# YiZhiXiaoGuLI/xerus

Measured on AMD Instinct MI355X. Metric: GFLOP/s on TT contraction + TT-round sweep time, order-10 rank-256, higher is better.
Workload: dtype f64; 1 GPU; TT order-10 n=20 rank-256: <x,y> + x.round(256) per step; order=10, mode_size=20, rank=256, parallelism=replicas x1

## Files before the change

include/xerus_amd.h:

```cpp
#ifndef XERUS_AMD_H
#define XERUS_AMD_H

#include <stddef.h>
#include <stdint.h>

#ifdef __cplusplus
extern "C" {
#endif

typedef struct xrs_handle_s* xrs_handle_t;

#define XRS_OK 0
#define XRS_EINVAL (-1)
#define XRS_ENOMEM (-2)
#define XRS_EHIP (-3)
#define XRS_ENUMERIC 1

int xrs_create(xrs_handle_t* handle, int device);
int xrs_destroy(xrs_handle_t handle);
int xrs_set_stream(xrs_handle_t handle, void* hip_stream);
void* xrs_get_stream(xrs_handle_t handle);
int xrs_synchronize(xrs_handle_t handle);
const char* xrs_last_error(void);
const char* xrs_version(void);

int xrs_malloc(xrs_handle_t handle, void** ptr, size_t bytes);
int xrs_free(xrs_handle_t handle, void* ptr);
size_t xrs_pool_bytes(xrs_handle_t handle);
int xrs_upload(xrs_handle_t handle, double* dst_dev, const double* src_host, size_t n);
int xrs_download(xrs_handle_t handle, double* dst_host, const double* src_dev, size_t n);
int xrs_memset_zero(xrs_handle_t handle, double* dst_dev, size_t n);
int xrs_copy(xrs_handle_t handle, double* dst_dev, const double* src_dev, size_t n);

int xrs_nrm2(xrs_handle_t handle, double* result, const double* x, size_t n);
int xrs_dot(xrs_handle_t handle, double* result, const double* x, const double* y, size_t n);
int xrs_asum(xrs_handle_t handle, double* result, const double* x, size_t n);
int xrs_scal(xrs_handle_t handle, double* x, double alpha, size_t n);
int xrs_axpy(xrs_handle_t handle, double* y, double alpha, const double* x, size_t n);
int xrs_scale_rows(xrs_handle_t handle, double* X, const double* s, size_t m, size_t n);

int xrs_gemm(xrs_handle_t handle, double* C, size_t M, size_t N, double alpha,
             const double* A, size_t lda, int transA, size_t K,
             const double* B, size_t ldb, int transB);

int xrs_gemm_batched(xrs_handle_t handle, size_t count, double* const* C, size_t M, size_t N, double alpha,
                     const double* const* A, size_t lda, int transA, size_t K,
                     const double* const* B, size_t ldb, int transB);

int xrs_gemm_sym(xrs_handle_t handle, double* C, size_t N, double alpha,
                 const double* A, size_t lda, int transA, size_t K,
                 const double* B, size_t ldb, int transB);

int xrs_gemm_f32(xrs_handle_t handle, float* C, size_t M, size_t N, float alpha,
                 const float* A, size_t lda, int transA, size_t K,
                 const float* B, size_t ldb, int transB);

int xrs_permute(xrs_handle_t handle, double* out, const double* in, size_t ndim,
                const size_t* dims, const size_t* shuffle);

int xrs_qc(xrs_handle_t handle, double* Q, double* C, size_t* rank, const double* A, size_t m, size_t n);
int xrs_cq(xrs_handle_t handle, double* C, double* Q, size_t* rank, const double* A, size_t m, size_t n);
int xrs_qr(xrs_handle_t handle, double* Q, double* R, const double* A, size_t m, size_t n);
int xrs_rq(xrs_handle_t handle, double* R, double* Q, const double* A, size_t m, size_t n);
int xrs_svd(xrs_handle_t handle, double* U, double* S, double* Vt, const double* A, size_t m, size_t n);
int xrs_svd_batched(xrs_handle_t handle, double* U, double* S, double* Vt, int* status,
                    const double* A, size_t batch, size_t m, size_t n);
int xrs_svd_batched_fits(size_t m, size_t n);
int xrs_solve(xrs_handle_t handle, double* X, const double* A, size_t m, size_t n, const double* B, size_t p);
int xrs_solve_least_squares(xrs_handle_t handle, double* X, const double* A, size_t m, size_t n, const double* B, size_t p);
int xrs_svd_rows_vt(xrs_handle_t handle, double* S, double* Vt, int* sweeps, const double* A, size_t p, size_t q, int kernel);
int xrs_sym_tridiag(xrs_handle_t handle, double* d, double* e, const double* A, size_t n);
int xrs_sym_eig_top(xrs_handle_t handle, double* lam, double* Ut, int* status, const double* A, size_t n, size_t kk);


int xrs_tt_move_core(xrs_handle_t handle, size_t d, const size_t* n, size_t* r, double** cores,
                     int canonicalized, size_t core_position, size_t position, int keep_rank);
int xrs_tt_round(xrs_handle_t handle, size_t d, const size_t* n, size_t* r, double** cores,
                 int canonicalized, size_t core_position, const size_t* max_ranks, double eps);
int xrs_tt_soft_threshold(xrs_handle_t handle, size_t d, const size_t* n, size_t* r, double** cores,
                          int canonicalized, size_t core_position, const double* taus);
int xrs_tt_entrywise_product(xrs_handle_t handle, size_t d, const size_t* ext, const size_t* ra, const double* const* A,
                             const size_t* rb, const double* const* B, double alpha, double** out);
int xrs_tt_entrywise_square(xrs_handle_t handle, size_t d, const size_t* ext, const size_t* r, const double* const* A,
                            double alpha, double** out, size_t* r_out);
int xrs_tt_rank_one_argmax(xrs_handle_t handle, size_t d, const size_t* ext, const double* const* cores, size_t* pos);
int xrs_tt_operator_apply(xrs_handle_t handle, size_t d, const size_t* n, const size_t* m, const size_t* p, const size_t* ra,
                          const double* const* A, const size_t* rb, const double* const* B, int transpose_a, double** out);
#define XRS_ROUND_CHAIN 1
#define XRS_ROUND_TRUNCATE 2
#define XRS_ROUND_REFERENCE 3
#define XRS_ROUND_GENERAL 4
int xrs_tt_last_round_path(xrs_handle_t handle);
int xrs_tt_dot(xrs_handle_t handle, double* result, size_t d, const size_t* n,
               const size_t* rx, const double* const* xcores,
               const size_t* ry, const double* const* ycores);

int xrs_tt_dot_async(xrs_handle_t handle, size_t d, const size_t* n,
                     const size_t* rx, const double* const* xcores,
                     const size_t* ry, const double* const* ycores);
int xrs_tt_dot_wait(xrs_handle_t handle, double* result);
int xrs_tt_dot_f32(xrs_handle_t handle, double* result, size_t d, const size_t* n,
                   const size_t* rx, const double* const* xcores,
                   const size_t* ry, const double* const* ycores);

int xrs_tt_tangent_project(xrs_handle_t handle, size_t d, const size_t* n, const size_t* ru, const double* const* U,
                           const size_t* rz, const double* const* Z, double** V, double** UU, size_t* fallback_edges);
int xrs_tt_tangent_to_tt(xrs_handle_t handle, size_t d, const size_t* n, const size_t* r, const double* const* U,
                         const double* const* V, int add_base, double** out);
int xrs_tt_tangent_dot(xrs_handle_t handle, double* result, size_t d, const size_t* n, const size_t* r,
                       const double* const* UU, const double* const* A, const double* const* B);

typedef int (*xrs_allreduce_fn)(void* ctx, double* buf, size_t count);
typedef int (*xrs_allgather_fn)(void* ctx, const double* send, double* recv, size_t count);

typedef struct xrs_comm_s* xrs_comm_t;
int xrs_comm_unique_id(void* id128_out);
int xrs_comm_create(xrs_handle_t handle, int nranks, int rank, const void* id128, xrs_comm_t* comm_out);
int xrs_comm_destroy(xrs_comm_t comm);
size_t xrs_comm_calls(xrs_comm_t comm);
int xrs_comm_allreduce(void* comm, double* buf, size_t count);
int xrs_comm_emulate(xrs_handle_t handle, int nranks, xrs_comm_t* comm_out);
int xrs_comm_allgather(void* comm, const double* send, double* recv, size_t count);

int xrs_tt_gather_sharded(xrs_handle_t handle, size_t d, const size_t* n_global, int world, int rank, const size_t* r,
                          const double* const* local_cores, double** full_cores_out, xrs_allgather_fn allgather, void* ctx);
int xrs_tt_shard(xrs_handle_t handle, size_t d, const size_t* n_global, int world, int rank, const size_t* r,
                 const double* const* full_cores, double** local_out);

int xrs_tt_round_sharded(xrs_handle_t handle, size_t d, const size_t* n_local, size_t* r, double** cores,
                         const size_t* max_ranks, double eps, xrs_allreduce_fn allreduce, void* ctx, int* certified);

int xrs_tt_round_sharded_ex(xrs_handle_t handle, size_t d, const size_t* n_local, size_t* r, double** cores,
                            const size_t* max_ranks, double eps, int world, int rank, xrs_allreduce_fn allreduce,
                            void* ctx, int* path);

int xrs_tt_dot_sharded(xrs_handle_t handle, double* result, size_t d, const size_t* n_local, const size_t* rx,
                       const double* const* X, const size_t* ry, const double* const* Y, xrs_allreduce_fn allreduce,
                       void* ctx);

int xrs_uq_basis(xrs_handle_t handle, double* P, const double* xi, size_t N, size_t n);
int xrs_uq_stack_congruence(xrs_handle_t handle, double* Lout, const double* Lprev, const double* X, const double* P,
                            size_t N, size_t a, size_t n, size_t b);
int xrs_uq_quadform(xrs_handle_t handle, double* result, const double* L, const double* V, size_t N, size_t a);


int xrs_philox_words(xrs_handle_t handle, uint32_t* out, size_t s, size_t q, uint64_t seed, uint32_t stream);
int xrs_gaussian_matrix(xrs_handle_t handle, double* G, size_t s, size_t m, uint64_t seed, uint32_t stream);
#define XRS_SKETCH_FUSED 1
#define XRS_SKETCH_MATERIALISED 2
int xrs_sketch_gaussian(xrs_handle_t handle, double* Y, size_t s, const double* A, size_t m, size_t n, uint64_t seed,
                        uint32_t stream, int route);
int xrs_sketch_last_route(xrs_handle_t handle);

#define XRS_KFAM_GEMM 1u
#define XRS_KFAM_PERMUTE 2u
#define XRS_KFAM_QR 4u
#define XRS_KFAM_SVD 8u
#define XRS_KFAM_ELEMWISE 16u
#define XRS_KFAM_SPLITK 32u
int xrs_prof_begin(xrs_handle_t handle, uint32_t family_mask);
int xrs_prof_end(xrs_handle_t handle, size_t* launches, double* total_ms, double* flops, double* bytes);

#ifdef __cplusplus
}
#endif
#endif
```

xerus_amd/capi.py:

```python
from __future__ import annotations

import ctypes as C
import os
from typing import Sequence

import numpy as np

_HERE = os.path.dirname(os.path.abspath(__file__))
LIB_PATH = os.environ.get("XRS_LIB_PATH") or os.path.join(_HERE, "libxerus_amd.so")

_SZ = C.c_size_t
_DP = C.c_void_p

SIGNATURES = {
    "xrs_create": (C.c_int, [C.POINTER(_DP), C.c_int]),
    "xrs_destroy": (C.c_int, [_DP]),
    "xrs_set_stream": (C.c_int, [_DP, _DP]),
    "xrs_get_stream": (_DP, [_DP]),
    "xrs_synchronize": (C.c_int, [_DP]),
    "xrs_last_error": (C.c_char_p, []),
    "xrs_version": (C.c_char_p, []),
    "xrs_malloc": (C.c_int, [_DP, C.POINTER(_DP), _SZ]),
    "xrs_free": (C.c_int, [_DP, _DP]),
    "xrs_pool_bytes": (_SZ, [_DP]),
    "xrs_upload": (C.c_int, [_DP, _DP, _DP, _SZ]),
    "xrs_download": (C.c_int, [_DP, _DP, _DP, _SZ]),
    "xrs_memset_zero": (C.c_int, [_DP, _DP, _SZ]),
    "xrs_copy": (C.c_int, [_DP, _DP, _DP, _SZ]),
    "xrs_nrm2": (C.c_int, [_DP, C.POINTER(C.c_double), _DP, _SZ]),
    "xrs_dot": (C.c_int, [_DP, C.POINTER(C.c_double), _DP, _DP, _SZ]),
    "xrs_asum": (C.c_int, [_DP, C.POINTER(C.c_double), _DP, _SZ]),
    "xrs_scal": (C.c_int, [_DP, _DP, C.c_double, _SZ]),
    "xrs_axpy": (C.c_int, [_DP, _DP, C.c_double, _DP, _SZ]),
    "xrs_scale_rows": (C.c_int, [_DP, _DP, _DP, _SZ, _SZ]),
    "xrs_gemm": (C.c_int, [_DP, _DP, _SZ, _SZ, C.c_double, _DP, _SZ, C.c_int, _SZ, _DP, _SZ, C.c_int]),
    "xrs_gemm_f32": (C.c_int, [_DP, _DP, _SZ, _SZ, C.c_float, _DP, _SZ, C.c_int, _SZ, _DP, _SZ, C.c_int]),
    "xrs_gemm_sym": (C.c_int,[_DP, _DP, _SZ, C.c_double, _DP, _SZ, C.c_int, _SZ, _DP, _SZ, C.c_int]),
    "xrs_gemm_batched": (C.c_int, [_DP, _SZ, C.POINTER(_DP), _SZ, _SZ, C.c_double, C.POINTER(_DP), _SZ, C.c_int, _SZ,
                                   C.POINTER(_DP), _SZ, C.c_int]),
    "xrs_permute": (C.c_int, [_DP, _DP, _DP, _SZ, C.POINTER(_SZ), C.POINTER(_SZ)]),
    "xrs_qc": (C.c_int, [_DP, _DP, _DP, C.POINTER(_SZ), _DP, _SZ, _SZ]),
    "xrs_cq": (C.c_int, [_DP, _DP, _DP, C.POINTER(_SZ), _DP, _SZ, _SZ]),
    "xrs_qr": (C.c_int, [_DP, _DP, _DP, _DP, _SZ, _SZ]),
    "xrs_rq": (C.c_int, [_DP, _DP, _DP, _DP, _SZ, _SZ]),
    "xrs_svd": (C.c_int, [_DP, _DP, _DP, _DP, _DP, _SZ, _SZ]),
    "xrs_svd_batched": (C.c_int, [_DP, _DP, _DP, _DP, C.POINTER(C.c_int), _DP, _SZ, _SZ, _SZ]),
    "xrs_svd_batched_fits": (C.c_int, [_SZ, _SZ]),
    "xrs_solve": (C.c_int, [_DP, _DP, _DP, _SZ, _SZ, _DP, _SZ]),
    "xrs_solve_least_squares": (C.c_int, [_DP, _DP, _DP, _SZ, _SZ, _DP, _SZ]),
    "xrs_svd_rows_vt": (C.c_int, [_DP, _DP, _DP, C.POINTER(C.c_int), _DP, _SZ, _SZ, C.c_int]),
    "xrs_sym_eig_top": (C.c_int, [_DP, _DP, _DP, C.POINTER(C.c_int), _DP, _SZ, _SZ]),
    "xrs_sym_tridiag": (C.c_int, [_DP, _DP, _DP, _DP, _SZ]),
    "xrs_tt_entrywise_product": (C.c_int, [_DP, _SZ, C.POINTER(_SZ), C.POINTER(_SZ), C.POINTER(_DP), C.POINTER(_SZ), C.POINTER(_DP),
                                           C.c_double, C.POINTER(_DP)]),
    "xrs_tt_entrywise_square": (C.c_int, [_DP, _SZ, C.POINTER(_SZ), C.POINTER(_SZ), C.POINTER(_DP), C.c_double, C.POINTER(_DP),
                                          C.POINTER(_SZ)]),
    "xrs_tt_rank_one_argmax": (C.c_int, [_DP, _SZ, C.POINTER(_SZ), C.POINTER(_DP), C.POINTER(_SZ)]),
    "xrs_tt_operator_apply": (C.c_int, [_DP, _SZ, C.POINTER(_SZ), C.POINTER(_SZ), C.POINTER(_SZ), C.POINTER(_SZ), C.POINTER(_DP),
                                        C.POINTER(_SZ), C.POINTER(_DP), C.c_int, C.POINTER(_DP)]),
    "xrs_tt_move_core": (C.c_int, [_DP, _SZ, C.POINTER(_SZ), C.POINTER(_SZ), C.POINTER(_DP), C.c_int, _SZ, _SZ, C.c_int]),
    "xrs_tt_round": (C.c_int, [_DP, _SZ, C.POINTER(_SZ), C.POINTER(_SZ), C.POINTER(_DP), C.c_int, _SZ,
                               C.POINTER(_SZ), C.c_double]),
    "xrs_tt_dot": (C.c_int, [_DP, C.POINTER(C.c_double), _SZ, C.POINTER(_SZ), C.POINTER(_SZ), C.POINTER(_DP),
                             C.POINTER(_SZ), C.POINTER(_DP)]),
    "xrs_tt_dot_async": (C.c_int, [_DP, _SZ, C.POINTER(_SZ), C.POINTER(_SZ), C.POINTER(_DP), C.POINTER(_SZ),
                                   C.POINTER(_DP)]),
    "xrs_tt_dot_wait": (C.c_int, [_DP, C.POINTER(C.c_double)]),
    "xrs_tt_dot_f32": (C.c_int, [_DP, C.POINTER(C.c_double), _SZ, C.POINTER(_SZ), C.POINTER(_SZ), C.POINTER(_DP),
                                 C.POINTER(_SZ), C.POINTER(_DP)]),
    "xrs_tt_round_sharded": (C.c_int, [_DP, _SZ, C.POINTER(_SZ), C.POINTER(_SZ), C.POINTER(_DP), C.POINTER(_SZ),
                                       C.c_double, _DP, _DP, C.POINTER(C.c_int)]),
    "xrs_tt_round_sharded_ex": (C.c_int, [_DP, _SZ, C.POINTER(_SZ), C.POINTER(_SZ), C.POINTER(_DP), C.POINTER(_SZ),
                                          C.c_double, C.c_int, C.c_int, _DP, _DP, C.POINTER(C.c_int)]),
    "xrs_tt_dot_sharded": (C.c_int, [_DP, C.POINTER(C.c_double), _SZ, C.POINTER(_SZ), C.POINTER(_SZ), C.POINTER(_DP),
                                     C.POINTER(_SZ), C.POINTER(_DP), _DP, _DP]),
    "xrs_tt_tangent_project": (C.c_int, [_DP, _SZ, C.POINTER(_SZ), C.POINTER(_SZ), C.POINTER(_DP), C.POINTER(_SZ),
                                         C.POINTER(_DP), C.POINTER(_DP), C.POINTER(_DP), C.POINTER(_SZ)]),
    "xrs_tt_tangent_to_tt": (C.c_int, [_DP, _SZ, C.POINTER(_SZ), C.POINTER(_SZ), C.POINTER(_DP), C.POINTER(_DP), C.c_int,
                                       C.POINTER(_DP)]),
    "xrs_tt_tangent_dot": (C.c_int, [_DP, C.POINTER(C.c_double), _SZ, C.POINTER(_SZ), C.POINTER(_SZ), C.POINTER(_DP),
                                     C.POINTER(_DP), C.POINTER(_DP)]),
    "xrs_tt_last_round_path": (C.c_int, [_DP]),
    "xrs_tt_soft_threshold": (C.c_int, [_DP, _SZ, C.POINTER(_SZ), C.POINTER(_SZ), C.POINTER(_DP), C.c_int, _SZ,
                                        C.POINTER(C.c_double)]),
    "xrs_comm_unique_id": (C.c_int, [_DP]),
    "xrs_comm_create": (C.c_int, [_DP, C.c_int, C.c_int, _DP, C.POINTER(_DP)]),
    "xrs_comm_emulate": (C.c_int, [_DP, C.c_int, C.POINTER(_DP)]),
    "xrs_comm_destroy": (C.c_int, [_DP]),
    "xrs_comm_calls": (_SZ, [_DP]),
    "xrs_comm_allreduce": (C.c_int, [_DP, _DP, _SZ]),
    "xrs_comm_allgather": (C.c_int, [_DP, _DP, _DP, _SZ]),
    "xrs_tt_gather_sharded": (C.c_int, [_DP, _SZ, C.POINTER(_SZ), C.c_int, C.c_int, C.POINTER(_SZ), C.POINTER(_DP),
                                        C.POINTER(_DP), _DP, _DP]),
    "xrs_tt_shard": (C.c_int, [_DP, _SZ, C.POINTER(_SZ), C.c_int, C.c_int, C.POINTER(_SZ), C.POINTER(_DP), C.POINTER(_DP)]),
    "xrs_uq_basis": (C.c_int, [_DP, _DP, _DP, _SZ, _SZ]),
    "xrs_uq_stack_congruence": (C.c_int, [_DP, _DP, _DP, _DP, _DP, _SZ, _SZ, _SZ, _SZ]),
    "xrs_uq_quadform": (C.c_int, [_DP, C.POINTER(C.c_double), _DP, _DP, _SZ, _SZ]),
    "xrs_philox_words": (C.c_int, [_DP, _DP, _SZ, _SZ, C.c_uint64, C.c_uint32]),
    "xrs_gaussian_matrix": (C.c_int, [_DP, _DP, _SZ, _SZ, C.c_uint64, C.c_uint32]),
    "xrs_sketch_gaussian": (C.c_int, [_DP, _DP, _SZ, _DP, _SZ, _SZ, C.c_uint64, C.c_uint32, C.c_int]),
    "xrs_sketch_last_route": (C.c_int, [_DP]),
    "xrs_prof_begin": (C.c_int, [_DP, C.c_uint32]),
    "xrs_prof_end": (C.c_int, [_DP, C.POINTER(_SZ), C.POINTER(C.c_double), C.POINTER(C.c_double),
                               C.POINTER(C.c_double)]),
}

KFAM_GEMM, KFAM_PERMUTE, KFAM_QR, KFAM_SVD, KFAM_ELEMWISE, KFAM_SPLITK = 1, 2, 4, 8, 16, 32
ROUND_PATHS = {0: None, 1: "chain", 2: "truncate", 3: "reference", 4: "general"}
SKETCH_AUTO, SKETCH_FUSED, SKETCH_MATERIALISED = 0, 1, 2
SKETCH_ROUTES = {0: None, 1: "fused", 2: "materialised"}

_lib = None


class XrsError(RuntimeError):

    def __init__(self, fn: str, code: int, msg: str):
        super().__init__(f"{fn} failed with status {code}: {msg}")
        self.code = code


def load(path: str | None = None) -> C.CDLL:
    global _lib
    if _lib is not None and path is None:
        return _lib
    p = path or LIB_PATH
    if not os.path.exists(p):
        raise ImportError(f"{p} is missing: build it with `python -c 'import __graft_entry__ as g; g.build()'`")
    lib = C.CDLL(p)
    for name, (res, args) in SIGNATURES.items():
        f = getattr(lib, name)
        f.restype = res
        f.argtypes = args
    if path is None:
        _lib = lib
    return lib


def _check(fn: str, status: int):
    if status != 0:
        raise XrsError(fn, status, load().xrs_last_error().decode())


def svd_batched_fits(m: int, n: int) -> bool:
    return bool(load().xrs_svd_batched_fits(int(m), int(n)))


def _arr(vals: Sequence[int]):
    return (_SZ * len(vals))(*[int(v) for v in vals])


class Handle:

    def __init__(self, device: int = 0):
        self.lib = load()
        self.h = _DP()
        _check("xrs_create", self.lib.xrs_create(C.byref(self.h), device))

    def close(self):
        if self.h:
            _check("xrs_destroy", self.lib.xrs_destroy(self.h))
            self.h = _DP()

    def __del__(self):
        try:
            self.close()
        except Exception:
            pass

    def malloc(self, nbytes: int) -> int:
        p = _DP()
        _check("xrs_malloc", self.lib.xrs_malloc(self.h, C.byref(p), nbytes))
        return p.value or 0

    def free(self, ptr: int):
        _check("xrs_free", self.lib.xrs_free(self.h, _DP(ptr)))

    def synchronize(self):
        _check("xrs_synchronize", self.lib.xrs_synchronize(self.h))

    def set_stream(self, stream_ptr: int | None):
        _check("xrs_set_stream", self.lib.xrs_set_stream(self.h, _DP(stream_ptr or 0)))

    def stream(self) -> int:
        return self.lib.xrs_get_stream(self.h) or 0

    def array(self, a: np.ndarray) -> "DeviceArray":
        return DeviceArray.from_host(self, a)

    def empty(self, shape) -> "DeviceArray":
        return DeviceArray(self, tuple(int(s) for s in shape))

    def zeros(self, shape) -> "DeviceArray":
        d = DeviceArray(self, tuple(int(s) for s in shape))
        _check("xrs_memset_zero", self.lib.xrs_memset_zero(self.h, _DP(d.ptr), d.size))
        return d

    def gemm(self, C_: "DeviceArray", M, N, alpha, A: "DeviceArray", lda, transA, K, B: "DeviceArray", ldb, transB):
        _check("xrs_gemm", self.lib.xrs_gemm(self.h, _DP(C_.ptr), M, N, alpha, _DP(A.ptr), lda, int(transA), K,
                                            _DP(B.ptr), ldb, int(transB)))

    def gemm_f32(self, C_: "Float32Array", M, N, alpha, A: "Float32Array", lda, transA, K, B: "Float32Array", ldb, transB):
        _check("xrs_gemm_f32", self.lib.xrs_gemm_f32(self.h, _DP(C_.ptr), M, N, float(alpha), _DP(A.ptr), lda, int(transA),
                                                    K, _DP(B.ptr), ldb, int(transB)))

    def array_f32(self, a: np.ndarray) -> "Float32Array":
        return Float32Array.from_host(self, a)

    def gemm_sym(self, C_: "DeviceArray", N, alpha, A: "DeviceArray", lda, transA, K, B: "DeviceArray", ldb, transB):
        _check("xrs_gemm_sym", self.lib.xrs_gemm_sym(self.h, _DP(C_.ptr), N, alpha, _DP(A.ptr), lda, int(transA), K,
                                                    _DP(B.ptr), ldb, int(transB)))

    def gemm_batched(self, Cs, M, N, alpha, As, lda, transA, K, Bs, ldb, transB):
        cnt = len(Cs)
        tab = lambda xs: (_DP * max(1, cnt))(*[_DP(x.ptr) for x in xs])
        _check("xrs_gemm_batched", self.lib.xrs_gemm_batched(self.h, cnt, tab(Cs), M, N, alpha, tab(As), lda, int(transA),
                                                            K, tab(Bs), ldb, int(transB)))

    def tangent_to_tt(self, n, r, Us, Vs, add_base: bool):
        d = len(n)
        tab = lambda xs: (_DP * d)(*[_DP(x.ptr) for x in xs])
        out = (_DP * d)()
        _check("xrs_tt_tangent_to_tt", self.lib.xrs_tt_tangent_to_tt(self.h, d, _arr(n), _arr(r), tab(Us), tab(Vs),
                                                                    int(add_base), out))
        cores = []
        for k in range(d):
            shape = (2 * r[k] if k else 1, n[k], 2 * r[k + 1] if k + 1 < d else 1)
            c = DeviceArray(self, shape, ptr=out[k])
            c.owned = True
            cores.append(c)
        return cores

    def matmul(self, A: "DeviceArray", transA: bool, B: "DeviceArray", transB: bool, alpha: float = 1.0):
        am, ak = (A.shape[1], A.shape[0]) if transA else (A.shape[0], A.shape[1])
        bk, bn = (B.shape[1], B.shape[0]) if transB else (B.shape[0], B.shape[1])
        assert ak == bk, (A.shape, B.shape)
        out = self.empty((am, bn))
        self.gemm(out, am, bn, alpha, A, A.shape[1], transA, ak, B, B.shape[1], transB)
        return out

    def permute(self, out: "DeviceArray", inp: "DeviceArray", dims, shuffle):
        _check("xrs_permute", self.lib.xrs_permute(self.h, _DP(out.ptr), _DP(inp.ptr), len(dims), _arr(dims),
                                                  _arr(shuffle)))

    def reshuffle(self, inp: "DeviceArray", shuffle):
        dims = inp.shape
        out_dims = [0] * len(dims)
        for i, s in enumerate(shuffle):
            out_dims[s] = dims[i]
        out = self.empty(tuple(out_dims))
        self.permute(out, inp, dims, shuffle)
        return out

    def nrm2(self, x: "DeviceArray") -> float:
        r = C.c_double()
        _check("xrs_nrm2", self.lib.xrs_nrm2(self.h, C.byref(r), _DP(x.ptr), x.size))
        return r.value

    def dot(self, x: "DeviceArray", y: "DeviceArray") -> float:
        r = C.c_double()
        _check("xrs_dot", self.lib.xrs_dot(self.h, C.byref(r), _DP(x.ptr), _DP(y.ptr), x.size))
        return r.value

    def asum(self, x: "DeviceArray") -> float:
        r = C.c_double()
        _check("xrs_asum", self.lib.xrs_asum(self.h, C.byref(r), _DP(x.ptr), x.size))
        return r.value

    def scal(self, x: "DeviceArray", alpha: float):
        _check("xrs_scal", self.lib.xrs_scal(self.h, _DP(x.ptr), alpha, x.size))

    def axpy(self, y: "DeviceArray", alpha: float, x: "DeviceArray"):
        _check("xrs_axpy", self.lib.xrs_axpy(self.h, _DP(y.ptr), alpha, _DP(x.ptr), x.size))

    def scale_rows(self, X: "DeviceArray", s: "DeviceArray"):
        _check("xrs_scale_rows", self.lib.xrs_scale_rows(self.h, _DP(X.ptr), _DP(s.ptr), X.shape[0], X.size // max(1, X.shape[0])))

    def qc(self, A: "DeviceArray"):
        m, n = A.shape
        k = min(m, n)
        Q, Cm = self.empty((m, k)), self.empty((k, n))
        r = _SZ()
        _check("xrs_qc", self.lib.xrs_qc(self.h, _DP(Q.ptr), _DP(Cm.ptr), C.byref(r), _DP(A.ptr), m, n))
        rank = r.value
        Q.shape, Cm.shape = (m, rank), (rank, n)
        return Q, Cm, rank

    def cq(self, A: "DeviceArray"):
        m, n = A.shape
        k = min(m, n)
        Cm, Q = self.empty((m, k)), self.empty((k, n))
        r = _SZ()
        _check("xrs_cq", self.lib.xrs_cq(self.h, _DP(Cm.ptr), _DP(Q.ptr), C.byref(r), _DP(A.ptr), m, n))
        rank = r.value
        Cm.shape, Q.shape = (m, rank), (rank, n)
        return Cm, Q, rank

    def qr(self, A: "DeviceArray"):
        m, n = A.shape
        k = min(m, n)
        Q, R = self.empty((m, k)), self.empty((k, n))
        _check("xrs_qr", self.lib.xrs_qr(self.h, _DP(Q.ptr), _DP(R.ptr), _DP(A.ptr), m, n))
        return Q, R

    def rq(self, A: "DeviceArray"):
        m, n = A.shape
        k = min(m, n)
        R, Q = self.empty((m, k)), self.empty((k, n))
        _check("xrs_rq", self.lib.xrs_rq(self.h, _DP(R.ptr), _DP(Q.ptr), _DP(A.ptr), m, n))
        return R, Q

    def svd(self, A: "DeviceArray"):
        m, n = A.shape
        k = min(m, n)
        U, S, Vt = self.empty((m, k)), self.empty((k,)), self.empty((k, n))
        _check("xrs_svd", self.lib.xrs_svd(self.h, _DP(U.ptr), _DP(S.ptr), _DP(Vt.ptr), _DP(A.ptr), m, n))
        return U, S, Vt

    def svd_batched(self, A: "DeviceArray", want_status: bool = True):
        batch, m, n = A.shape
        k = min(m, n)
        U, S, Vt = self.empty((batch, m, k)), self.empty((batch, k)), self.empty((batch, k, n))
        st = np.zeros(batch, dtype=np.intc) if want_status else None
        _check("xrs_svd_batched", self.lib.xrs_svd_batched(
            self.h, _DP(U.ptr), _DP(S.ptr), _DP(Vt.ptr), st.ctypes.data_as(C.POINTER(C.c_int)) if want_status else None,
            _DP(A.ptr), batch, m, n))
        return U, S, Vt, st

    def solve(self, A: "DeviceArray", B: "DeviceArray", least_squares: bool = False):
        m, n = A.shape
        p = B.shape[1] if len(B.shape) == 2 else 1
        X = self.empty((n, p) if len(B.shape) == 2 else (n,))
        fn = "xrs_solve_least_squares" if least_squares else "xrs_solve"
        _check(fn, getattr(self.lib, fn)(self.h, _DP(X.ptr), _DP(A.ptr), m, n, _DP(B.ptr), p))
        return X

    def sym_eig_top(self, A: "DeviceArray", kk: int):
        n = A.shape[0]
        lam, Ut, st = self.empty((kk,)), self.empty((kk, n)), C.c_int()
        _check("xrs_sym_eig_top", self.lib.xrs_sym_eig_top(self.h, _DP(lam.ptr), _DP(Ut.ptr), C.byref(st), _DP(A.ptr), n, kk))
        return lam, Ut, st.value

    def sym_tridiag(self, A: "DeviceArray"):
        n = A.shape[0]
        d, e = self.empty((n,)), self.empty((n,))
        _check("xrs_sym_tridiag", self.lib.xrs_sym_tridiag(self.h, _DP(d.ptr), _DP(e.ptr), _DP(A.ptr), n))
        return d.numpy(), e.numpy()[: n - 1]

    def svd_rows_vt(self, A: "DeviceArray", kernel: int = 0):
        p, q = A.shape
        S, Vt, sw = self.empty((p,)), self.empty((p, q)), C.c_int()
        _check("xrs_svd_rows_vt", self.lib.xrs_svd_rows_vt(self.h, _DP(S.ptr), _DP(Vt.ptr), C.byref(sw), _DP(A.ptr), p, q, kernel))
        return S, Vt, sw.value

    def tt_operator_apply(self, n, m, ra, A, rb, B, p=None, transpose=False):
        d = len(n)
        out = (_DP * d)()
        tab = lambda xs: (_DP * d)(*[_DP(x.ptr) for x in xs])
        _check("xrs_tt_operator_apply", self.lib.xrs_tt_operator_apply(
            self.h, d, _arr(n), _arr(m), _arr(p) if p is not None else None, _arr(ra), tab(A), _arr(rb), tab(B),
            int(transpose), out))
        res = []
        for k in range(d):
            nk = m[k] if transpose else n[k]
            shape = (ra[k] * rb[k], nk) + ((p[k],) if p is not None else ()) + (ra[k + 1] * rb[k + 1],)
            arr = DeviceArray(self, shape, ptr=out[k], owned=False)
            res.append(arr.numpy())
            self.free(out[k])
        return res

    def uq_basis(self, xi: "DeviceArray", n: int) -> "DeviceArray":
        N = xi.size
        P = self.empty((N, n))
        _check("xrs_uq_basis", self.lib.xrs_uq_basis(self.h, _DP(P.ptr), _DP(xi.ptr), N, n))
        return P

    def uq_stack_congruence(self, Lprev: "DeviceArray | None", X: "DeviceArray", P: "DeviceArray") -> "DeviceArray":
        a, n, b = X.shape
        N = P.shape[0]
        out = self.empty((N, b, b))
        _check("xrs_uq_stack_congruence", self.lib.xrs_uq_stack_congruence(
            self.h, _DP(out.ptr), _DP(Lprev.ptr) if Lprev is not None else None, _DP(X.ptr), _DP(P.ptr), N, a, n, b))
        return out

    def uq_quadform(self, L: "DeviceArray | None", V: "DeviceArray") -> float:
        N, a = V.shape
        r = C.c_double()
        _check("xrs_uq_quadform", self.lib.xrs_uq_quadform(self.h, C.byref(r), _DP(L.ptr) if L is not None else None,
                                                          _DP(V.ptr), N, a))
        return r.value

    @staticmethod
    def _seed_stream(fn: str, seed: int, stream: int):
        if not 0 <= int(seed) < 2 ** 64:
            raise XrsError(fn, -1, f"seed {seed} is not a 64-bit word")
        if not 0 <= int(stream) < 2 ** 32:
            raise XrsError(fn, -1, f"stream {stream} must be below 2^32")
        return int(seed), int(stream)

    def philox_words(self, s: int, q: int, seed: int, stream: int = 0) -> np.ndarray:
        seed, stream = self._seed_stream("xrs_philox_words", seed, stream)
        legal = 0 < s <= 2 ** 32 and q > 0
        buf = self.empty((2 * s * q,)) if legal else None
        _check("xrs_philox_words", self.lib.xrs_philox_words(self.h, _DP(buf.ptr) if legal else None, s, q, seed, stream))
        return buf.numpy().view(np.uint32).reshape(s, q, 4)

    def gaussian_matrix(self, s: int, m: int, seed: int, stream: int = 0) -> "DeviceArray":
        seed, stream = self._seed_stream("xrs_gaussian_matrix", seed, stream)
        legal = 0 < s <= 2 ** 32 and m > 0
        G = self.empty((s, m)) if legal else None
        _check("xrs_gaussian_matrix", self.lib.xrs_gaussian_matrix(self.h, _DP(G.ptr) if legal else None, s, m, seed, stream))
        return G

    def sketch_gaussian(self, s: int, A: "DeviceArray", seed: int, stream: int = 0, route: int = 0, m: int | None = None,
                        out: "DeviceArray | None" = None) -> "DeviceArray":
        seed, stream = self._seed_stream("xrs_sketch_gaussian", seed, stream)
        n = A.shape[1]
        m = A.shape[0] if m is None else int(m)
        legal = 0 < s <= 2 ** 32 and m > 0 and n > 0
        Y = out if out is not None else (self.empty((s, n)) if legal else None)
        _check("xrs_sketch_gaussian", self.lib.xrs_sketch_gaussian(self.h, _DP(Y.ptr) if Y is not None else None, s, _DP(A.ptr),
                                                                  m, n, seed, stream, int(route)))
        return Y

    def sketch_last_route(self) -> str | None:
        return SKETCH_ROUTES[self.lib.xrs_sketch_last_route(self.h)]

    def last_round_path(self) -> str | None:
        return ROUND_PATHS[self.lib.xrs_tt_last_round_path(self.h)]

    def prof_begin(self, mask: int):
        _check("xrs_prof_begin", self.lib.xrs_prof_begin(self.h, mask))

    def prof_end(self):
        n, ms, fl, by = _SZ(), C.c_double(), C.c_double(), C.c_double()
        _check("xrs_prof_end", self.lib.xrs_prof_end(self.h, C.byref(n), C.byref(ms), C.byref(fl), C.byref(by)))
        return {"launches": n.value, "ms": ms.value, "flops": fl.value, "bytes": by.value}


class DeviceArray:

    def __init__(self, handle: Handle, shape: tuple, ptr: int | None = None, owned: bool = True):
        self.handle = handle
        self.shape = tuple(shape)
        self.capacity = self.size
        self.owned = owned and ptr is None
        self.ptr = ptr if ptr is not None else (handle.malloc(max(8, self.capacity * 8)))

    @property
    def size(self) -> int:
        return int(np.prod(self.shape)) if self.shape else 1

    @classmethod
    def from_host(cls, handle: Handle, a: np.ndarray) -> "DeviceArray":
        a = np.ascontiguousarray(a, dtype=np.float64)
        d = cls(handle, a.shape)
        if a.size:
            _check("xrs_upload", handle.lib.xrs_upload(handle.h, _DP(d.ptr), a.ctypes.data_as(_DP), a.size))
        return d

    def numpy(self) -> np.ndarray:
        out = np.empty(self.shape, dtype=np.float64)
        assert self.size <= self.capacity, "shape exceeds the allocation"
        if self.size:
            _check("xrs_download", self.handle.lib.xrs_download(self.handle.h, out.ctypes.data_as(_DP), _DP(self.ptr),
                                                               self.size))
        return out

    def free(self):
        if self.owned and self.ptr:
            self.handle.free(self.ptr)
        self.ptr = 0

    def __del__(self):
        try:
            self.free()
        except Exception:
            pass


class Float32Array:

    def __init__(self, handle: Handle, shape: tuple, offset: int = 0):
        self.handle = handle
        self.shape = tuple(int(s) for s in shape)
        self.offset = int(offset)
        self._words = max(1, (self.size + self.offset + 1) // 2)
        self.base = handle.malloc(8 * self._words)
        self.ptr = self.base + 4 * self.offset

    @property
    def size(self) -> int:
        return int(np.prod(self.shape)) if self.shape else 1

    @classmethod
    def from_host(cls, handle: Handle, a: np.ndarray, offset: int = 0) -> "Float32Array":
        a = np.ascontiguousarray(a, dtype=np.float32)
        d = cls(handle, a.shape, offset)
        buf = np.zeros(2 * d._words, dtype=np.float32)
        buf[d.offset:d.offset + a.size] = a.ravel()
        _check("xrs_upload", handle.lib.xrs_upload(handle.h, _DP(d.base), buf.view(np.float64).ctypes.data_as(_DP), d._words))
        return d

    def numpy(self) -> np.ndarray:
        buf = np.empty(self._words, dtype=np.float64)
        _check("xrs_download", self.handle.lib.xrs_download(self.handle.h, buf.ctypes.data_as(_DP), _DP(self.base), self._words))
        return buf.view(np.float32)[self.offset:self.offset + self.size].reshape(self.shape).copy()

    def free(self):
        if self.base:
            self.handle.free(self.base)
        self.base = self.ptr = 0

    def __del__(self):
        try:
            self.free()
        except Exception:
            pass


class DotFuture:

    def __init__(self, handle: Handle):
        self.handle = handle
        self._value = None

    def result(self) -> float:
        if self._value is None:
            out = C.c_double()
            _check("xrs_tt_dot_wait", self.handle.lib.xrs_tt_dot_wait(self.handle.h, C.byref(out)))
            self._value = out.value
        return self._value


class TTDevice:

    def __init__(self, handle: Handle, dims, ranks, ptrs, canonicalized=False, core_position=0):
        self.handle = handle
        self.dims = [int(x) for x in dims]
        self.r = [int(x) for x in ranks]
        self.ptrs = list(ptrs)
        self.canonicalized = canonicalized
        self.core_position = core_position

    @classmethod
    def from_cores(cls, handle: Handle, cores, canonicalized=False, core_position=0) -> "TTDevice":
        dims = [c.shape[1] for c in cores]
        ranks = [cores[0].shape[0]] + [c.shape[2] for c in cores]
        ptrs = []
        for c in cores:
            c = np.ascontiguousarray(c, dtype=np.float64)
            p = handle.malloc(max(8, c.size * 8))
            _check("xrs_upload", handle.lib.xrs_upload(handle.h, _DP(p), c.ctypes.data_as(_DP), c.size))
            ptrs.append(p)
        return cls(handle, dims, ranks, ptrs, canonicalized, core_position)

    def clone(self) -> "TTDevice":
        ptrs = []
        for k, p in enumerate(self.ptrs):
            size = self.r[k] * self.dims[k] * self.r[k + 1]
            q = self.handle.malloc(max(8, size * 8))
            _check("xrs_copy", self.handle.lib.xrs_copy(self.handle.h, _DP(q), _DP(p), size))
            ptrs.append(q)
        return TTDevice(self.handle, self.dims, self.r, ptrs, self.canonicalized, self.core_position)

    @property
    def order(self):
        return len(self.dims)

    @property
    def ranks(self):
        return self.r[1:-1]

    def cores(self):
        out = []
        for k, p in enumerate(self.ptrs):
            shp = (self.r[k], self.dims[k], self.r[k + 1])
            a = np.empty(shp)
            _check("xrs_download", self.handle.lib.xrs_download(self.handle.h, a.ctypes.data_as(_DP), _DP(p), a.size))
            out.append(a)
        return out

    def _arrays(self):
        c = getattr(self, "_cache", None)
        if c is not None and c[3] is self.r and c[4] is self.ptrs:
            return c[0], c[1], c[2]
        d = self.order
        n = _arr(self.dims)
        r = _arr(self.r)
        cores = (_DP * d)(*self.ptrs)
        self._cache = (n, r, cores, self.r, self.ptrs)
        return n, r, cores

    def _writeback(self, r, cores):
        self.r = r[:]
        self.ptrs = [p or 0 for p in cores[:]]
        c = getattr(self, "_cache", None)
        if c is not None and c[1] is r and c[2] is cores:
            self._cache = (c[0], r, cores, self.r, self.ptrs)

    def move_core(self, position: int, keep_rank: bool = False):
        n, r, cores = self._arrays()
        st = self.handle.lib.xrs_tt_move_core(self.handle.h, self.order, n, r, cores, int(self.canonicalized),
                                              self.core_position, position, int(keep_rank))
        self._writeback(r, cores)
        _check("xrs_tt_move_core", st)
        self.canonicalized, self.core_position = True, position

    def round(self, max_ranks, eps: float = 8 * np.finfo(float).eps):
        d = self.order
        if isinstance(max_ranks, (int, np.integer)):
            max_ranks = [int(max_ranks)] * (d - 1)
        n, r, cores = self._arrays()
        key = tuple(max_ranks)
        mc = getattr(self, "_mr_cache", None)
        if mc is None or mc[0] != key:
            mc = (key, _arr(list(max_ranks) + [1]))
            self._mr_cache = mc
        mr = mc[1]
        st = self.handle.lib.xrs_tt_round(self.handle.h, d, n, r, cores, int(self.canonicalized), self.core_position,
                                          mr, eps)
        self._writeback(r, cores)
        _check("xrs_tt_round", st)
        self.canonicalized, self.core_position = True, 0

    def soft_threshold(self, taus):
        d = self.order
        if isinstance(taus, (int, float)):
            taus = [float(taus)] * (d - 1)
        n, r, cores = self._arrays()
        t = (C.c_double * max(1, d - 1))(*taus)
        st = self.handle.lib.xrs_tt_soft_threshold(self.handle.h, d, n, r, cores, int(self.canonicalized),
                                                   self.core_position, t)
        self._writeback(r, cores)
        _check("xrs_tt_soft_threshold", st)
        self.canonicalized, self.core_position = True, 0

    def dot(self, other: "TTDevice") -> float:
        if self.dims != other.dims:
            raise ValueError(f"dot of TTs with different dimensions: {self.dims} vs {other.dims}")
        out = C.c_double()
        n, rx, xc = self._arrays()
        _, ry, yc = other._arrays()
        _check("xrs_tt_dot", self.handle.lib.xrs_tt_dot(self.handle.h, C.byref(out), self.order, n, rx, xc, ry, yc))
        return out.value

    def dot_f32(self, other: "TTDevice") -> float:
        if self.dims != other.dims:
            raise ValueError(f"dot of TTs with different dimensions: {self.dims} vs {other.dims}")
        out = C.c_double()
        n, rx, xc = self._arrays()
        _, ry, yc = other._arrays()
        _check("xrs_tt_dot_f32", self.handle.lib.xrs_tt_dot_f32(self.handle.h, C.byref(out), self.order, n, rx, xc, ry, yc))
        return out.value

    def dot_async(self, other: "TTDevice") -> "DotFuture":
        if self.dims != other.dims:
            raise ValueError(f"dot of TTs with different dimensions: {self.dims} vs {other.dims}")
        if other.handle is not self.handle:
            raise ValueError("dot_async: both TTs must live on the same handle")
        n, rx, xc = self._arrays()
        _, ry, yc = other._arrays()
        _check("xrs_tt_dot_async", self.handle.lib.xrs_tt_dot_async(self.handle.h, self.order, n, rx, xc, ry, yc))
        return DotFuture(self.handle)

    def entrywise_square(self, alpha: float = 1.0) -> "TTDevice":
        d = self.order
        n, r, cores = self._arrays()
        out, r_out = (_DP * d)(), (_SZ * (d + 1))()
        _check("xrs_tt_entrywise_square", self.handle.lib.xrs_tt_entrywise_square(self.handle.h, d, n, r, cores, float(alpha),
                                                                                  out, r_out))
        return TTDevice(self.handle, self.dims, list(r_out), [p or 0 for p in out])

    def rank_one_argmax(self) -> list:
        if any(x != 1 for x in self.r):
            raise ValueError(f"rank_one_argmax needs ranks 1, got {self.r}")
        d = self.order
        n, _, cores = self._arrays()
        pos = (_SZ * d)()
        _check("xrs_tt_rank_one_argmax", self.handle.lib.xrs_tt_rank_one_argmax(self.handle.h, d, n, cores, pos))
        return [int(p) for p in pos]

    def frob_norm(self) -> float:
        if self.canonicalized:
            k = self.core_position
            size = self.r[k] * self.dims[k] * self.r[k + 1]
            return self.handle.nrm2(DeviceArray(self.handle, (size,), ptr=self.ptrs[k], owned=False))
        return float(np.sqrt(max(0.0, self.dot(self))))

    def free(self):
        for p in self.ptrs:
            if p:
                self.handle.free(p)
        self.ptrs = [0] * len(self.ptrs)

    def __del__(self):
        try:
            self.free()
        except Exception:
            pass
```

xerus_amd/csrc/chol_batch.hip:

```cpp
#include <algorithm>

#include "tt_common.hpp"

namespace xrs {

namespace {

using ttd::GemmJob;
using ttd::gemm_grouped;

static_assert(kCholLaunchJobs == kPotrfBatchMax);
constexpr int kBigMax = 64;
struct BigJob {
    const double* src;
    double shift_rel;
    int n;
    double* L;
    double* Z;
};

struct BigArgs {
    const double* src[kBigMax];
    double* w11[kBigMax];
    double* w21[kBigMax];
    double* w22[kBigMax];
    double shift[kBigMax];
    int n[kBigMax];
};

__global__ void __launch_bounds__(256) k_split_shift(const BigArgs a) {
    const int j = blockIdx.y, n = a.n[j], n1 = 256, n2 = n - 256;
    const double* A = a.src[j];
    __shared__ double red[4];
    double tr = 0.0;
    for (int i = threadIdx.x; i < n; i += 256) tr += A[size_t(i) * n + i];
#pragma unroll
    for (int o = 32; o > 0; o >>= 1) tr += __shfl_xor(tr, o, 64);
    if ((threadIdx.x & 63) == 0) red[threadIdx.x >> 6] = tr;
    __syncthreads();
    const double shift = a.shift[j] * (red[0] + red[1] + red[2] + red[3]);
    const size_t total = size_t(n) * n;
    for (size_t e = size_t(blockIdx.x) * 256 + threadIdx.x; e < total; e += size_t(gridDim.x) * 256) {
        const int r = int(e / n), c = int(e - size_t(r) * n);
        const double v = A[e] + (r == c ? shift : 0.0);
        if (r < n1 && c < n1) a.w11[j][size_t(r) * n1 + c] = v;
        else if (r >= n1 && c < n1) a.w21[j][size_t(r - n1) * n1 + c] = v;
        else if (r >= n1 && c >= n1) a.w22[j][size_t(r - n1) * n2 + (c - n1)] = v;
    }
}

struct SubArgs {
    double* y[kBigMax];
    const double* x[kBigMax];
    int count[kBigMax];
};

__global__ void __launch_bounds__(256) k_sub_batched(const SubArgs a) {
    const int j = blockIdx.y;
    for (int e = blockIdx.x * 256 + threadIdx.x; e < a.count[j]; e += gridDim.x * 256) a.y[j][e] -= a.x[j][e];
}

struct AssembleArgs {
    double* out[kBigMax];
    const double* b11[kBigMax];
    const double* b21[kBigMax];
    const double* b22[kBigMax];
    int n[kBigMax];
};

__global__ void __launch_bounds__(256) k_assemble_lower(const AssembleArgs a) {
    const int j = blockIdx.y, n = a.n[j], n1 = 256, n2 = n - 256;
    const size_t total = size_t(n) * n;
    for (size_t e = size_t(blockIdx.x) * 256 + threadIdx.x; e < total; e += size_t(gridDim.x) * 256) {
        const int r = int(e / n), c = int(e - size_t(r) * n);
        double v = 0.0;
        if (r < n1) v = c < n1 ? a.b11[j][size_t(r) * n1 + c] : 0.0;
        else v = c < n1 ? a.b21[j][size_t(r - n1) * n1 + c] : a.b22[j][size_t(r - n1) * n2 + (c - n1)];
        a.out[j][e] = v;
    }
}


void factor_big(xrs_handle_t h, const std::vector<BigJob>& jobs, int* status, std::vector<DevBuf>& keep) {
    const int nj = int(jobs.size());
    XRS_REQUIRE(nj <= kBigMax, "factor_big: too many jobs");
    constexpr int n1 = 256;
    BigArgs ba{};
    std::vector<double*> w11(nj), w21(nj), w22(nj), d11(nj), d22(nj), z11(nj), pp(nj);
    auto buf = [&](size_t elems) { keep.emplace_back(h, std::max<size_t>(elems, 1) * 8); return keep.back().d(); };
    size_t maxn2 = 0;
    for (int j = 0; j < nj; ++j) {
        const int n = jobs[j].n, n2 = n - n1;
        XRS_REQUIRE(n > n1 && n <= 2 * n1, "factor_big: n out of range");
        w11[j] = buf(size_t(n1) * n1);
        w21[j] = buf(size_t(n2) * n1);
        w22[j] = buf(size_t(n2) * n2);
        d11[j] = buf(dinv_elems(n1));
        d22[j] = buf(dinv_elems(n2));
        z11[j] = buf(size_t(n1) * n1);
        pp[j] = buf(size_t(n2) * n2);
        ba.src[j] = jobs[j].src;
        ba.w11[j] = w11[j];
        ba.w21[j] = w21[j];
        ba.w22[j] = w22[j];
        ba.shift[j] = jobs[j].shift_rel;
        ba.n[j] = n;
        maxn2 = std::max(maxn2, size_t(n2));
    }
    hipLaunchKernelGGL(k_split_shift, dim3(256, nj), dim3(256), 0, h->stream, ba);
    check_launch("k_split_shift");
    auto chol = [&](const std::vector<double*>& W, const std::vector<double*>& D, int first_slot, bool upper_half) {
        for (int b0 = 0; b0 < nj; b0 += kPotrfBatchMax) {
            PotrfBatch pb{};
            const int c = std::min(kPotrfBatchMax, nj - b0);
            for (int i = 0; i < c; ++i) {
                pb.src[i] = nullptr;
                pb.G[i] = W[b0 + i];
                pb.Dinv[i] = D[b0 + i];
                pb.shift[i] = 0.0;
                pb.n[i] = upper_half ? n1 : jobs[b0 + i].n - n1;
            }
            pb.status = status + first_slot + b0;
            potrf_batched(h, pb, c);
        }
    };
    auto inverse = [&](const std::vector<double*>& L, const std::vector<double*>& D, const std::vector<double*>& X,
                       bool upper_half, const std::vector<int>& which) {
        TrinvBatch tb{};
        int c = 0;
        for (int j : which) {
            tb.L[c] = L[j];
            tb.Dinv[c] = D[j];
            tb.X[c] = X[j];
            tb.n[c] = upper_half ? n1 : jobs[j].n - n1;
            ++c;
        }
        if (c) trinv_batched(h, tb, c);
    };
    std::vector<int> all(nj), fac;
    for (int j = 0; j < nj; ++j) {
        all[j] = j;
        if (jobs[j].L) fac.push_back(j);
    }
    chol(w11, d11, 0, true);
    inverse(w11, d11, z11, true, all);
    std::vector<GemmJob> g1, g2;
    for (int j = 0; j < nj; ++j) {
        const size_t n2 = size_t(jobs[j].n - n1);
        g1.push_back({n2, size_t(n1), size_t(n1), size_t(n1), size_t(n1), false, true, w21[j], z11[j], w21[j] == nullptr ? nullptr : buf(n2 * n1)});
    }
    std::vector<double*> l21(nj);
    for (int j = 0; j < nj; ++j) l21[j] = g1[j].C;
    gemm_grouped(h, g1);
    for (int j = 0; j < nj; ++j) {
        const size_t n2 = size_t(jobs[j].n - n1);
        g2.push_back({n2, n2, size_t(n1), size_t(n1), size_t(n1), false, true, l21[j], l21[j], pp[j], true});
    }
    gemm_grouped(h, g2);
    SubArgs sa{};
    for (int j = 0; j < nj; ++j) {
        sa.y[j] = w22[j];
        sa.x[j] = pp[j];
        sa.count[j] = (jobs[j].n - n1) * (jobs[j].n - n1);
    }
    hipLaunchKernelGGL(k_sub_batched, dim3(64, nj), dim3(256), 0, h->stream, sa);
    check_launch("k_sub_batched");
    chol(w22, d22, nj, false);
    if (fac.empty()) return;
    std::vector<double*> z22(nj, nullptr), tt(nj, nullptr), z21(nj, nullptr);
    for (int j : fac) {
        const size_t n2 = size_t(jobs[j].n - n1);
        z22[j] = buf(n2 * n2);
        tt[j] = buf(n2 * n1);
        z21[j] = buf(n2 * n1);
    }
    inverse(w22, d22, z22, false, fac);
    std::vector<GemmJob> g3, g4;
    for (int j : fac) {
        const size_t n2 = size_t(jobs[j].n - n1);
        g3.push_back({n2, size_t(n1), size_t(n1), size_t(n1), size_t(n1), false, false, l21[j], z11[j], tt[j]});
    }
    gemm_grouped(h, g3);
    for (int j : fac) {
        const size_t n2 = size_t(jobs[j].n - n1);
        GemmJob g{n2, size_t(n1), n2, n2, size_t(n1), false, false, z22[j], tt[j], z21[j]};
        g.alpha = -1.0;
        g4.push_back(g);
    }
    gemm_grouped(h, g4);
    AssembleArgs al{}, az{};
    int c = 0;
    for (int j : fac) {
        al.out[c] = jobs[j].L; al.b11[c] = w11[j]; al.b21[c] = l21[j]; al.b22[c] = w22[j]; al.n[c] = jobs[j].n;
        az.out[c] = jobs[j].Z; az.b11[c] = z11[j]; az.b21[c] = z21[j]; az.b22[c] = z22[j]; az.n[c] = jobs[j].n;
        ++c;
    }
    hipLaunchKernelGGL(k_assemble_lower, dim3(256, c), dim3(256), 0, h->stream, al);
    check_launch("k_assemble_lower");
    hipLaunchKernelGGL(k_assemble_lower, dim3(256, c), dim3(256), 0, h->stream, az);
    check_launch("k_assemble_lower");
}

}

int chol_status_count(const std::vector<CholJob>& jobs) {
    int c = 0;
    for (const CholJob& j : jobs) c += j.n > 512 ? chol_full_blocks(size_t(j.n)) : (j.n > 256 ? 2 : 1);
    return c;
}

void chol_enqueue(xrs_handle_t h, const std::vector<CholJob>& jobs, int* status, std::vector<DevBuf>& keep) {
    std::vector<const CholJob*> small, huge;
    std::vector<BigJob> big;
    size_t dsz = 0;
    for (const CholJob& j : jobs) {
        XRS_REQUIRE(j.A != nullptr && j.n >= 1, "chol_enqueue: empty job");
        if (j.n > 512) {
            huge.push_back(&j);
        } else if (j.n > 256) {
            double* Z = j.Z;
            if (j.L && !Z) {
                keep.emplace_back(h, size_t(j.n) * j.n * 8);
                Z = keep.back().d();
            }
            big.push_back({j.A, j.shift, j.n, j.L, Z});
        } else {
            small.push_back(&j);
            dsz += dinv_elems(j.n);
        }
    }
    const int ns = int(small.size());
    int slot = ns + 2 * int(big.size());
    for (const CholJob* j : huge) {
        chol_full(h, j->A, size_t(j->n), j->shift, j->L, j->Z, status + slot);
        slot += chol_full_blocks(size_t(j->n));
    }
    for (size_t b0 = 0; b0 < big.size(); b0 += kBigMax) {
        const std::vector<BigJob> part(big.begin() + long(b0), big.begin() + long(std::min(big.size(), b0 + kBigMax)));
        factor_big(h, part, status + ns + 2 * b0, keep);
    }
    if (ns == 0) return;
    keep.emplace_back(h, dsz * 8);
    double* dinv = keep.back().d();
    struct Inverse { const double* L; const double* Dinv; double* X; int n; };
    std::vector<Inverse> inv;
    for (int b0 = 0; b0 < ns; b0 += kPotrfBatchMax) {
        PotrfBatch pb{};
        const int c = std::min(kPotrfBatchMax, ns - b0);
        for (int i = 0; i < c; ++i) {
            const CholJob& j = *small[size_t(b0 + i)];
            pb.src[i] = j.A;
            pb.G[i] = j.L;
            pb.Dinv[i] = dinv;
            pb.shift[i] = j.shift;
            pb.n[i] = j.n;
            if (j.L && j.Z) inv.push_back({j.L, dinv, j.Z, j.n});
            dinv += dinv_elems(j.n);
        }
        pb.status = status + b0;
        potrf_batched(h, pb, c);
    }
    for (size_t b0 = 0; b0 < inv.size(); b0 += kTrinvBatchMax) {
        TrinvBatch tb{};
        const int c = int(std::min<size_t>(kTrinvBatchMax, inv.size() - b0));
        for (int i = 0; i < c; ++i) {
            const Inverse& v = inv[b0 + size_t(i)];
            tb.L[i] = v.L;
            tb.Dinv[i] = v.Dinv;
            tb.X[i] = v.X;
            tb.n[i] = v.n;
        }
        trinv_batched(h, tb, c);
    }
}

}
```

xerus_amd/csrc/elementwise.hpp:

```cpp
#pragma once
#include <algorithm>

#include "runtime.hpp"

namespace xrs {

void reduce_to_device(xrs_handle_t h, int mode, const double* x, const double* y, size_t n, double* out_dev,
                      double* partial = nullptr);
double reduce_to_host(xrs_handle_t h, int mode, const double* x, const double* y, size_t n);
void scal(xrs_handle_t h, double* x, double alpha, size_t n);
void axpy(xrs_handle_t h, double* y, double alpha, const double* x, size_t n);
void ldexp_copy(xrs_handle_t h, double* dst, const double* src, int ex, size_t n);
constexpr int kAmaxMany = 64;
void amax_enqueue(xrs_handle_t h, const double* const* x, const size_t* n, int count, double* out_dev);
void norms_enqueue(xrs_handle_t h, const double* const* x, const size_t* n, int count, double* out_dev);
int range_exponent(double am);
int range_exponent(xrs_handle_t h, const double* A, size_t n);
void scale_rows(xrs_handle_t h, double* X, const double* s, size_t m, size_t n);
void scale_cols(xrs_handle_t h, double* X, const double* s, size_t m, size_t n);
void diag_sum(xrs_handle_t h, double* out, const double* X, size_t P, size_t m);
void offset_add(xrs_handle_t h, double* out, const size_t* out_dims, const double* in, const size_t* in_dims, size_t nd,
                const size_t* offsets, double alpha);
void strided_eval(xrs_handle_t h, double* out, const double* in, size_t nd, const size_t* out_dims, const size_t* in_strides,
                  size_t nt, const size_t* tr_dims, const size_t* tr_strides, size_t base);

constexpr int kTriA = 1, kTriB = 2;
void gemm(xrs_handle_t h, double* C, size_t M, size_t N, double alpha, const double* A, size_t lda, bool ta, size_t K,
          const double* B, size_t ldb, bool tb, int tri = 0);
constexpr int kGemmBatchMax = 32;
void gemm_batched(xrs_handle_t h, int count, double* const* C, size_t M, size_t N, double alpha, const double* const* A,
                  size_t lda, bool ta, size_t K, const double* const* B, size_t ldb, bool tb, bool sym = false,
                  int tri = 0);
void gemm_sym(xrs_handle_t h, double* C, size_t N, double alpha, const double* A, size_t lda, bool ta, size_t K,
              const double* B, size_t ldb, bool tb);

struct GemmSpec {
    const double* A;
    const double* B;
    double* C;
    size_t M, N, K, lda, ldb;
    bool ta, tb;
};
inline void gemm(xrs_handle_t h, const GemmSpec& g) {
    gemm(h, g.C, g.M, g.N, 1.0, g.A, g.lda, g.ta, g.K, g.B, g.ldb, g.tb);
}

void permute(xrs_handle_t h, double* out, const double* in, size_t ndim, const size_t* dims, const size_t* shuffle);

}
```

xerus_amd/csrc/gemm.hip:

```cpp
#include <algorithm>
#include <type_traits>
#include <utility>
#include <cstdio>
#include <cstdlib>

#include <hip/hip_ext.h>

#include "elementwise.hpp"
#include "runtime.hpp"

namespace xrs {

typedef double d4 __attribute__((ext_vector_type(4)));

struct GemmOne {
    const double* A;
    const double* B;
    double* C;
    __host__ __device__ const double* a(int) const { return A; }
    __host__ __device__ const double* b(int) const { return B; }
    __device__ double* c(int) const { return C; }
};
struct GemmMany {
    const double* A[kGemmBatchMax];
    const double* B[kGemmBatchMax];
    double* C[kGemmBatchMax];
    __host__ __device__ const double* a(int i) const { return A[i]; }
    __host__ __device__ const double* b(int i) const { return B[i]; }
    __device__ double* c(int i) const { return C[i]; }
};

template <int BM, int BN, int WGM, int WGN, int WGK>
constexpr int gemm_min_waves() { return (BM * BN >= 128 * 128) ? 2 : 4; }

#ifdef XRS_GEMM_TRACE
__device__ unsigned long long* g_gemm_trace = nullptr;
__device__ unsigned long long* g_gemm_steps = nullptr;
#define XRS_TRACE_BEGIN                                                   \
    const unsigned long long xrs_t0 = __builtin_amdgcn_s_memrealtime();  \
    const unsigned long long xrs_c0 = __builtin_amdgcn_s_memtime();
#define XRS_TRACE_STEP(t)                                                                                   \
    if (threadIdx.x == 0 && g_gemm_steps != nullptr && (t) < 15) {                                          \
        const size_t wg = blockIdx.x + size_t(gridDim.x) * (blockIdx.y + size_t(gridDim.y) * blockIdx.z);   \
        g_gemm_steps[16 * wg + (t)] = __builtin_amdgcn_s_memtime() - xrs_c0;                                \
    }
#define XRS_TRACE_END                                                                                     \
    if (threadIdx.x == 0 && g_gemm_trace != nullptr) {                                                    \
        const size_t wg = blockIdx.x + size_t(gridDim.x) * (blockIdx.y + size_t(gridDim.y) * blockIdx.z); \
        const unsigned long long t1 = __builtin_amdgcn_s_memrealtime();                                   \
        const unsigned hw = __builtin_amdgcn_s_getreg((31 << 11) | 4);                 \
        const unsigned xcc = __builtin_amdgcn_s_getreg((31 << 11) | 20);              \
        g_gemm_trace[3 * wg] = xrs_t0;                                                                   \
        g_gemm_trace[3 * wg + 1] = t1;                                                                   \
        g_gemm_trace[3 * wg + 2] = (static_cast<unsigned long long>(xcc) << 32) | hw;                    \
        if (g_gemm_steps != nullptr) g_gemm_steps[16 * wg + 15] = __builtin_amdgcn_s_memtime() - xrs_c0;  \
    }
#else
#define XRS_TRACE_BEGIN
#define XRS_TRACE_END
#define XRS_TRACE_STEP(t)
#endif

template <int BM, int BN, int GBK, int WGM, int WGN, int WGK, int PD, bool TA, bool TB, class PTR>
__device__ __forceinline__ void gemm_body(const PTR& ptrs, size_t lda, size_t ldb, int M, int N, int K, int kps,
                                          double alpha, double* __restrict__ slab, int tiles_m, int xcd_group,
                                          int* __restrict__ tickets, int sym);

template <int BM, int BN, int GBK, int WGM, int WGN, int WGK, int PD, bool TA, bool TB, class PTR>
__global__ void __launch_bounds__(WGM * WGN * WGK * 64, (gemm_min_waves<BM, BN, WGM, WGN, WGK>()))
k_gemm_f64(const PTR ptrs, size_t lda, size_t ldb, int M, int N, int K, int kps, double alpha,
           double* __restrict__ slab, int tiles_m, int xcd_group, int* __restrict__ tickets, int sym) {
    XRS_TRACE_BEGIN
    gemm_body<BM, BN, GBK, WGM, WGN, WGK, PD, TA, TB, PTR>(ptrs, lda, ldb, M, N, K, kps, alpha, slab, tiles_m,
                                                          xcd_group, tickets, sym);
    XRS_TRACE_END
}

template <int TM, int TN, int WGM, int WGN, int WGK, int NACC, class PTR>
__device__ __forceinline__ void gemm_finish(d4 (&acc2)[NACC][TM][TN], double* lds, const PTR& ptrs, int M, int N,
                                            double alpha, double* __restrict__ slab, int* __restrict__ tickets,
                                            int sym, int m0, int n0, int wm, int wn, int kg, int pos, int xb, int yb, int zb) {
    const int bz = yb;
    double* __restrict__ C = ptrs.c(bz);
    const int zslice = bz * int(gridDim.z) + zb;
    const int tslot = bz * int(gridDim.x) + xb;
    const int tid = threadIdx.x;
    const int lane = tid & 63;
    const bool mirror = sym != 0;
    d4 acc[TM][TN];
#pragma unroll
    for (int i = 0; i < TM; ++i)
#pragma unroll
        for (int j = 0; j < TN; ++j) {
            acc[i][j] = acc2[0][i][j];
            if constexpr (NACC > 1) acc[i][j] += acc2[1][i][j];
        }
    if constexpr (WGK > 1) {
        double* red = lds;
        if (kg > 0) {
#pragma unroll
            for (int i = 0; i < TM; ++i)
#pragma unroll
                for (int j = 0; j < TN; ++j)
#pragma unroll
                    for (int r = 0; r < 4; ++r)
                        red[((((kg - 1) * (WGM * WGN) + pos) * TM * TN + i * TN + j) * 4 + r) * 64 + lane] = acc[i][j][r];
        }
        __syncthreads();
        if (kg > 0 && tickets == nullptr) return;
        if (kg == 0)
#pragma unroll
        for (int g = 1; g < WGK; ++g)
#pragma unroll
            for (int i = 0; i < TM; ++i)
#pragma unroll
                for (int j = 0; j < TN; ++j)
#pragma unroll
                    for (int r = 0; r < 4; ++r)
                        acc[i][j][r] += red[((((g - 1) * (WGM * WGN) + pos) * TM * TN + i * TN + j) * 4 + r) * 64 + lane];
    }
    const bool to_slab = slab != nullptr;
    const size_t MN = size_t(M) * size_t(N);
    double* out = to_slab ? slab + size_t(zslice) * MN : C;
    const double scale = to_slab ? 1.0 : alpha;
    const int lc = lane & 15, lg = lane >> 4;
    if (kg == 0) {
#pragma unroll
        for (int i = 0; i < TM; ++i)
#pragma unroll
            for (int j = 0; j < TN; ++j) {
                const int col = n0 + wn + j * 16 + lc;
#pragma unroll
                for (int r = 0; r < 4; ++r) {
                    const int row = m0 + wm + i * 16 + lg + 4 * r;
                    if (row < M && col < N) {
                        if (tickets != nullptr)
                            __hip_atomic_store(&out[size_t(row) * N + col], acc[i][j][r], __ATOMIC_RELAXED,
                                               __HIP_MEMORY_SCOPE_AGENT);
                        else if (!mirror || to_slab)
                            out[size_t(row) * N + col] = scale * acc[i][j][r];
                        else if (row >= col) {
                            out[size_t(row) * N + col] = scale * acc[i][j][r];
                            out[size_t(col) * N + row] = scale * acc[i][j][r];
                        }
                    }
                }
            }
    }
    if (tickets == nullptr) return;
    asm volatile("s_waitcnt vmcnt(0)" ::: "memory");
    __syncthreads();
    double* flag = lds;
    if (tid == 0) {
        const int t = __hip_atomic_fetch_add(&tickets[tslot], 1, __ATOMIC_RELAXED, __HIP_MEMORY_SCOPE_AGENT);
        const bool last = (t == int(gridDim.z) - 1);
        if (last) __hip_atomic_store(&tickets[tslot], 0, __ATOMIC_RELAXED, __HIP_MEMORY_SCOPE_AGENT);
        flag[0] = last ? 1.0 : 0.0;
    }
    __syncthreads();
    if (flag[0] == 0.0 || kg != 0) return;
#pragma unroll
    for (int i = 0; i < TM; ++i)
#pragma unroll
        for (int j = 0; j < TN; ++j) {
            const int col = n0 + wn + j * 16 + lc;
#pragma unroll
            for (int r = 0; r < 4; ++r) {
                const int row = m0 + wm + i * 16 + lg + 4 * r;
                if (row < M && col < N && (!mirror || row >= col)) {
                    const size_t o = size_t(row) * N + col;
                    double sum = 0.0;
                    for (int z = 0; z < int(gridDim.z); ++z)
                        sum += (z == zb) ? acc[i][j][r]
                                                      : __hip_atomic_load(&slab[(size_t(bz) * gridDim.z + z) * MN + o], __ATOMIC_RELAXED,
                                                                          __HIP_MEMORY_SCOPE_AGENT);
                    C[o] = alpha * sum;
                    if (mirror) C[size_t(col) * N + row] = alpha * sum;
                }
            }
        }
}


template <int BM, int BN, int GBK, int WGM, int WGN, int WGK, int PD, bool TA, bool TB, class PTR>
__device__ __forceinline__ void gemm_body(const PTR& ptrs, size_t lda, size_t ldb, int M, int N, int K, int kps,
                                          double alpha, double* __restrict__ slab, int tiles_m, int xcd_group,
                                          int* __restrict__ tickets, int sym) {
    const int bz = blockIdx.y;
    const double* __restrict__ A = ptrs.a(bz);
    const double* __restrict__ B = ptrs.b(bz);
    constexpr int NT = WGM * WGN * WGK * 64;
    constexpr int SA = BM;
    constexpr int SB = BN;
    static_assert(BM % 16 == 0 && BN % 16 == 0, "tile rows must be whole MFMA tiles");
    constexpr bool WIDE_SWZ_A = BM % 32 == 0, WIDE_SWZ_B = BN % 32 == 0;
    constexpr int WM = BM / WGM, WN = BN / WGN;
    constexpr int TM = WM / 16, TN = WN / 16;
    static_assert(TM >= 1 && TN >= 1, "wave tile smaller than one MFMA tile");
    constexpr int NACC = (TM * TN <= 2) ? 2 : 1;
    constexpr int A_PER = (BM * GBK + NT - 1) / NT;
    constexpr int B_PER = (BN * GBK + NT - 1) / NT;

    __shared__ double As[2][GBK * SA];
    __shared__ double Bs[2][GBK * SB];

    const int tid = threadIdx.x;
    const int lane = tid & 63;
    const int wave = tid >> 6;
    const int kg = wave / (WGM * WGN);
    const int pos = wave % (WGM * WGN);
    const int wm = (pos / WGN) * WM;
    const int wn = (pos % WGN) * WN;
    static_assert(GBK % (4 * WGK) == 0, "K-step must split evenly over the wave groups");
    static_assert(WGK == 1 || (WGK - 1) * BM * BN <= 2 * GBK * (SA + SB), "LDS reduction buffer too small");

    int tm, tn;
    {
        const int b = blockIdx.x, tiles_n = gridDim.x / tiles_m;
        if (xcd_group == 1) {
            const int xcd = b & 7, slot = b >> 3;
            tn = (slot / tiles_m) * 8 + xcd;
            tm = slot % tiles_m;
        } else if (xcd_group == 2) {
            const int xcd = b & 7, slot = b >> 3;
            tm = (slot / tiles_n) * 8 + xcd;
            tn = slot % tiles_n;
        } else {
            tm = b % tiles_m;
            tn = b / tiles_m;
        }
    }
    if (sym && tm < tn) return;
    const int m0 = tm * BM, n0 = tn * BN;
    const int kbeg = blockIdx.z * kps;
    const int kend = min(K, kbeg + kps);

    d4 acc2[NACC][TM][TN];
#pragma unroll
    for (int a = 0; a < NACC; ++a)
#pragma unroll
        for (int i = 0; i < TM; ++i)
#pragma unroll
            for (int j = 0; j < TN; ++j) acc2[a][i][j] = d4{0.0, 0.0, 0.0, 0.0};
    auto swza = [](int k) { return WIDE_SWZ_A ? (((k & 1) << 4) | (k & 15)) : (k & 15); };
    auto swzb = [](int k) { return WIDE_SWZ_B ? (((k & 1) << 4) | (k & 15)) : (k & 15); };

    double ra[PD][A_PER], rb[PD][B_PER];

    auto a_coord = [&](int e, int& m, int& k) {
        const int idx = tid + e * NT;
        if (TA) { m = idx % BM; k = idx / BM; } else { k = idx % GBK; m = idx / GBK; }
    };
    auto b_coord = [&](int e, int& n, int& k) {
        const int idx = tid + e * NT;
        if (TB) { k = idx % GBK; n = idx / GBK; } else { n = idx % BN; k = idx / BN; }
    };
    auto load_tile = [&](int k0, auto slot_c) {
        constexpr int slot = decltype(slot_c)::value;
#pragma unroll
        for (int e = 0; e < A_PER; ++e) {
            int m, k;
            a_coord(e, m, k);
            const int gm = min(m0 + m, M - 1), gk = min(k0 + k, kend - 1);
            ra[slot][e] = TA ? A[size_t(gk) * lda + gm] : A[size_t(gm) * lda + gk];
        }
#pragma unroll
        for (int e = 0; e < B_PER; ++e) {
            int n, k;
            b_coord(e, n, k);
            const int gn = min(n0 + n, N - 1), gk = min(k0 + k, kend - 1);
            rb[slot][e] = TB ? B[size_t(gn) * ldb + gk] : B[size_t(gk) * ldb + gn];
        }
    };
    auto store_tile = [&](int buf, int k0, auto slot_c) {
        constexpr int slot = decltype(slot_c)::value;
#pragma unroll
        for (int e = 0; e < A_PER; ++e) {
            int m, k;
            a_coord(e, m, k);
            const bool ok = (m0 + m < M) && (k0 + k < kend);
            if ((BM * GBK) % NT == 0 || tid + e * NT < BM * GBK) As[buf][k * SA + (m ^ swza(k))] = ok ? ra[slot][e] : 0.0;
        }
#pragma unroll
        for (int e = 0; e < B_PER; ++e) {
            int n, k;
            b_coord(e, n, k);
            const bool ok = (n0 + n < N) && (k0 + k < kend);
            if ((BN * GBK) % NT == 0 || tid + e * NT < BN * GBK) Bs[buf][k * SB + (n ^ swzb(k))] = ok ? rb[slot][e] : 0.0;
        }
    };
    const int lr = lane & 15, lk = lane >> 4;
    auto compute = [&](int buf) {
        const double* as = As[buf];
        const double* bs = Bs[buf];
#pragma unroll
        for (int q = 0; q < GBK / (4 * WGK); ++q) {
            const int kk = (q * WGK + kg) * 4;
            double af[TM], bf[TN];
#pragma unroll
            for (int i = 0; i < TM; ++i) af[i] = as[(kk + lk) * SA + ((wm + i * 16 + lr) ^ swza(kk + lk))];
#pragma unroll
            for (int j = 0; j < TN; ++j) bf[j] = bs[(kk + lk) * SB + ((wn + j * 16 + lr) ^ swzb(kk + lk))];
#pragma unroll
            for (int i = 0; i < TM; ++i)
#pragma unroll
                for (int j = 0; j < TN; ++j)
                    acc2[q % NACC][i][j] = __builtin_amdgcn_mfma_f64_16x16x4f64(af[i], bf[j], acc2[q % NACC][i][j], 0, 0, 0);
        }
    };

    const int nsteps = (kend > kbeg) ? (kend - kbeg + GBK - 1) / GBK : 0;
    if (nsteps > 0) {
        static_assert(PD % 2 == 0, "ring depth must be even (LDS double buffer parity)");
        [&]<int... U>(std::integer_sequence<int, U...>) {
            (load_tile(kbeg + U * GBK, std::integral_constant<int, U>{}), ...);
        }(std::make_integer_sequence<int, PD>{});
        store_tile(0, kbeg, std::integral_constant<int, 0>{});
        __syncthreads();
        int t0 = 0;
        for (; t0 + 2 * PD <= nsteps; t0 += PD) {
            [&]<int... U>(std::integer_sequence<int, U...>) {
                (([&] {
                     const int t = t0 + U;
                     compute(U & 1);
                     store_tile((U + 1) & 1, kbeg + (t + 1) * GBK, std::integral_constant<int, (U + 1) % PD>{});
                     load_tile(kbeg + (t + PD) * GBK, std::integral_constant<int, U>{});
                     __syncthreads();
                 }()),
                 ...);
            }(std::make_integer_sequence<int, PD>{});
        }
        for (; t0 < nsteps; t0 += PD) {
            [&]<int... U>(std::integer_sequence<int, U...>) {
                (([&] {
                     const int t = t0 + U;
                     if (t < nsteps) {
                         compute(U & 1);
                         if (t + 1 < nsteps)
                             store_tile((U + 1) & 1, kbeg + (t + 1) * GBK, std::integral_constant<int, (U + 1) % PD>{});
                         if (t + PD < nsteps) load_tile(kbeg + (t + PD) * GBK, std::integral_constant<int, U>{});
                     }
                     __syncthreads();
                 }()),
                 ...);
            }(std::make_integer_sequence<int, PD>{});
        }
    }

    gemm_finish<TM, TN, WGM, WGN, WGK, NACC>(acc2, &As[0][0], ptrs, M, N, alpha, slab, tickets, sym, m0, n0, wm, wn, kg, pos,
                                             int(blockIdx.x), int(blockIdx.y), int(blockIdx.z));
}

constexpr int kGldsBK = 32;

template <int R, bool KMAJ, int BK = kGldsBK>
struct GldsImg {
    static_assert(!KMAJ || R % 16 == 0, "k-major image rows must be whole MFMA tiles");
    static constexpr int KSWZ = (R % 32 == 0) ? 8 : 0;
    static constexpr int DOUBLES = R * BK;
    static constexpr int INSTR = DOUBLES * 8 / 1024;
    __device__ static int at(int r, int k) {
        if constexpr (!KMAJ) return r * BK + ((((k >> 1) ^ (r & 15))) << 1) + (k & 1);
        else return k * R + ((((r >> 1) ^ ((k & 1) * KSWZ))) << 1) + (r & 1);
    }
    template <int NF, int WGK>
    struct Frag {
        static_assert((WGK & (WGK - 1)) == 0, "wave groups must be a power of 2");
        int base[KMAJ ? NF : 1];
        int z = 0;
        __device__ Frag(int w0, int kg, int lane) {
            const int lr = lane & 15, lk = lane >> 4;
            if constexpr (!KMAJ) {
                base[0] = (w0 + lr) * BK + (lk & 1);
                z = (2 * kg) ^ (lk >> 1) ^ lr;
            } else {
                const int swz = (lk & 1) * (KSWZ / 8);
#pragma unroll
                for (int i = 0; i < NF; ++i) base[i] = (4 * kg + lk) * R + 16 * ((w0 / 16 + i) ^ swz) + lr;
            }
        }
        __device__ int off(int q, int i) const {
            if constexpr (!KMAJ) return base[0] + i * 16 * BK + (((2 * q * WGK) ^ z) << 1);
            else return base[i] + 4 * q * WGK * R;
        }
    };
    __device__ static void src(int q, int& r, int& k) {
        if constexpr (!KMAJ) {
            constexpr int CPR = BK / 2;
            r = q / CPR;
            k = ((q % CPR) ^ (r & 15)) << 1;
        } else {
            constexpr int CR = R / 2;
            k = q / CR;
            r = ((q % CR) ^ ((k & 1) * KSWZ)) << 1;
        }
    }
};

template <int BM, int BN, int WGM, int WGN, int WGK>
constexpr int glds_min_waves() { return (WGM * WGN * WGK * 64 >= 512) ? 2 : 1; }

template <int BK, int ST = 0>
constexpr int glds_stages() { return ST > 0 ? ST : (BK == 64 ? 2 : 3); }
template <int BM, int BN, int BK = kGldsBK, int ST = 0>
constexpr int glds_lds_doubles() { return glds_stages<BK, ST>() * (BM + BN) * BK; }

template <int BM, int BN, int WGM, int WGN, int WGK, bool TA, bool TB, class PTR, int BK = kGldsBK, int ST = 0>
__device__ __forceinline__ void glds_body(double* __restrict__ lds, const PTR& ptrs, size_t lda, size_t ldb, int M, int N,
                                          int K, int kps, double alpha, double* __restrict__ slab, int tiles_m,
                                          int xcd_group, int* __restrict__ tickets, int sym, int tri) {
#ifdef XRS_GEMM_TRACE
    const unsigned long long xrs_c0 = __builtin_amdgcn_s_memtime();
#endif
    constexpr int S = glds_stages<BK, ST>();
    constexpr int NW = WGM * WGN * WGK;
    using IA = GldsImg<BM, TA, BK>;
    using IB = GldsImg<BN, !TB, BK>;
    constexpr int STAGE = IA::DOUBLES + IB::DOUBLES;
    static_assert(S * STAGE == glds_lds_doubles<BM, BN, BK, ST>(), "LDS layout");
    constexpr int INSTR = IA::INSTR + IB::INSTR;
    constexpr int PER_WAVE = (INSTR + NW - 1) / NW;
    static_assert(PER_WAVE * (S - 2) <= 63, "vmcnt range");
    constexpr int WM = BM / WGM, WN = BN / WGN;
    constexpr int TM = WM / 16, TN = WN / 16;
    static_assert(TM >= 1 && TN >= 1 && WM % 16 == 0 && WN % 16 == 0, "wave tile must be whole MFMA tiles");
    static_assert(BK % (4 * WGK) == 0, "K-step must split evenly over the wave groups");
    constexpr int NACC = (TM * TN <= 2) ? 2 : 1;
    static_assert(WGK == 1 || (WGK - 1) * WGM * WGN * TM * TN * 256 <= S * STAGE, "LDS reduction buffer too small");

    int xb = int(blockIdx.x), bz = int(blockIdx.y), zb = int(blockIdx.z);
    if (xcd_group == 3) {
        const int X = int(gridDim.x), Y = int(gridDim.y);
        const int L = xb + X * (bz + Y * zb), c = L & 7, q = L >> 3;
        const int u = c + 8 * (q / X);
        xb = q % X;
        bz = u % Y;
        zb = u / Y;
    }
    const double* __restrict__ A = ptrs.a(bz);
    const double* __restrict__ B = ptrs.b(bz);
    const int tid = threadIdx.x, lane = tid & 63, wave = tid >> 6;
    const int kg = wave / (WGM * WGN), pos = wave % (WGM * WGN);
    const int wm = (pos / WGN) * WM, wn = (pos % WGN) * WN;
    int tm, tn;
    if (sym) {
        const int x = xb;
        tm = int((__builtin_sqrtf(8.0f * float(x) + 1.0f) - 1.0f) * 0.5f);
        while ((tm + 1) * (tm + 2) / 2 <= x) ++tm;
        while (tm * (tm + 1) / 2 > x) --tm;
        tn = x - tm * (tm + 1) / 2;
    } else {
        const int b = xb, tiles_n = gridDim.x / tiles_m;
        if (xcd_group == 1) {
            const int xcd = b & 7, slot = b >> 3;
            tn = (slot / tiles_m) * 8 + xcd;
            tm = slot % tiles_m;
        } else if (xcd_group == 2) {
            const int xcd = b & 7, slot = b >> 3;
            tm = (slot / tiles_n) * 8 + xcd;
            tn = slot % tiles_n;
        } else {
            tm = b % tiles_m;
            tn = b / tiles_m;
        }
    }
    const int m0 = tm * BM, n0 = tn * BN;
    const int klo = (tri & 2) ? (n0 / BK) * BK : 0;
    const int khi = (tri & 1) ? min(K, (m0 + BM + BK - 1) / BK * BK) : K;
    const int kbeg = max(zb * kps, klo);
    const int nsteps = max(0, min(khi, zb * kps + kps) - kbeg) / BK;
    const bool full = wave < INSTR % NW || INSTR % NW == 0;

    const double* gsrc[PER_WAVE];
    size_t gstep[PER_WAVE];
    int ldsoff[PER_WAVE];
#pragma unroll
    for (int u = 0; u < PER_WAVE; ++u) {
        const int j = min(wave + NW * u, INSTR - 1);
        int r, k;
        if (j < IA::INSTR) {
            IA::src((j * 64) + lane, r, k);
            gsrc[u] = TA ? A + size_t(kbeg + k) * lda + (m0 + r) : A + size_t(m0 + r) * lda + (kbeg + k);
            gstep[u] = TA ? size_t(BK) * lda : size_t(BK);
            ldsoff[u] = j * 128;
        } else {
            IB::src(((j - IA::INSTR) * 64) + lane, r, k);
            gsrc[u] = TB ? B + size_t(n0 + r) * ldb + (kbeg + k) : B + size_t(kbeg + k) * ldb + (n0 + r);
            gstep[u] = TB ? size_t(BK) : size_t(BK) * ldb;
            ldsoff[u] = IA::DOUBLES + (j - IA::INSTR) * 128;
        }
    }
    auto issue = [&](int t) {
        double* st = lds + (t % S) * STAGE;
#pragma unroll
        for (int u = 0; u < PER_WAVE; ++u)
            if (u < PER_WAVE - 1 || full)
            __builtin_amdgcn_global_load_lds(static_cast<const void*>(gsrc[u] + size_t(t) * gstep[u]),
                                             (__attribute__((address_space(3))) void*)(st + ldsoff[u]),
                                             16, 0, 0);
    };

    d4 acc2[NACC][TM][TN];
#pragma unroll
    for (int a = 0; a < NACC; ++a)
#pragma unroll
        for (int i = 0; i < TM; ++i)
#pragma unroll
            for (int j = 0; j < TN; ++j) acc2[a][i][j] = d4{0.0, 0.0, 0.0, 0.0};
    const typename IA::template Frag<TM, WGK> fa(wm, kg, lane);
    const typename IB::template Frag<TN, WGK> fb(wn, kg, lane);

#pragma unroll
    for (int s = 0; s < S - 1; ++s)
        if (s < nsteps) issue(s);
    for (int t = 0; t < nsteps; ++t) {
        const int ahead = min(S - 2, nsteps - 1 - t);
        if (ahead <= 0) asm volatile("s_waitcnt vmcnt(0)" ::: "memory");
        else if (ahead == 1) {
            if (full) asm volatile("s_waitcnt vmcnt(%0)" ::"n"(PER_WAVE) : "memory");
            else asm volatile("s_waitcnt vmcnt(%0)" ::"n"(PER_WAVE - 1) : "memory");
        } else {
            if (full) asm volatile("s_waitcnt vmcnt(%0)" ::"n"(PER_WAVE * (S - 2)) : "memory");
            else asm volatile("s_waitcnt vmcnt(%0)" ::"n"((PER_WAVE - 1) * (S - 2)) : "memory");
        }
        asm volatile("s_waitcnt lgkmcnt(0)" ::: "memory");
        __builtin_amdgcn_s_barrier();
        XRS_TRACE_STEP(t)
        const double* as = lds + (t % S) * STAGE;
        const double* bs = as + IA::DOUBLES;
        constexpr int NQ = BK / (4 * WGK);
        double af[2][TM], bf[2][TN];
        auto frag = [&](int q, double(&a)[TM], double(&b)[TN]) {
#pragma unroll
            for (int i = 0; i < TM; ++i) a[i] = as[fa.off(q, i)];
#pragma unroll
            for (int j = 0; j < TN; ++j) b[j] = bs[fb.off(q, j)];
        };
        frag(0, af[0], bf[0]);
#ifndef XRS_GLDS_NOLOAD
        if (t + S - 1 < nsteps) issue(t + S - 1);
#endif
#pragma unroll
        for (int q = 0; q < NQ; ++q) {
            if (q + 1 < NQ) frag(q + 1, af[(q + 1) & 1], bf[(q + 1) & 1]);
            __builtin_amdgcn_sched_barrier(0);
#pragma unroll
            for (int i = 0; i < TM; ++i)
#pragma unroll
                for (int j = 0; j < TN; ++j)
                    acc2[q % NACC][i][j] = __builtin_amdgcn_mfma_f64_16x16x4f64(af[q & 1][i], bf[q & 1][j], acc2[q % NACC][i][j], 0, 0, 0);
        }
    }
    __syncthreads();
    gemm_finish<TM, TN, WGM, WGN, WGK, NACC>(acc2, lds, ptrs, M, N, alpha, slab, tickets, sym, m0, n0, wm, wn, kg, pos, xb, bz, zb);
}

template <int BM, int BN, int WGM, int WGN, int WGK, bool TA, bool TB, class PTR, int BK = kGldsBK, int ST = 0>
__global__ void __launch_bounds__(WGM * WGN * WGK * 64, (glds_min_waves<BM, BN, WGM, WGN, WGK>()))
k_gemm_glds(const PTR ptrs, size_t lda, size_t ldb, int M, int N, int K, int kps, double alpha,
            double* __restrict__ slab, int tiles_m, int xcd_group, int* __restrict__ tickets, int sym, int tri) {
    XRS_TRACE_BEGIN
    __shared__ double lds[glds_lds_doubles<BM, BN, BK, ST>()];
    glds_body<BM, BN, WGM, WGN, WGK, TA, TB, PTR, BK, ST>(lds, ptrs, lda, ldb, M, N, K, kps, alpha, slab, tiles_m, xcd_group,
                                                      tickets, sym, tri);
    XRS_TRACE_END
}

#ifndef XRS_REDUCE_CHUNK
#define XRS_REDUCE_CHUNK 16
#endif
constexpr int kReduceChunk = XRS_REDUCE_CHUNK;

__device__ __forceinline__ double slice_sum(const double* __restrict__ slab, size_t MN, int splits, size_t i) {
    double s = 0.0;
    for (int z0 = 0; z0 < splits; z0 += kReduceChunk) {
        double v[kReduceChunk];
#pragma unroll
        for (int u = 0; u < kReduceChunk; ++u)
            v[u] = (z0 + u < splits) ? __builtin_nontemporal_load(&slab[size_t(z0 + u) * MN + i]) : 0.0;
#pragma unroll
        for (int u = 0; u < kReduceChunk; ++u)
            if (z0 + u < splits) s += v[u];
    }
    return s;
}

template <class PTR>
__global__ void __launch_bounds__(256) k_splitk_reduce(const PTR ptrs, const double* __restrict__ slab, size_t MN,
                                                       int splits, double alpha, int symN) {
    double* __restrict__ C = ptrs.c(blockIdx.y);
    slab += size_t(blockIdx.y) * splits * MN;
    const size_t stride = size_t(gridDim.x) * blockDim.x;
    for (size_t i = size_t(blockIdx.x) * blockDim.x + threadIdx.x; i < MN; i += stride) {
        size_t row = 0, col = 0;
        if (symN) {
            row = i / size_t(symN);
            col = i - row * size_t(symN);
            if (col > row) continue;
        }
        const double s = alpha * slice_sum(slab, MN, splits, i);
        C[i] = s;
        if (symN) C[col * size_t(symN) + row] = s;
    }
}

constexpr int kSymTile = 16;
template <class PTR>
__global__ void __launch_bounds__(256) k_splitk_reduce_sym(const PTR ptrs, const double* __restrict__ slab, int N,
                                                           int splits, double alpha) {
    __shared__ double t[kSymTile][kSymTile + 1];
    double* __restrict__ C = ptrs.c(blockIdx.y);
    const size_t MN = size_t(N) * N;
    slab += size_t(blockIdx.y) * splits * MN;
    int ti = int((sqrt(8.0 * blockIdx.x + 1.0) - 1.0) * 0.5);
    while ((ti + 1) * (ti + 2) / 2 <= int(blockIdx.x)) ++ti;
    while (ti * (ti + 1) / 2 > int(blockIdx.x)) --ti;
    const int tj = int(blockIdx.x) - ti * (ti + 1) / 2;
    const int r = int(threadIdx.x) / kSymTile, c = int(threadIdx.x) % kSymTile;
    const size_t row = size_t(ti) * kSymTile + r, col = size_t(tj) * kSymTile + c;
    const bool diag = ti == tj;
    const double s = (!diag || c <= r) ? alpha * slice_sum(slab, MN, splits, row * N + col) : 0.0;
    t[c][r] = s;
    __syncthreads();
    C[row * N + col] = (diag && c > r) ? t[r][c] : s;
    if (!diag) C[(size_t(tj) * kSymTile + r) * N + size_t(ti) * kSymTile + c] = t[r][c];
}

template <class PTR>
static void splitk_reduce(xrs_handle_t h, const PTR& P, int count, const double* slab, int M, int N, int splits,
                          double alpha, bool sym) {
    static const bool sym_tiled = [] {
        const char* e = std::getenv("XRS_REDUCE_SYM");
        return !(e && e[0] == '0');
    }();
    const size_t MN = size_t(M) * N;
    KernelTimer timer(h, XRS_KFAM_SPLITK, count * double(MN) * splits, count * 8.0 * double(MN) * (splits + 1), true);
    if (sym && sym_tiled && N % kSymTile == 0) {
        const unsigned T = unsigned(N / kSymTile);
        hipExtLaunchKernelGGL(k_splitk_reduce_sym<PTR>, dim3(T * (T + 1) / 2, unsigned(count)), dim3(256), 0, h->stream,
                              timer.start(), timer.stop(), 0, P, slab, N, splits, alpha);
        check_launch("k_splitk_reduce_sym");
        return;
    }
    const unsigned blocks = unsigned(std::min<size_t>((MN + 255) / 256, 4096));
    hipExtLaunchKernelGGL(k_splitk_reduce<PTR>, dim3(blocks, unsigned(count)), dim3(256), 0, h->stream, timer.start(),
                          timer.stop(), 0, P, slab, MN, splits, alpha, sym ? N : 0);
    check_launch("k_splitk_reduce");
}

template <int BM, int BN, int GBK, int WGM, int WGN, int WGK, int PD, class PTR>
static void launch_tiles(xrs_handle_t h, const PTR& P, int count, size_t lda, bool ta, size_t ldb, bool tb,
                         int M, int N, int K, int splits, int kps, double alpha, double* slab, int* tickets, int sym) {
    const int tiles_m = (M + BM - 1) / BM, tiles_n = (N + BN - 1) / BN;
    dim3 grid(unsigned(tiles_m * tiles_n), unsigned(count), unsigned(splits));
    int xg = 0;
    if (double(N) >= double(M)) xg = (tiles_n % 8 == 0) ? 1 : 0;
    else xg = (tiles_m % 8 == 0) ? 2 : 0;
    KernelTimer timer(h, XRS_KFAM_GEMM, count * 2.0 * double(M) * double(N) * double(K),
                      count * 8.0 * (double(M) * K + double(K) * N + double(M) * N * splits), true);
#define XRS_GEMM_LAUNCH(TA_, TB_)                                                                             \
    hipExtLaunchKernelGGL((k_gemm_f64<BM, BN, GBK, WGM, WGN, WGK, PD, TA_, TB_, PTR>), grid, dim3(WGM * WGN * WGK * 64), 0, \
                          h->stream, timer.start(), timer.stop(), 0, P, lda, ldb, M, N, K, kps, alpha, slab, tiles_m, xg, tickets, sym)
    if (!ta && !tb) XRS_GEMM_LAUNCH(false, false);
    else if (!ta && tb) XRS_GEMM_LAUNCH(false, true);
    else if (ta && !tb) XRS_GEMM_LAUNCH(true, false);
    else XRS_GEMM_LAUNCH(true, true);
#undef XRS_GEMM_LAUNCH
    check_launch("k_gemm_f64");
}

template <int BM, int BN, int WGM, int WGN, int WGK, int BK = kGldsBK, int ST = 0, class PTR>
static void launch_glds(xrs_handle_t h, const PTR& P, int count, size_t lda, bool ta, size_t ldb, bool tb, int M, int N,
                        int K, int splits, int kps, double alpha, double* slab, int* tickets, int sym, int tri) {
    const int tiles_m = M / BM, tiles_n = N / BN;
    dim3 grid(unsigned(sym ? tiles_m * (tiles_m + 1) / 2 : tiles_m * tiles_n), unsigned(count), unsigned(splits));
    int xg = 0;
    if (double(N) >= double(M)) xg = (tiles_n % 8 == 0) ? 1 : 0;
    else xg = (tiles_m % 8 == 0) ? 2 : 0;
    static const bool xcd_split = [] {
        const char* e = std::getenv("XRS_GLDS_XCD_SPLIT");
        return !(e && e[0] == '0');
    }();
    if (xcd_split && splits >= 2 && (count * splits) % 8 == 0) xg = 3;
    double kdepth = double(K);
    if (tri & 1) {
        double s = 0;
        for (int m0 = 0; m0 < M; m0 += BM) s += std::min(K, (m0 + BM + BK - 1) / BK * BK);
        kdepth = s / tiles_m;
    } else if (tri & 2) {
        double s = 0;
        for (int n0 = 0; n0 < N; n0 += BN) s += K - (n0 / BK) * BK;
        kdepth = s / tiles_n;
    }
    KernelTimer timer(h, XRS_KFAM_GEMM, count * 2.0 * double(M) * double(N) * kdepth,
                      count * 8.0 * (double(M) * K + double(K) * N + double(M) * N * splits), true);
#define XRS_GLDS_LAUNCH(TA_, TB_)                                                                              \
    hipExtLaunchKernelGGL((k_gemm_glds<BM, BN, WGM, WGN, WGK, TA_, TB_, PTR, BK, ST>), grid, dim3(WGM * WGN * WGK * 64), 0, \
                          h->stream, timer.start(), timer.stop(), 0, P, lda, ldb, M, N, K, kps, alpha, slab, tiles_m, xg, tickets, sym, tri)
    if (!ta && !tb) XRS_GLDS_LAUNCH(false, false);
    else if (!ta && tb) XRS_GLDS_LAUNCH(false, true);
    else if (ta && !tb) XRS_GLDS_LAUNCH(true, false);
    else XRS_GLDS_LAUNCH(true, true);
#undef XRS_GLDS_LAUNCH
    check_launch("k_gemm_glds");
}

template <class PTR>
static bool gemm_glds(xrs_handle_t h, const PTR& P, int count, int M, int N, int K, double alpha, size_t lda, bool ta,
                      size_t ldb, bool tb, bool sym, int tri) {
    static const std::pair<int, int> g_env = [] {
        int v = -1, t = 256;
        if (const char* e = std::getenv("XRS_GEMM_GLDS")) std::sscanf(e, "%d,%d", &v, &t);
        return std::make_pair(v, t);
    }();
    const int g_var = g_env.first, g_target = g_env.second;
    static const int g_st2 = [] {
        const char* e = std::getenv("XRS_GLDS_ST2");
        return e ? std::atoi(e) : 7;
    }();
    if (g_var == 0) return false;
    if (K % kGldsBK != 0 || (lda & 1) || (ldb & 1)) return false;
    for (int i = 0; i < count; ++i)
        if ((reinterpret_cast<uintptr_t>(P.a(i)) & 15) || (reinterpret_cast<uintptr_t>(P.b(i)) & 15)) return false;
    const int bms[12] = {0, 64, 80, 64, 64, 32, 64, 80, 64, 80, 64, 64},
              bns[12] = {0, 80, 64, 64, 64, 32, 80, 64, 80, 64, 64, 64};
    auto fits = [&](int v) { return M % bms[v] == 0 && N % bns[v] == 0 && (!sym || bms[v] == bns[v]); };
    auto ntiles = [&](int v) {
        const long tm = M / bms[v], tn = N / bns[v];
        return sym ? long(count) * tm * (tm + 1) / 2 : long(count) * tm * tn;
    };
    int var = g_var;
    if (var < 0) {
        var = 0;
        if (sym) {
            if (fits(4)) var = 4;
            else if (fits(5)) var = 5;
        } else if (fits(6) && ntiles(6) >= 192) var = 6;
        else if (fits(7) && ntiles(7) >= 192) var = 7;
        else if (fits(4)) var = 4;
        else if (fits(5)) var = 5;
        if (var == 0) return false;
    }
    if (var < 1 || var > 11 || !fits(var)) return false;
    const int bk = kGldsBK;
    const long tiles = ntiles(var);
    const int ksteps = K / bk;
    int splits = 1;
    if (tiles < g_target) {
        const int nwaves = (var == 4 || var == 6 || var == 7) ? 8 : 4;
        const bool st2 = (var == 4 && (g_st2 & 2)) || ((var == 6 || var == 7) && (g_st2 & 1));
        const int nst = (bk == 64 || (st2 && !(g_st2 & 4))) ? 2 : 3;
        const int lds_kb = nst * (bms[var] + bns[var]) * bk * 8 / 1024;
        const long resident = long(g_target) * std::max(1, std::min(160 / lds_kb, 16 / nwaves));
        const int smax = std::max(1, ksteps * bk / 128);
        long best = -1;
        for (int s = 1; s <= smax; ++s) {
            const int steps = (ksteps + s - 1) / s, seff = (ksteps + steps - 1) / steps;
            const long cost = (tiles * seff + resident - 1) / resident * steps;
            if (best < 0 || cost < best) best = cost, splits = seff;
        }
    }
    int kps = (ksteps + splits - 1) / splits * bk;
    splits = (K + kps - 1) / kps;
    DevBuf slab;
    if (splits > 1) slab = DevBuf(h, size_t(count) * splits * M * N * sizeof(double));
    const bool small_slab = size_t(splits) * bms[var] * bns[var] * sizeof(double) <= 65536 && bms[var] * bns[var] <= 4096;
    const long grid_tiles = long(count) * (M / bms[var]) * (N / bns[var]);
    int* tickets = (splits > 1 && small_slab && grid_tiles <= xrs_handle_s::kTicketCap) ? h->tickets : nullptr;
#define XRS_GLDS(...) launch_glds<__VA_ARGS__>(h, P, count, lda, ta, ldb, tb, M, N, K, splits, kps, alpha, slab.d(), tickets, sym ? 1 : 0, tri)
    switch (var) {
        case 1: XRS_GLDS(64, 80, 4, 1, 1); break;
        case 2: XRS_GLDS(80, 64, 1, 4, 1); break;
        case 3: XRS_GLDS(64, 64, 2, 2, 1); break;
        case 4: if (g_st2 & 2) XRS_GLDS(64, 64, 2, 2, 2, kGldsBK, 2); else XRS_GLDS(64, 64, 2, 2, 2); break;
        case 6: if (g_st2 & 1) XRS_GLDS(64, 80, 4, 1, 2, kGldsBK, 2); else XRS_GLDS(64, 80, 4, 1, 2); break;
        case 7: if (g_st2 & 1) XRS_GLDS(80, 64, 1, 4, 2, kGldsBK, 2); else XRS_GLDS(80, 64, 1, 4, 2); break;
        case 8: XRS_GLDS(64, 80, 2, 1, 2); break;
        case 9: XRS_GLDS(80, 64, 1, 2, 2); break;
        case 10: XRS_GLDS(64, 64, 1, 1, 4); break;
        case 11: XRS_GLDS(64, 64, 2, 1, 2); break;
        default: XRS_GLDS(32, 32, 2, 2, 1); break;
    }
#undef XRS_GLDS
    if (splits > 1 && tickets == nullptr) splitk_reduce(h, P, count, slab.d(), M, N, splits, alpha, sym);
    return true;
}

template <class PTR>
static void gemm_impl(xrs_handle_t h, const PTR& P, int count, size_t Ms, size_t Ns, double alpha, size_t lda, bool ta,
                      size_t Ks, size_t ldb, bool tb, bool sym = false, int tri = 0) {
    const int M = int(Ms), N = int(Ns), K = int(Ks);
    if (gemm_glds(h, P, count, M, N, K, alpha, lda, ta, ldb, tb, sym, tri)) return;
    struct Cfg { int var = 0, kmin = 256, target = 512; };
    static const Cfg g_cfg = [] {
        Cfg c;
        if (const char* e = std::getenv("XRS_GEMM_CFG")) std::sscanf(e, "%d,%d,%d", &c.var, &c.kmin, &c.target);
        return c;
    }();
    const int cfg_var = g_cfg.var, cfg_kmin = g_cfg.kmin, cfg_target = g_cfg.target;
    auto ntiles = [&](int bm, int bn) { return long(count) * ((M + bm - 1) / bm) * ((N + bn - 1) / bn); };
    const int bms[16] = {0, 128, 64, 64, 32, 64, 64, 64, 64, 32, 32, 32, 32, 64, 64, 80},
              bns[16] = {0, 128, 64, 32, 32, 32, 64, 64, 32, 32, 32, 32, 32, 32, 80, 64};
    int var = cfg_var;
    long cfg_target_eff = cfg_target;
    if (sym) cfg_target_eff = 160;
    if (sym) {
        auto lower = [&](int b) { const long T = (M + b - 1) / b; return long(count) * T * (T + 1) / 2; };
        auto ntl = [&](int v) { return lower(bms[v]); };
        var = 4;
        if (lower(128) >= 1000) var = 1;
        else if (lower(64) >= 512) var = 2;
        else if (lower(32) < 512)
            for (int v : {1, 2, 4}) {
                const long t = ntl(v);
                const long sp = std::min<long>((cfg_target_eff + t - 1) / t, std::max<long>(1, K / cfg_kmin));
                if (t * sp >= cfg_target_eff) { var = v; break; }
            }
    } else if (var == 0) {
        if (ntiles(128, 128) >= 1000) var = 1;
        else if (ntiles(64, 64) >= 512) var = 2;
        else if (ntiles(32, 32) >= 1024) var = 4;
        else if (ntiles(64, 32) >= 256) var = 3;
        else if (ntiles(32, 32) >= 512) var = 4;
        else {
            var = 4;
            for (int v : {1, 2, 3}) {
                const long t = ntiles(bms[v], bns[v]);
                const long sp = std::min<long>((cfg_target_eff + t - 1) / t, std::max<long>(1, K / cfg_kmin));
                if (t * sp >= cfg_target_eff) { var = v; break; }
            }
        }
    }
    const long tiles = sym ? long(count) * ((M + bms[var] - 1) / bms[var]) * ((M + bms[var] - 1) / bms[var] + 1) / 2
                           : ntiles(bms[var], bns[var]);
    int splits = 1;
    if (tiles < cfg_target_eff) {
        const long want = (cfg_target_eff + tiles - 1) / tiles;
        const long maxs = std::max<long>(1, K / cfg_kmin);
        splits = int(std::max<long>(1, std::min(want, maxs)));
    }
    const int bk = ((var >= 5 && var <= 7) || var == 10 || var == 12 || var == 13 || var == 14 || var == 15) ? 32 : 16;
    int kps = (K + splits - 1) / splits;
    kps = (kps + bk - 1) / bk * bk;
    splits = (K + kps - 1) / kps;
    if (std::is_same<PTR, GemmMany>::value && var >= 5 && var <= 13) var = (var == 5 || var == 8 || var == 13) ? 3 : ((var == 9 || var >= 10) ? 4 : 2);
    DevBuf slab;
    if (splits > 1) slab = DevBuf(h, size_t(count) * splits * M * N * sizeof(double));
    const bool small_slab = size_t(splits) * bms[var] * bns[var] * sizeof(double) <= 65536 && bms[var] * bns[var] <= 4096;
    int* tickets = (splits > 1 && small_slab && ntiles(bms[var], bns[var]) <= xrs_handle_s::kTicketCap)
                       ? h->tickets : nullptr;
#define XRS_TILES(...) launch_tiles<__VA_ARGS__>(h, P, count, lda, ta, ldb, tb, M, N, K, splits, kps, alpha, slab.d(), tickets, sym ? 1 : 0)
    switch (var) {
        case 1: XRS_TILES(128, 128, 16, 2, 4, 1, 2); break;
        case 2: XRS_TILES(64, 64, 16, 2, 4, 1, 4); break;
        case 3: XRS_TILES(64, 32, 16, 2, 2, 2, 2); break;
        case 5: if constexpr (std::is_same<PTR, GemmOne>::value) XRS_TILES(64, 32, 32, 2, 2, 2, 4); break;
        case 6: if constexpr (std::is_same<PTR, GemmOne>::value) XRS_TILES(64, 64, 32, 2, 2, 1, 4); break;
        case 7: if constexpr (std::is_same<PTR, GemmOne>::value) XRS_TILES(64, 64, 32, 2, 2, 2, 4); break;
        case 8: if constexpr (std::is_same<PTR, GemmOne>::value) XRS_TILES(64, 32, 16, 2, 2, 2, 4); break;
        case 9: if constexpr (std::is_same<PTR, GemmOne>::value) XRS_TILES(32, 32, 16, 2, 2, 2, 4); break;
        case 10: if constexpr (std::is_same<PTR, GemmOne>::value) XRS_TILES(32, 32, 32, 2, 2, 2, 2); break;
        case 11: if constexpr (std::is_same<PTR, GemmOne>::value) XRS_TILES(32, 32, 16, 2, 2, 1, 2); break;
        case 12: if constexpr (std::is_same<PTR, GemmOne>::value) XRS_TILES(32, 32, 32, 2, 2, 4, 2); break;
        case 13: if constexpr (std::is_same<PTR, GemmOne>::value) XRS_TILES(64, 32, 32, 2, 2, 2, 2); break;
        case 14: XRS_TILES(64, 80, 32, 4, 1, 2, 2); break;
        case 15: XRS_TILES(80, 64, 32, 1, 4, 2, 2); break;
        default: XRS_TILES(32, 32, 16, 2, 2, 2, 2); break;
    }
#undef XRS_TILES
    if (splits > 1 && tickets == nullptr) splitk_reduce(h, P, count, slab.d(), M, N, splits, alpha, sym);
}

void gemm(xrs_handle_t h, double* C, size_t Ms, size_t Ns, double alpha, const double* A, size_t lda, bool ta, size_t Ks,
          const double* B, size_t ldb, bool tb, int tri) {
    if (Ms == 0 || Ns == 0) return;
    XRS_REQUIRE(Ms < (1u << 30) && Ns < (1u << 30) && Ks < (1u << 30), "GEMM dimension too large");
    if (Ks == 0) {
        XRS_HIP(hipMemsetAsync(C, 0, Ms * Ns * 8, h->stream));
        return;
    }
    gemm_impl(h, GemmOne{A, B, C}, 1, Ms, Ns, alpha, lda, ta, Ks, ldb, tb, false, tri);
}

void gemm_sym(xrs_handle_t h, double* C, size_t Ns, double alpha, const double* A, size_t lda, bool ta, size_t Ks,
              const double* B, size_t ldb, bool tb) {
    if (Ns == 0) return;
    XRS_REQUIRE(Ns < (1u << 30) && Ks < (1u << 30), "GEMM dimension too large");
    if (Ks == 0) {
        XRS_HIP(hipMemsetAsync(C, 0, Ns * Ns * 8, h->stream));
        return;
    }
    gemm_impl(h, GemmOne{A, B, C}, 1, Ns, Ns, alpha, lda, ta, Ks, ldb, tb, true);
}

void gemm_batched(xrs_handle_t h, int count, double* const* C, size_t Ms, size_t Ns, double alpha, const double* const* A,
                  size_t lda, bool ta, size_t Ks, const double* const* B, size_t ldb, bool tb, bool sym, int tri) {
    XRS_REQUIRE(!sym || Ms == Ns, "symmetric batch needs square results");
    if (Ms == 0 || Ns == 0 || count <= 0) return;
    XRS_REQUIRE(Ms < (1u << 30) && Ns < (1u << 30) && Ks < (1u << 30), "GEMM dimension too large");
    if (Ks == 0) {
        for (int i = 0; i < count; ++i) XRS_HIP(hipMemsetAsync(C[i], 0, Ms * Ns * 8, h->stream));
        return;
    }
    for (int b0 = 0; b0 < count; b0 += kGemmBatchMax) {
        const int c = std::min(kGemmBatchMax, count - b0);
        GemmMany P{};
        for (int i = 0; i < c; ++i) {
            P.A[i] = A[b0 + i];
            P.B[i] = B[b0 + i];
            P.C[i] = C[b0 + i];
        }
        gemm_impl(h, P, c, Ms, Ns, alpha, lda, ta, Ks, ldb, tb, sym, tri);
    }
}

}

#ifdef XRS_GEMM_TRACE
extern "C" int xrs_debug_gemm_trace(void* buf, void* steps) {
    unsigned long long* p = static_cast<unsigned long long*>(buf);
    unsigned long long* q = static_cast<unsigned long long*>(steps);
    return hipMemcpyToSymbol(HIP_SYMBOL(xrs::g_gemm_trace), &p, sizeof(p)) == hipSuccess &&
                   hipMemcpyToSymbol(HIP_SYMBOL(xrs::g_gemm_steps), &q, sizeof(q)) == hipSuccess
               ? 0 : 1;
}
#endif

extern "C" int xrs_gemm(xrs_handle_t h, double* C, size_t M, size_t N, double alpha, const double* A, size_t lda,
                        int transA, size_t K, const double* B, size_t ldb, int transB) {
    return xrs::guarded([&] {
        XRS_REQUIRE(h, "null handle");
        XRS_REQUIRE(M == 0 || N == 0 || C, "null C");
        XRS_REQUIRE(K == 0 || M == 0 || N == 0 || (A && B), "null A/B");
        XRS_REQUIRE(transA ? lda >= M || K == 0 : lda >= K || M == 0, "lda too small");
        XRS_REQUIRE(transB ? ldb >= K || N == 0 : ldb >= N || K == 0, "ldb too small");
        XRS_REQUIRE(C != A && C != B, "C must not alias A or B");
        xrs::fence_readers(h);
        xrs::gemm(h, C, M, N, alpha, A, lda, transA != 0, K, B, ldb, transB != 0);
    });
}

extern "C" int xrs_gemm_batched(xrs_handle_t h, size_t count, double* const* C, size_t M, size_t N, double alpha,
                                const double* const* A, size_t lda, int transA, size_t K, const double* const* B,
                                size_t ldb, int transB) {
    return xrs::guarded([&] {
        XRS_REQUIRE(h, "null handle");
        XRS_REQUIRE(count == 0 || (A && B && C), "null pointer table");
        XRS_REQUIRE(count < (1u << 20), "batch too large");
        XRS_REQUIRE(transA ? lda >= M || K == 0 : lda >= K || M == 0, "lda too small");
        XRS_REQUIRE(transB ? ldb >= K || N == 0 : ldb >= N || K == 0, "ldb too small");
        for (size_t i = 0; i < count; ++i) {
            XRS_REQUIRE(M == 0 || N == 0 || C[i], "null C");
            XRS_REQUIRE(K == 0 || M == 0 || N == 0 || (A[i] && B[i]), "null A/B");
            XRS_REQUIRE(C[i] != A[i] && C[i] != B[i], "C must not alias A or B");
        }
        xrs::fence_readers(h);
        xrs::gemm_batched(h, int(count), C, M, N, alpha, A, lda, transA != 0, K, B, ldb, transB != 0, false);
    });
}

extern "C" int xrs_gemm_sym(xrs_handle_t h, double* C, size_t N, double alpha, const double* A, size_t lda, int transA,
                            size_t K, const double* B, size_t ldb, int transB) {
    return xrs::guarded([&] {
        XRS_REQUIRE(h, "null handle");
        XRS_REQUIRE(N == 0 || C, "null C");
        XRS_REQUIRE(K == 0 || N == 0 || (A && B), "null A/B");
        XRS_REQUIRE(transA ? lda >= N || K == 0 : lda >= K || N == 0, "lda too small");
        XRS_REQUIRE(transB ? ldb >= K || N == 0 : ldb >= N || K == 0, "ldb too small");
        XRS_REQUIRE(C != A && C != B, "C must not alias A or B");
        xrs::fence_readers(h);
        xrs::gemm_sym(h, C, N, alpha, A, lda, transA != 0, K, B, ldb, transB != 0);
    });
}
```

xerus_amd/csrc/scratch_map.hpp:

```cpp
#pragma once
#include <string>

#include "runtime.hpp"

namespace xrs {
namespace scratch {

constexpr size_t kBytes = size_t(1) << 16;

struct Region {
    size_t off, len;
    const char* owner;
};

template <size_t N>
constexpr bool disjoint_within(const Region (&r)[N], size_t lo, size_t hi) {
    for (size_t i = 0; i < N; ++i) {
        if (r[i].len == 0 || r[i].off < lo || r[i].off + r[i].len > hi) return false;
        for (size_t j = 0; j < i; ++j)
            if (r[i].off < r[j].off + r[j].len && r[j].off < r[i].off + r[i].len) return false;
    }
    return true;
}

constexpr Region kHostLocal{0, 16384, "call-local read-backs (read_status, reductions, <x,y>, chain_check, ...)"};
constexpr Region kHostTruncDev{16384, 16384, "truncating rounds: (d - 1) x 16 orthonormality deviations"};
constexpr Region kHostDotOnes{32768, 16, "dot_two_ended: the unit boundary environments (upload source)"};
constexpr Region kHostRangeAmax{32784, 8, "range_controlled: max |A|, read behind the factorisation's own wait"};
constexpr Region kHostShardLayout{32800, 16320, "shard_layout: world x d mode-size table (<= 2040 doubles)"};
constexpr Region kHostChainStatus{49152, 3072, "chain_pass: factorisation statuses (<= 64 edges x 3 jobs x 4 words)"};
constexpr Region kHostTruncStatus{53248, 4096, "round_truncate: the 1024 status words of a sweep"};
constexpr Region kHostRangeProbe{57600, 7680, "probe_core_ranges: one norm per core (<= 960)"};
constexpr Region kHostMap[] = {kHostLocal,       kHostTruncDev,    kHostDotOnes,     kHostRangeAmax,
                               kHostShardLayout, kHostChainStatus, kHostTruncStatus, kHostRangeProbe};
static_assert(disjoint_within(kHostMap, 0, kBytes), "pinned scratch regions overlap or leave the allocation");
constexpr Region kHostGeneralStatus{kHostChainStatus.off, 8192, "round_general: 2048 status words"};
static_assert(kHostGeneralStatus.off + kHostGeneralStatus.len == kHostTruncStatus.off + kHostTruncStatus.len);

constexpr Region kHostResult{0, 64, "a scalar result or up to 16 status words"};
constexpr Region kHostOrthEmax{64, 64, "orthogonalize: the 8 partial maxima of its first-order pass"};
constexpr Region kHostIdentityDev{256, 8, "max_abs_dev_identity"};
constexpr Region kHostAmax{384, 8, "range_exponent: max |A|"};
constexpr Region kHostLocalSlots[] = {kHostResult, kHostOrthEmax, kHostIdentityDev, kHostAmax};
static_assert(disjoint_within(kHostLocalSlots, kHostLocal.off, kHostLocal.off + kHostLocal.len));
constexpr Region kHostChainDev{512, 8192, "chain_check: (d - 1) x 16 orthonormality deviations"};
constexpr Region kHostSvdCheck{640, 40, "svd_bidiag: residuals (4 doubles) and the multisection status"};
static_assert(kHostChainDev.off + kHostChainDev.len <= kHostLocal.len && kHostSvdCheck.off + kHostSvdCheck.len <= kHostLocal.len);

constexpr Region kDevResult{0, 8, "reduce_to_host: the reduced scalar"};
constexpr Region kDevIdentityDev{256, 8, "max_abs_dev_identity"};
constexpr Region kDevOrthEmax{320, 64, "orthogonalize: the 8 partial maxima of its first-order pass"};
constexpr Region kDevAmax{384, 8, "range_exponent: max |A|"};
constexpr Region kDevRangeAmax{392, 8, "range_controlled: max |A|"};
constexpr Region kDevPartials{512, 24576, "reduce_to_device: 3 x 1024 partial sums"};
constexpr Region kDevRangeProbe{32768, 7680, "probe_core_ranges: one norm per core (<= 960)"};
constexpr Region kDevMap[] = {kDevResult, kDevIdentityDev, kDevOrthEmax, kDevAmax, kDevRangeAmax, kDevPartials, kDevRangeProbe};
static_assert(disjoint_within(kDevMap, 0, kBytes), "device scratch regions overlap or leave the allocation");

template <class T>
T* at(void* base, const Region& r, size_t count) {
    XRS_REQUIRE(count * sizeof(T) <= r.len, std::string("scratch region too small -- ") + r.owner);
    return reinterpret_cast<T*>(static_cast<char*>(base) + r.off);
}
template <class T>
T* host(xrs_handle_t h, const Region& r, size_t count = 1) { return at<T>(h->host_scratch, r, count); }
template <class T>
T* dev(xrs_handle_t h, const Region& r, size_t count = 1) { return at<T>(h->dev_scratch, r, count); }

}
}
```

xerus_amd/csrc/tt.hip:

```cpp
#include <algorithm>
#include <atomic>
#include <chrono>
#include <condition_variable>
#include <limits>
#include <mutex>
#include <thread>
#include <cstdio>
#include <cstdlib>
#include <cmath>
#include <string>
#include <vector>

#include "tt_common.hpp"

namespace xrs {

namespace ttd {


std::vector<size_t> maximal_ranks(const TT& t) {
    std::vector<size_t> rk(t.r + 1, t.r + t.d);
    size_t cur = 1;
    for (size_t i = 0; i + 1 < t.d; ++i) {
        cur *= t.n[i];
        if (cur < rk[i]) rk[i] = cur;
        else cur = rk[i];
    }
    cur = 1;
    for (size_t i = 1; i < t.d; ++i) {
        cur *= t.n[t.d - i];
        if (cur < rk[t.d - i - 1]) rk[t.d - i - 1] = cur;
        else cur = rk[t.d - i - 1];
    }
    return rk;
}

bool exceeds_maximal_ranks(const TT& t) {
    const auto mx = maximal_ranks(t);
    for (size_t i = 0; i + 1 < t.d; ++i)
        if (t.r[i + 1] != mx[i]) return true;
    return false;
}

void transfer_right(TT& t, size_t k, bool rank_reduce) {
    const size_t m = t.rows_left(k), nn = t.r[k + 1], kmax = std::min(m, nn);
    double* Q = t.alloc(m * kmax);
    double* C = t.alloc(kmax * nn);
    size_t rank = kmax;
    if (rank_reduce) rank = qc(t.h, t.core[k], m, nn, Q, C);
    else qr(t.h, t.core[k], m, nn, Q, C);
    const size_t ncols = t.cols_right(k + 1);
    double* nxt = t.alloc(rank * ncols);
    gemm(t.h, nxt, rank, ncols, 1.0, C, nn, false, nn, t.core[k + 1], ncols, false);
    t.release(C);
    t.replace(k, Q);
    t.replace(k + 1, nxt);
    t.r[k + 1] = rank;
}

void transfer_left(TT& t, size_t k, bool rank_reduce) {
    const size_t m = t.r[k], nn = t.cols_right(k), kmax = std::min(m, nn);
    double* C = t.alloc(m * kmax);
    double* Q = t.alloc(kmax * nn);
    size_t rank = kmax;
    if (rank_reduce) rank = cq(t.h, t.core[k], m, nn, C, Q);
    else rq(t.h, t.core[k], m, nn, C, Q);
    const size_t prow = t.rows_left(k - 1);
    double* prv = t.alloc(prow * rank);
    gemm(t.h, prv, prow, rank, 1.0, t.core[k - 1], m, false, m, C, rank, false);
    t.release(C);
    t.replace(k, Q);
    t.replace(k - 1, prv);
    t.r[k] = rank;
}

void move_core(TT& t, bool canonicalized, size_t core_pos, size_t pos, bool keep_rank) {
    const size_t d = t.d;
    if (canonicalized) {
        for (size_t k = core_pos; k < pos; ++k) transfer_right(t, k, !keep_rank);
        for (size_t k = core_pos; k > pos; --k) transfer_left(t, k, !keep_rank);
    } else {
        for (size_t k = 0; k < pos; ++k) transfer_right(t, k, !keep_rank);
        for (size_t k = d - 1; k > pos; --k) transfer_left(t, k, !keep_rank);
    }
    while (exceeds_maximal_ranks(t)) {
        for (size_t k = pos; k > 0; --k) transfer_left(t, k, !keep_rank);
        for (size_t k = 0; k + 1 < d; ++k) transfer_right(t, k, !keep_rank);
        for (size_t k = d - 1; k > pos; --k) transfer_left(t, k, !keep_rank);
    }
}

void orth_right(TT& t, size_t k) { transfer_right(t, k, true); }

size_t svd_cut(const std::vector<double>& s, size_t max_rank, double eps) {
    size_t rank = s.size();
    if (max_rank != 0) rank = std::min(rank, max_rank);
    for (size_t j = 1; j < rank; ++j)
        if (s[j] <= eps * s[0]) return j;
    return rank;
}

__global__ void k_soft_cols(double* __restrict__ T, const double* __restrict__ S, size_t rows, size_t cols, double soft) {
    for (size_t e = size_t(blockIdx.x) * blockDim.x + threadIdx.x; e < rows * cols; e += size_t(gridDim.x) * blockDim.x) {
        const double s = S[e % cols];
        T[e] = s > 0.0 ? T[e] * (fmax(0.0, s - soft) / s) : 0.0;
    }
}

void truncate_edge(TT& t, size_t k, size_t max_rank, double eps, double soft) {
    const size_t m = t.r[k], nn = t.cols_right(k);
    const size_t prow = t.rows_left(k - 1);
    xrs_handle_t h = t.h;
    const bool wide = m <= nn;
    const size_t g = wide ? m : nn;
    XRS_REQUIRE(g <= kHugeMax, "TT round: an edge whose unfoldings both exceed 1024 is not supported");
    double* Q = t.alloc(m * nn);
    double* F = t.alloc(g * g);
    const OrthResult o = orthogonalize(h, t.core[k], m, nn, wide, Q, F);
    if (wide && o.certified && eps < 0.5 * o.cert_ratio && max_rank >= m && !(soft > 0.0)) {
        double* prv = t.alloc(prow * m);
        gemm(h, prv, prow, m, 1.0, t.core[k - 1], m, false, m, F, m, false);
        t.release(F);
        t.replace(k, Q);
        t.replace(k - 1, prv);
        return;
    }
    DevBuf S(h, g * 8), Vt(h, g * g * 8), st(h, 64);
    XRS_HIP(hipMemsetAsync(st.d(), 0, 64, h->stream));
    jacobi_right_vectors(h, F, int(g), wide, S.d(), Vt.d(), st.as<int>(), 60);
    jacobi_settle(h, st.as<int>(), int(g), int(g), [&](int kernel) {
        jacobi_vt(h, F, int(g), false, int(g), int(g), S.d(), Vt.d(), int(g), st.as<int>(), 60, kernel);
    });
    std::vector<double> s(g);
    XRS_HIP(hipMemcpyAsync(s.data(), S.d(), g * 8, hipMemcpyDeviceToHost, h->stream));
    host_wait(h);
    const size_t kk = svd_cut(s, max_rank, eps);
    double* T = t.alloc(m * kk);
    if (wide) gemm(h, T, m, kk, 1.0, F, g, false, g, Vt.d(), g, true);
    else gemm(h, T, m, kk, 1.0, t.core[k], nn, false, nn, Vt.d(), g, true);
    if (soft > 0.0) {
        hipLaunchKernelGGL(k_soft_cols, dim3(unsigned(std::min<size_t>((m * kk + 255) / 256, 4096))), dim3(256), 0, h->stream, T, S.d(), m, kk,
                           soft);
        check_launch("k_soft_cols");
    }
    double* cur = t.alloc(kk * nn);
    if (wide) gemm(h, cur, kk, nn, 1.0, Vt.d(), g, false, g, Q, nn, false);
    else XRS_HIP(hipMemcpyAsync(cur, Vt.d(), kk * nn * 8, hipMemcpyDeviceToDevice, h->stream));
    double* prv = t.alloc(prow * kk);
    gemm(h, prv, prow, kk, 1.0, t.core[k - 1], m, false, m, T, kk, false);
    t.release(T);
    t.release(F);
    t.release(Q);
    t.replace(k, cur);
    t.replace(k - 1, prv);
    t.r[k] = kk;
}


void left_gram_step(TT& t, std::vector<double*>& G, double* T, size_t k, bool do_reduce) {
    xrs_handle_t h = t.h;
    if (k == 0) {
        gemm_sym(h, G[1], t.r[1], 1.0, t.core[0], t.r[1], true, t.rows_left(0), t.core[0], t.r[1], false);
        if (do_reduce) t.reduce(G[1], t.r[1] * t.r[1]);
        return;
    }
    const size_t a = t.r[k], b = t.r[k + 1], cols = t.cols_right(k);
    gemm(h, T, a, cols, 1.0, G[k], a, false, a, t.core[k], cols, false);
    gemm_sym(h, G[k + 1], b, 1.0, t.core[k], b, true, a * t.n[k], T, b, false);
    if (do_reduce) t.reduce(G[k + 1], b * b);
}

void right_gram_step(TT& t, std::vector<double*>& H, double* T, size_t k, bool do_reduce) {
    xrs_handle_t h = t.h;
    const size_t last = t.d - 1;
    if (k == last) {
        const size_t cl = t.cols_right(last);
        gemm_sym(h, H[last], t.r[last], 1.0, t.core[last], cl, false, cl, t.core[last], cl, true);
        if (do_reduce) t.reduce(H[last], t.r[last] * t.r[last]);
        return;
    }
    const size_t a = t.r[k], b = t.r[k + 1], cols = t.cols_right(k);
    gemm(h, T, a * t.n[k], b, 1.0, t.core[k], b, false, b, H[k + 1], b, false);
    gemm_sym(h, H[k], a, 1.0, t.core[k], cols, false, cols, T, cols, true);
    if (do_reduce) t.reduce(H[k], a * a);
}

void gram_chains(TT& t, std::vector<double*>& G, std::vector<double*>& H, std::vector<DevBuf>& store, bool left) {
    const size_t d = t.d;
    xrs_handle_t h = t.h;
    G.assign(d, nullptr);
    H.assign(d, nullptr);
    size_t tmax = 1;
    for (size_t k = 1; k + 1 < d; ++k) tmax = std::max(tmax, t.size(k));
    DevBuf TL(h, tmax * 8), TR(h, tmax * 8);
    if (t.sharded()) {
        for (size_t s = 0; s + 1 < d; ++s) {
            const size_t kl = s + 1, kr = d - 1 - s;
            const size_t nl = left ? t.r[kl] * t.r[kl] : 0, nr = t.r[kr] * t.r[kr];
            store.emplace_back(h, (nl + nr) * 8);
            double* base = store.back().d();
            if (left) G[kl] = base;
            H[kr] = base + nl;
            if (left) {
                StreamFork fork(h);
                fork.side();
                left_gram_step(t, G, TL.d(), s, false);
                fork.main();
                right_gram_step(t, H, TR.d(), kr, false);
                fork.join();
            } else {
                right_gram_step(t, H, TR.d(), kr, false);
            }
            t.reduce(base, nl + nr);
        }
        return;
    }
    for (size_t k = 1; k < d; ++k) {
        if (left) {
            store.emplace_back(h, t.r[k] * t.r[k] * 8);
            G[k] = store.back().d();
        }
        store.emplace_back(h, t.r[k] * t.r[k] * 8);
        H[k] = store.back().d();
    }
    if (!left) {
        for (size_t k = d - 1; k >= 1; --k) right_gram_step(t, H, TR.d(), k);
        return;
    }
    StreamFork fork(h);
    for (size_t s = 0; s + 1 < d; ++s) {
        fork.side();
        left_gram_step(t, G, TL.d(), s);
        fork.main();
        right_gram_step(t, H, TR.d(), d - 1 - s);
    }
    fork.join();
}

struct HostMarks {
    bool on = stamps_enabled("round");
    std::chrono::steady_clock::time_point t0 = std::chrono::steady_clock::now();
    std::string line;
    void mark(const char* what) {
        if (!on) return;
        const double us = std::chrono::duration<double, std::micro>(std::chrono::steady_clock::now() - t0).count();
        char buf[64];
        std::snprintf(buf, sizeof(buf), " %s %.0f", what, us);
        line += buf;
    }
    ~HostMarks();
};
HostMarks* g_marks = nullptr;
HostMarks::~HostMarks() {
    if (g_marks == this) g_marks = nullptr;
    if (on) std::fprintf(stderr, "[round host us]%s\n", line.c_str());
}
#define XRS_MARK(what) do { if (g_marks) g_marks->mark(what); } while (0)


__global__ void __launch_bounds__(256) k_dev_identity_many(const DevIdArgs args) {
    const double* G = args.G[blockIdx.x];
    const int n = args.n[blockIdx.x];
    __shared__ double red[4];
    double mx = 0.0;
    for (int e = threadIdx.x + 256 * blockIdx.y; e < n * n; e += 256 * gridDim.y) {
        const double v = fabs(G[e] - ((e / n) == (e % n) ? 1.0 : 0.0));
        mx = (v > mx || v != v) ? v : mx;
    }
#pragma unroll
    for (int o = 32; o > 0; o >>= 1) {
        const double q = __shfl_xor(mx, o, 64);
        mx = (q > mx || q != q) ? q : mx;
    }
    if ((threadIdx.x & 63) == 0) red[threadIdx.x >> 6] = mx;
    __syncthreads();
    if (threadIdx.x == 0) {
        double m = red[0];
        for (int i = 1; i < 4; ++i) m = (red[i] > m || red[i] != red[i]) ? red[i] : m;
        args.out[blockIdx.x * gridDim.y + blockIdx.y] = m;
    }
}

void rl_sweep(TT& t, const size_t* max_ranks, double eps, double cX, size_t from);


void gemm_grouped(xrs_handle_t h, const std::vector<GemmJob>& jobs) {
    std::vector<bool> done(jobs.size(), false);
    for (size_t i = 0; i < jobs.size(); ++i) {
        if (done[i]) continue;
        const GemmJob& g = jobs[i];
        std::vector<const double*> A, B;
        std::vector<double*> C;
        for (size_t j = i; j < jobs.size(); ++j) {
            const GemmJob& o = jobs[j];
            if (done[j] || o.M != g.M || o.N != g.N || o.K != g.K || o.lda != g.lda || o.ldb != g.ldb || o.ta != g.ta ||
                o.tb != g.tb || o.sym != g.sym || o.alpha != g.alpha || o.tri != g.tri)
                continue;
            done[j] = true;
            A.push_back(o.A);
            B.push_back(o.B);
            C.push_back(o.C);
        }
        if (C.size() == 1 && g.sym) gemm_sym(h, C[0], g.N, g.alpha, A[0], g.lda, g.ta, g.K, B[0], g.ldb, g.tb);
        else if (C.size() == 1) gemm(h, C[0], g.M, g.N, g.alpha, A[0], g.lda, g.ta, g.K, B[0], g.ldb, g.tb, g.tri);
        else gemm_batched(h, int(C.size()), C.data(), g.M, g.N, g.alpha, A.data(), g.lda, g.ta, g.K, B.data(), g.ldb,
                          g.tb, g.sym, g.tri);
    }
}

struct ChainPass {
    std::vector<double*> C;
    int* status = nullptr;
    int count = 0;
};

void chain_pass(TT& t, bool certify, ChainPass& out) {
    const size_t d = t.d;
    xrs_handle_t h = t.h;
    std::vector<double*> G, H;
    std::vector<DevBuf> gram_store, Lf(d);
    XRS_MARK("pass");
    gram_chains(t, G, H, gram_store, certify);
    open_dot_gate(h);
    XRS_MARK("chains");
    std::vector<DevBuf> Z(d), Cs;
    for (size_t k = 1; k < d; ++k) Z[k] = DevBuf(h, t.r[k] * t.r[k] * 8);
    std::vector<CholJob> jobs;
    for (size_t k = 1; k < d; ++k) {
        const size_t a = t.r[k];
        Lf[k] = DevBuf(h, a * a * 8);
        jobs.push_back({H[k], int(a), Lf[k].d(), Z[k].d()});
        if (certify) {
            jobs.push_back(CholJob::certificate(G[k], int(a), kGramShift));
            jobs.push_back(CholJob::certificate(H[k], int(a), kGramShift));
        }
    }
    const int cnt = chol_status_count(jobs);
    int* host_status = scratch::host<int>(h, scratch::kHostChainStatus, size_t(cnt));
    DevBuf st(h, size_t(cnt) * 4 + 64);
    chol_enqueue(h, jobs, st.as<int>(), Cs);
    XRS_HIP(hipMemcpyAsync(host_status, st.d(), size_t(cnt) * 4, hipMemcpyDeviceToHost, h->stream));
    XRS_MARK("potrf");
    out.status = host_status;
    out.count = cnt;
    out.C.assign(d, nullptr);
    std::vector<DevBuf> W(d);
    for (size_t k = 0; k < d; ++k) {
        out.C[k] = t.alloc(t.size(k));
        if (k > 0 && k + 1 < d) W[k] = DevBuf(h, t.size(k) * 8);
    }
    std::vector<GemmJob> right, left;
    for (size_t k = 0; k + 1 < d; ++k) {
        const size_t b = t.r[k + 1];
        right.push_back({t.rows_left(k), b, b, b, b, false, false, t.core[k], Lf[k + 1].d(), k == 0 ? out.C[k] : W[k].d()});
        right.back().tri = b <= 256 ? kTriB : 0;
    }
    for (size_t k = 1; k < d; ++k) {
        const size_t a = t.r[k], cols = t.cols_right(k);
        left.push_back({a, cols, a, a, cols, false, false, Z[k].d(), k + 1 < d ? W[k].d() : t.core[k], out.C[k]});
        left.back().tri = a <= 256 ? kTriA : 0;
    }
    gemm_grouped(h, right);
    gemm_grouped(h, left);
    XRS_MARK("transforms");
}

bool chain_status_ok(const ChainPass& p) {
    static const bool dbg = std::getenv("XRS_DEBUG_ROUND") != nullptr;
    for (int i = 0; i < p.count; ++i)
        if (p.status[i] != 0) {
            if (dbg) std::fprintf(stderr, "chain_pass: status word %d of %d is %d (a factorisation failed)\n", i, p.count, p.status[i]);
            return false;
        }
    return true;
}

double chain_check(TT& t, const std::vector<double*>& C) {
    const size_t d = t.d;
    xrs_handle_t h = t.h;
    XRS_MARK("check");
    std::vector<double*> Gr(d, nullptr);
    DevIdArgs da{};
    DevBuf dev(h, d * 16 * 8 + 64);
    int nchk = 0;
    size_t gtot = 0;
    for (size_t k = 1; k < d; ++k) gtot += t.r[k] * t.r[k];
    DevBuf Gall(h, gtot * 8);
    for (size_t k = 1, off = 0; k < d; off += t.r[k] * t.r[k], ++k) Gr[k] = Gall.d() + off;
    std::vector<GemmJob> grams;
    for (size_t k = 1; k < d; ++k) {
        const size_t a = t.r[k], cols = t.cols_right(k);
        grams.push_back({a, a, cols, cols, cols, false, true, C[k], C[k], Gr[k], true});
    }
    gemm_grouped(h, grams);
    t.reduce(Gall.d(), gtot);
    for (size_t k = 1; k < d; ++k) {
        da.G[nchk] = Gr[k];
        da.n[nchk] = int(t.r[k]);
        ++nchk;
    }
    da.out = dev.d();
    constexpr int kSlices = 16;
    hipLaunchKernelGGL(k_dev_identity_many, dim3(nchk, kSlices), dim3(256), 0, h->stream, da);
    check_launch("k_dev_identity_many");
    double* hd = scratch::host<double>(h, scratch::kHostChainDev, size_t(nchk) * kSlices);
    XRS_HIP(hipMemcpyAsync(hd, dev.d(), size_t(nchk) * kSlices * 8, hipMemcpyDeviceToHost, h->stream));
    XRS_MARK("enq");
    host_wait(h);
    XRS_MARK("sync");
    double worst = 0.0;
    for (int i = 0; i < nchk * kSlices; ++i) worst = (hd[i] > worst || hd[i] != hd[i]) ? hd[i] : worst;
    return worst;
}

bool round_chain(TT& t, const size_t* max_ranks, double eps) {
    const size_t d = t.d;
    static const bool dbg = std::getenv("XRS_DEBUG_ROUND") != nullptr;
    if (d < 2 || d > 65 || (!t.sharded() && exceeds_maximal_ranks(t))) return false;
    for (size_t k = 1; k < d; ++k)
        if (t.r[k] > max_ranks[k - 1] || t.r[k] > kHugeMax) return false;
    const double cX = 0.5 * std::sqrt(kGramShift);
    if (!(eps < 0.25 * cX * cX)) return false;
    HostMarks marks;
    g_marks = marks.on ? &marks : nullptr;
    ChainPass p1;
    chain_pass(t, true, p1);
    double dev = chain_check(t, p1.C);
    if (!chain_status_ok(p1)) {
        for (size_t k = 0; k < d; ++k) t.release(p1.C[k]);
        { g_marks = nullptr; return false; }
    }
    std::vector<double*> C = p1.C;
    if (!(dev <= kOrthTol)) {
        if (dbg) std::fprintf(stderr, "round_chain: pass 1 orthogonality %.3e, second pass\n", dev);
        TT t2 = t;
        t2.core = C.data();
        ChainPass p2;
        chain_pass(t2, false, p2);
        const double dev2 = chain_check(t2, p2.C);
        const bool ok2 = chain_status_ok(p2);
        if (dbg) std::fprintf(stderr, "round_chain: pass 2 orthogonality %.3e (factors %s)\n", dev2, ok2 ? "ok" : "failed");
        if (ok2 && dev2 <= kOrthTol) {
            for (size_t k = 0; k < d; ++k) t.release(C[k]);
            C = p2.C;
            dev = dev2;
        } else {
            for (size_t k = 0; k < d; ++k) t.release(p2.C[k]);
        }
    }
    const bool ok = dev <= kOrthTol;
    if (!ok && t.sharded()) {
        for (size_t k = 0; k < d; ++k) t.release(C[k]);
        { g_marks = nullptr; return false; }
    }
    for (size_t k = 0; k < d; ++k) t.replace(k, C[k]);
    if (!ok) rl_sweep(t, max_ranks, eps, cX, d - 1);
    g_marks = nullptr;
    return true;
}

bool reorthonormalize(TT& t) {
    ChainPass p;
    chain_pass(t, false, p);
    const double dev = chain_check(t, p.C);
    const bool ok = chain_status_ok(p) && dev <= kOrthTol;
    for (size_t k = 0; k < t.d; ++k) {
        if (ok) t.replace(k, p.C[k]);
        else t.release(p.C[k]);
    }
    return ok;
}

void rl_sweep(TT& t, const size_t* max_ranks, double eps, double cX, size_t from) {
    for (size_t k = from; k >= 1; --k) {
        const size_t m = t.r[k], nn = t.cols_right(k), prow = t.rows_left(k - 1);
        double* Q = t.alloc(m * nn);
        double* L = t.alloc(m * m);
        const OrthResult o = orthogonalize(t.h, t.core[k], m, nn, true, Q, L);
        const double c = o.certified ? cX * o.cert_ratio : 0.0;
        if (!(m <= nn && c > 16.0 * 2.220446049250313e-16 && eps < 0.5 * c)) {
            t.release(Q);
            t.release(L);
            for (size_t j = 0; j < k; ++j) orth_right(t, j);
            for (size_t kk = k; kk >= 1; --kk) truncate_edge(t, kk, max_ranks[kk - 1], eps);
            return;
        }
        double* prv = t.alloc(prow * m);
        gemm(t.h, prv, prow, m, 1.0, t.core[k - 1], m, false, m, L, m, false);
        t.release(L);
        t.replace(k, Q);
        t.replace(k - 1, prv);
    }
}

constexpr size_t kProbeMax = std::min(scratch::kHostRangeProbe.len, scratch::kDevRangeProbe.len) / 8;

void probe_core_ranges(TT& t) {
    t.range_probed = false;
    if (t.sharded() || t.d > kProbeMax) return;
    xrs_handle_t h = t.h;
    std::vector<const double*> x(t.core, t.core + t.d);
    std::vector<size_t> n(t.d);
    for (size_t k = 0; k < t.d; ++k) n[k] = t.size(k);
    double* dev = scratch::dev<double>(h, scratch::kDevRangeProbe, t.d);
    norms_enqueue(h, x.data(), n.data(), int(t.d), dev);
    XRS_HIP(hipMemcpyAsync(scratch::host<double>(h, scratch::kHostRangeProbe, t.d), dev, t.d * 8, hipMemcpyDeviceToHost, h->stream));
    t.range_probed = true;
}

static bool core_exponents(const TT& t, std::vector<int>& ex) {
    const double* am = scratch::host<double>(t.h, scratch::kHostRangeProbe, t.d);
    ex.assign(t.d, 0);
    long prefix = 0, lo = 0, hi = 0;
    for (size_t k = 0; k < t.d; ++k) {
        const size_t rank = std::max(std::min(t.rows_left(k), t.r[k + 1]), std::min(t.r[k], t.cols_right(k)));
        if (am[k] > 0.0 && std::isfinite(am[k])) {
            int e2 = 0;
            const double mant = std::frexp(am[k], &e2);
            ex[k] = e2 + std::ilogb(mant / std::sqrt(double(rank)));
        }
        prefix += ex[k];
        lo = std::min(lo, prefix);
        hi = std::max(hi, prefix);
    }
    return hi - lo > 200;
}

bool core_range_exceeded(const TT& t) {
    if (!t.range_probed) return false;
    std::vector<int> ex;
    return core_exponents(t, ex);
}

static void round_ranged(TT& t, bool canonicalized, size_t core_pos, const size_t* max_ranks, double eps, bool probe);

void round(TT& t, bool canonicalized, size_t core_pos, const size_t* max_ranks, double eps) {
    round_ranged(t, canonicalized, core_pos, max_ranks, eps, true);
}

static void round_ranged(TT& t, bool canonicalized, size_t core_pos, const size_t* max_ranks, double eps, bool probe) {
    const size_t d = t.d;
    t.h->last_round_path = XRS_ROUND_CHAIN;
    if (round_chain(t, max_ranks, eps)) return;
    t.range_probed = t.range_hit = false;
    if (probe && d >= 2) probe_core_ranges(t);
    t.h->last_round_path = XRS_ROUND_TRUNCATE;
    if (round_truncate(t, max_ranks, eps)) return;
    static const bool no_general = std::getenv("XRS_NO_GENERAL_ROUND") != nullptr;
    t.h->last_round_path = XRS_ROUND_GENERAL;
    if (!t.range_hit && !no_general && round_general(t, max_ranks, eps)) return;
    if (t.range_probed && !t.range_hit) {
        host_wait(t.h);
        t.range_hit = core_range_exceeded(t);
    }
    if (t.range_hit) {
        std::vector<int> ex;
        probe_core_ranges(t);
        host_wait(t.h);
        core_exponents(t, ex);
        t.range_probed = t.range_hit = false;
        long total = 0;
        for (size_t k = 0; k < d; ++k) {
            if (ex[k] == 0) continue;
            double* c = t.alloc(t.size(k));
            ldexp_copy(t.h, c, t.core[k], -ex[k], t.size(k));
            t.replace(k, c);
            total += ex[k];
        }
        round_ranged(t, canonicalized, core_pos, max_ranks, eps, false);
        ldexp_copy(t.h, t.core[0], t.core[0], int(std::max(-4000L, std::min(4000L, total))), t.size(0));
        return;
    }
    t.range_probed = false;
    t.h->last_round_path = XRS_ROUND_REFERENCE;
    const size_t start = canonicalized ? core_pos : 0;
    for (size_t k = start; k + 1 < d; ++k) orth_right(t, k);
    for (size_t k = d - 1; k >= 1; --k) truncate_edge(t, k, max_ranks[k - 1], eps);
}

void soft_threshold(TT& t, bool canonicalized, size_t core_pos, const double* taus) {
    const size_t d = t.d;
    t.h->last_round_path = XRS_ROUND_REFERENCE;
    const size_t start = canonicalized ? core_pos : 0;
    for (size_t k = start; k + 1 < d; ++k) orth_right(t, k);
    for (size_t i = 0; i + 1 < d; ++i) truncate_edge(t, d - 1 - i, std::numeric_limits<size_t>::max(), 0.0, taus[i]);
}

double dot_two_ended(xrs_handle_t h, size_t d, const size_t* n, const size_t* rx, const double* const* X, const size_t* ry,
                     const double* const* Y, const TT* shard = nullptr) {
    const size_t m = d / 2;
    size_t emax = 1, tmax = 1;
    for (size_t k = 0; k <= d; ++k) emax = std::max(emax, rx[k] * ry[k]);
    for (size_t k = 0; k < d; ++k) tmax = std::max(tmax, std::max(ry[k] * n[k] * rx[k + 1], rx[k] * n[k] * ry[k + 1]));
    DevBuf P0(h, 2 * emax * 8), P1(h, 2 * emax * 8), TL(h, tmax * 8), TR(h, tmax * 8);
    const bool unit_l = rx[0] == 1 && ry[0] == 1, unit_r = rx[d] == 1 && ry[d] == 1;
    bool self = true;
    for (size_t k = 0; k < d && self; ++k) self = X[k] == Y[k] && rx[k + 1] == ry[k + 1];
    auto second = [&](const GemmSpec& g) {
        if (self) gemm_sym(h, g.C, g.M, 1.0, g.A, g.lda, g.ta, g.K, g.B, g.ldb, g.tb);
        else gemm(h, g);
    };
    if (!unit_l || !unit_r) {
        double* ones = scratch::host<double>(h, scratch::kHostDotOnes, 2);
        ones[0] = ones[1] = 1.0;
        XRS_HIP(hipMemcpyAsync(P0.d(), &ones[0], 8, hipMemcpyHostToDevice, h->stream));
        XRS_HIP(hipMemcpyAsync(P0.d() + emax, &ones[1], 8, hipMemcpyHostToDevice, h->stream));
    }
    struct EndStep {
        bool on = false, first = false;
        GemmSpec g1{}, g2{};
    };
    const size_t steps = std::max(m, d - m);
    auto plan = [&](size_t s, double* E, double* F, double* nb, EndStep& L, EndStep& R, size_t& ne) {
        L = EndStep{};
        R = EndStep{};
        ne = 0;
        if (s < m) {
            const size_t k = s, a = rx[k], b = ry[k], nk = n[k], a2 = rx[k + 1], b2 = ry[k + 1];
            L.on = true;
            L.first = !(s == 0 && unit_l);
            const double* T = L.first ? TL.d() : X[k];
            L.g1 = GemmSpec{E, X[k], TL.d(), b, nk * a2, a, b, nk * a2, true, false};
            L.g2 = GemmSpec{T, Y[k], nb, a2, b2, b * nk, a2, b2, true, false};
            ne = a2 * b2;
        }
        if (s < d - m) {
            const size_t k = d - 1 - s, a = rx[k], b = ry[k], nk = n[k], a2 = rx[k + 1], b2 = ry[k + 1];
            R.on = true;
            R.first = !(s == 0 && unit_r);
            const double* T = R.first ? TR.d() : X[k];
            R.g1 = GemmSpec{X[k], F, TR.d(), a * nk, b2, a2, a2, b2, false, false};
            R.g2 = GemmSpec{T, Y[k], nb + (shard ? ne : emax), a, b, nk * b2, nk * b2, nk * b2, false, true};
        }
    };
    double *E = P0.d(), *F = P0.d() + emax;
    double* nextbuf = P1.d();
    double* curbuf = P0.d();
    {
        StreamFork fork(h);
        for (size_t s = 0; s < steps; ++s) {
            EndStep L, R;
            size_t ne;
            plan(s, E, F, nextbuf, L, R, ne);
            if (L.on) {
                if (!shard) fork.side();
                if (L.first) gemm(h, L.g1);
                second(L.g2);
            }
            if (R.on) {
                if (!shard) fork.main();
                if (R.first) gemm(h, R.g1);
                second(R.g2);
            }
            if (shard) shard->reduce(nextbuf, ne + (R.on ? R.g2.M * R.g2.N : 0));
            if (L.on) E = L.g2.C;
            if (R.on) F = R.g2.C;
            std::swap(curbuf, nextbuf);
        }
        fork.join();
    }
    return reduce_to_host(h, 1, E, F, rx[m] * ry[m]);
}

double dot(xrs_handle_t h, size_t d, const size_t* n, const size_t* rx, const double* const* X, const size_t* ry,
           const double* const* Y, const TT* shard = nullptr) {
    size_t emax = 1, tmax = 1;
    for (size_t k = 0; k < d; ++k) {
        emax = std::max(emax, rx[k + 1] * ry[k + 1]);
        tmax = std::max(tmax, ry[k] * n[k] * rx[k + 1]);
    }
    if (d >= 4) return dot_two_ended(h, d, n, rx, X, ry, Y, shard);
    DevBuf E0(h, emax * 8), E1(h, emax * 8), T(h, tmax * 8);
    const double one = 1.0;
    XRS_HIP(hipMemcpyAsync(E0.d(), &one, 8, hipMemcpyHostToDevice, h->stream));
    double* E = E0.d();
    double* En = E1.d();
    for (size_t k = 0; k < d; ++k) {
        const size_t a = rx[k], b = ry[k], nk = n[k], a2 = rx[k + 1], b2 = ry[k + 1];
        gemm(h, T.d(), b, nk * a2, 1.0, E, b, true, a, X[k], nk * a2, false);
        gemm(h, En, a2, b2, 1.0, T.d(), a2, true, b * nk, Y[k], b2, false);
        if (shard) shard->reduce(En, a2 * b2);
        std::swap(E, En);
    }
    double* hs = scratch::host<double>(h, scratch::kHostResult);
    XRS_HIP(hipMemcpyAsync(hs, E, 8, hipMemcpyDeviceToHost, h->stream));
    host_wait(h);
    return hs[0];
}

}

class DotWorker {
   public:
    explicit DotWorker(xrs_handle_t parent) : child_(create_child_handle(parent)), th_([this] { run(); }) {}
    ~DotWorker() {
        {
            std::lock_guard<std::mutex> g(m_);
            quit_ = true;
            state_.store(kPosted, std::memory_order_release);
            gate_.store(1, std::memory_order_release);
        }
        cv_.notify_all();
        th_.join();
        (void)xrs_destroy(child_);
    }
    xrs_handle_t child() const { return child_; }
    void post(size_t d, const size_t* n, const size_t* rx, const double* const* X, const size_t* ry,
              const double* const* Y, bool gated) {
        gate_ev_ = nullptr;
        gate_.store(gated ? 0 : 1, std::memory_order_release);
        d_ = d;
        n_.assign(n, n + d);
        rx_.assign(rx, rx + d + 1);
        ry_.assign(ry, ry + d + 1);
        X_.assign(X, X + d);
        Y_.assign(Y, Y + d);
        err_code_ = 0;
        {
            std::lock_guard<std::mutex> g(m_);
            state_.store(kPosted, std::memory_order_release);
        }
        cv_.notify_all();
    }
    void open_gate(hipEvent_t ev) {
        if (gate_.load(std::memory_order_acquire) != 0) return;
        gate_ev_ = ev;
        {
            std::lock_guard<std::mutex> g(m_);
            gate_.store(1, std::memory_order_release);
        }
        cv_.notify_all();
    }
    bool gate_closed() const { return gate_.load(std::memory_order_acquire) == 0; }
    void wait_done() {
        open_gate(nullptr);
        for (int i = 0; i < (1 << 16) && state_.load(std::memory_order_acquire) != kDone; ++i) __builtin_ia32_pause();
        if (state_.load(std::memory_order_acquire) != kDone) {
            std::unique_lock<std::mutex> g(m_);
            cv_.wait(g, [&] { return state_.load(std::memory_order_acquire) == kDone; });
        }
    }
    double take() {
        wait_done();
        state_.store(kIdle, std::memory_order_release);
        if (err_code_ != 0) throw Error{err_code_, err_msg_};
        return value_;
    }

   private:
    static constexpr int kIdle = 0, kPosted = 1, kDone = 2;
    void run() {
        (void)hipSetDevice(child_->device);
        for (;;) {
            for (int i = 0; i < (1 << 18) && state_.load(std::memory_order_acquire) != kPosted; ++i) __builtin_ia32_pause();
            if (state_.load(std::memory_order_acquire) != kPosted) {
                std::unique_lock<std::mutex> g(m_);
                cv_.wait(g, [&] { return state_.load(std::memory_order_acquire) == kPosted; });
            }
            if (quit_) return;
            for (int i = 0; i < (1 << 18) && gate_.load(std::memory_order_acquire) == 0; ++i) __builtin_ia32_pause();
            if (gate_.load(std::memory_order_acquire) == 0) {
                std::unique_lock<std::mutex> g(m_);
                cv_.wait(g, [&] { return gate_.load(std::memory_order_acquire) != 0 || quit_; });
            }
            if (quit_) return;
            try {
                if (gate_ev_ != nullptr) {
                    XRS_HIP(hipStreamWaitEvent(child_->stream, gate_ev_, 0));
                    XRS_HIP(hipStreamWaitEvent(child_->side_stream[0], gate_ev_, 0));
                }
                value_ = ttd::dot(child_, d_, n_.data(), rx_.data(), X_.data(), ry_.data(), Y_.data());
            } catch (const Error& e) {
                err_code_ = e.code;
                err_msg_ = e.msg;
            } catch (const std::exception& e) {
                err_code_ = XRS_EINVAL;
                err_msg_ = e.what();
            }
            {
                std::lock_guard<std::mutex> g(m_);
                state_.store(kDone, std::memory_order_release);
            }
            cv_.notify_all();
        }
    }
    xrs_handle_t child_;
    size_t d_ = 0;
    std::vector<size_t> n_, rx_, ry_;
    std::vector<const double*> X_, Y_;
    double value_ = 0.0;
    int err_code_ = 0;
    std::string err_msg_;
    bool quit_ = false;
    std::atomic<int> state_{kIdle};
    std::atomic<int> gate_{1};
    hipEvent_t gate_ev_ = nullptr;
    std::mutex m_;
    std::condition_variable cv_;
    std::thread th_;
};

void dot_async(xrs_handle_t h, size_t d, const size_t* n, const size_t* rx, const double* const* X, const size_t* ry,
               const double* const* Y) {
    XRS_REQUIRE(!h->dot_pending, "an asynchronous inner product is already in flight on this handle");
    if (h->dot_worker == nullptr) h->dot_worker = new DotWorker(h);
    xrs_handle_t c = h->dot_worker->child();
    c->prof_mask = h->prof_mask;
    static const bool gate = [] {
        const char* e = std::getenv("XRS_DOT_GATE");
        return !(e && e[0] == '0');
    }();
    if (!gate) {
        XRS_HIP(hipEventRecord(h->ev_dot, h->stream));
        XRS_HIP(hipStreamWaitEvent(c->stream, h->ev_dot, 0));
        XRS_HIP(hipStreamWaitEvent(c->side_stream[0], h->ev_dot, 0));
    }
    h->dot_worker->post(d, n, rx, X, ry, Y, gate);
    h->dot_pending = true;
    h->reader_pending = true;
}

void open_dot_gate(xrs_handle_t h) {
    if (!h->dot_pending || h->dot_worker == nullptr || !h->dot_worker->gate_closed()) return;
    XRS_HIP(hipEventRecord(h->ev_dot_join, h->stream));
    h->dot_worker->open_gate(h->ev_dot_join);
}

double dot_wait(xrs_handle_t h) {
    XRS_REQUIRE(h->dot_pending, "no asynchronous inner product in flight on this handle");
    open_dot_gate(h);
    h->dot_pending = false;
    h->reader_pending = false;
    return h->dot_worker->take();
}

xrs_handle_t dot_child(xrs_handle_t h) { return h->dot_worker ? h->dot_worker->child() : nullptr; }

namespace ttd {

void check_tt(size_t d, const size_t* n, const size_t* r, double* const* cores) {
    XRS_REQUIRE(d >= 1, "TT must have at least one component");
    XRS_REQUIRE(n && r && cores, "null TT description");
    XRS_REQUIRE(r[0] == 1 && r[d] == 1, "boundary ranks must be 1");
    for (size_t k = 0; k < d; ++k) {
        XRS_REQUIRE(n[k] > 0 && r[k + 1] > 0, "dimensions and ranks must be positive");
        XRS_REQUIRE(cores[k] != nullptr, "null core");
    }
}

}

using namespace ttd;

void wait_dot_done(xrs_handle_t h) {
    if (!h->dot_pending || h->dot_worker == nullptr) return;
    open_dot_gate(h);
    h->dot_worker->wait_done();
}

void destroy_dot_worker(xrs_handle_t h) {
    if (h->dot_worker == nullptr) return;
    if (h->dot_pending) {
        try {
            open_dot_gate(h);
            (void)h->dot_worker->take();
        } catch (...) {
        }
        h->dot_pending = false;
    }
    delete h->dot_worker;
    h->dot_worker = nullptr;
}

namespace tt {
void move_core(xrs_handle_t h, size_t d, const size_t* n, size_t* r, double** cores, bool canonicalized, size_t core_pos,
               size_t pos, bool keep_rank) {
    check_tt(d, n, r, cores);
    TT t{h, d, n, r, cores};
    xrs::move_core(t, canonicalized, core_pos, pos, keep_rank);
}
void round(xrs_handle_t h, size_t d, const size_t* n, size_t* r, double** cores, bool canonicalized, size_t core_pos,
           const size_t* max_ranks, double eps) {
    check_tt(d, n, r, cores);
    TT t{h, d, n, r, cores};
    xrs::round(t, canonicalized, core_pos, max_ranks, eps);
}
double dot(xrs_handle_t h, size_t d, const size_t* n, const size_t* rx, const double* const* X, const size_t* ry,
           const double* const* Y) {
    return xrs::dot(h, d, n, rx, X, ry, Y);
}
void soft_threshold(xrs_handle_t h, size_t d, const size_t* n, size_t* r, double** cores, bool canonicalized, size_t core_pos,
                    const double* taus) {
    check_tt(d, n, r, cores);
    TT t{h, d, n, r, cores};
    xrs::soft_threshold(t, canonicalized, core_pos, taus);
}
}

}

using namespace xrs;

extern "C" {

int xrs_tt_move_core(xrs_handle_t h, size_t d, const size_t* n, size_t* r, double** cores, int canonicalized,
                     size_t core_position, size_t position, int keep_rank) {
    return guarded([&] {
        XRS_REQUIRE(h, "null handle");
        check_tt(d, n, r, cores);
        XRS_REQUIRE(position < d, "Illegal core-position");
        XRS_REQUIRE(!canonicalized || core_position < d, "Illegal current core position");
        TT t{h, d, n, r, cores};
        move_core(t, canonicalized != 0, core_position, position, keep_rank != 0);
    });
}

int xrs_tt_round(xrs_handle_t h, size_t d, const size_t* n, size_t* r, double** cores, int canonicalized,
                 size_t core_position, const size_t* max_ranks, double eps) {
    return guarded([&] {
        XRS_REQUIRE(h, "null handle");
        check_tt(d, n, r, cores);
        XRS_REQUIRE(eps < 1.0 && eps >= 0.0, "_eps must be smaller than one.");
        for (size_t k = 0; k + 1 < d; ++k)
            XRS_REQUIRE(max_ranks[k] > 0, "Trying to round a TTTensor to rank 0 is not possible.");
        XRS_REQUIRE(!canonicalized || core_position < d, "Illegal current core position");
        TT t{h, d, n, r, cores};
        round(t, canonicalized != 0, core_position, max_ranks, eps);
    });
}

int xrs_tt_soft_threshold(xrs_handle_t h, size_t d, const size_t* n, size_t* r, double** cores, int canonicalized,
                          size_t core_position, const double* taus) {
    return guarded([&] {
        XRS_REQUIRE(h && (d < 2 || taus), "null argument");
        check_tt(d, n, r, cores);
        XRS_REQUIRE(!canonicalized || core_position < d, "Illegal current core position");
        for (size_t k = 0; k + 1 < d; ++k) XRS_REQUIRE(taus[k] >= 0.0, "soft threshold must not be negative");
        TT t{h, d, n, r, cores};
        soft_threshold(t, canonicalized != 0, core_position, taus);
    });
}

int xrs_tt_round_sharded(xrs_handle_t h, size_t d, const size_t* n_local, size_t* r, double** cores,
                         const size_t* max_ranks, double eps, xrs_allreduce_fn allreduce, void* ctx, int* certified) {
    return guarded([&] {
        XRS_REQUIRE(h && certified, "null argument");
        XRS_REQUIRE(d >= 2 && n_local && r && cores, "null TT description");
        XRS_REQUIRE(r[0] == 1 && r[d] == 1, "boundary ranks must be 1");
        XRS_REQUIRE(eps < 1.0 && eps >= 0.0, "_eps must be smaller than one.");
        for (size_t k = 0; k + 1 < d; ++k)
            XRS_REQUIRE(max_ranks[k] > 0, "Trying to round a TTTensor to rank 0 is not possible.");
        TT t{h, d, n_local, r, cores};
        t.shard_mode = true;
        t.ar = allreduce;
        t.ar_ctx = ctx;
        *certified = (round_chain(t, max_ranks, eps) || round_truncate(t, max_ranks, eps)) ? 1 : 0;
    });
}

int xrs_tt_round_sharded_ex(xrs_handle_t h, size_t d, const size_t* n_local, size_t* r, double** cores,
                            const size_t* max_ranks, double eps, int world, int rank, xrs_allreduce_fn allreduce,
                            void* ctx, int* path) {
    return guarded([&] {
        XRS_REQUIRE(h && path, "null argument");
        XRS_REQUIRE(d >= 2 && n_local && r && cores && max_ranks, "null TT description");
        XRS_REQUIRE(r[0] == 1 && r[d] == 1, "boundary ranks must be 1");
        XRS_REQUIRE(world >= 1 && rank >= 0 && rank < world, "world / rank out of range");
        XRS_REQUIRE(size_t(world) * d <= 2040, "world * d above 2040");
        XRS_REQUIRE(eps < 1.0 && eps >= 0.0, "_eps must be smaller than one.");
        for (size_t k = 0; k + 1 < d; ++k)
            XRS_REQUIRE(max_ranks[k] > 0, "Trying to round a TTTensor to rank 0 is not possible.");
        TT t{h, d, n_local, r, cores};
        t.shard_mode = true;
        t.ar = allreduce;
        t.ar_ctx = ctx;
        t.world = world;
        t.rank = rank;
        static const bool no_general = std::getenv("XRS_NO_GENERAL_ROUND") != nullptr;
        *path = 0;
        if (round_chain(t, max_ranks, eps)) *path = XRS_ROUND_CHAIN;
        else if (round_truncate(t, max_ranks, eps)) *path = XRS_ROUND_TRUNCATE;
        else if (!no_general && round_general(t, max_ranks, eps)) *path = XRS_ROUND_GENERAL;
        if (*path) h->last_round_path = *path;
    });
}

int xrs_tt_dot_sharded(xrs_handle_t h, double* result, size_t d, const size_t* n_local, const size_t* rx,
                       const double* const* X, const size_t* ry, const double* const* Y, xrs_allreduce_fn allreduce,
                       void* ctx) {
    return guarded([&] {
        XRS_REQUIRE(h && result, "null argument");
        XRS_REQUIRE(d >= 1 && n_local && rx && ry && X && Y, "null TT description");
        check_tt(d, n_local, rx, const_cast<double* const*>(X));
        check_tt(d, n_local, ry, const_cast<double* const*>(Y));
        TT t{h, d, n_local, const_cast<size_t*>(rx), const_cast<double**>(X)};
        t.shard_mode = true;
        t.ar = allreduce;
        t.ar_ctx = ctx;
        *result = dot(h, d, n_local, rx, X, ry, Y, &t);
    });
}

int xrs_tt_last_round_path(xrs_handle_t h) { return h ? h->last_round_path : -1; }

int xrs_tt_dot(xrs_handle_t h, double* result, size_t d, const size_t* n, const size_t* rx, const double* const* X,
               const size_t* ry, const double* const* Y) {
    return guarded([&] {
        XRS_REQUIRE(h && result, "null argument");
        check_tt(d, n, rx, const_cast<double* const*>(X));
        check_tt(d, n, ry, const_cast<double* const*>(Y));
        *result = dot(h, d, n, rx, X, ry, Y);
    });
}

int xrs_tt_dot_async(xrs_handle_t h, size_t d, const size_t* n, const size_t* rx, const double* const* X,
                     const size_t* ry, const double* const* Y) {
    return guarded([&] {
        XRS_REQUIRE(h, "null handle");
        check_tt(d, n, rx, const_cast<double* const*>(X));
        check_tt(d, n, ry, const_cast<double* const*>(Y));
        XRS_REQUIRE(d >= 2, "the asynchronous inner product needs at least two components");
        dot_async(h, d, n, rx, X, ry, Y);
    });
}

int xrs_tt_dot_wait(xrs_handle_t h, double* result) {
    return guarded([&] {
        XRS_REQUIRE(h && result, "null argument");
        *result = dot_wait(h);
    });
}

}
```

Before: 36150 GFLOP/s.

## Add ragged grouped GEMM launch and merge chain status/deviation readbacks

Singleton GEMM jobs of differing shapes in a group, when they fit the small-tile path, are now packed into one ragged kernel launch whose blocks look up their job from a prefix table of tile offsets. This replaces one launch per job. The Cholesky status words and orthogonality-deviation results of a chain pass now share one device buffer and are copied to the host in a single transfer instead of two. The change also exposes grouped-GEMM and batched-Cholesky C APIs, and it adds a linear job search per block plus more complex split-K slab indexing.

```diff
diff --git a/include/xerus_amd.h b/include/xerus_amd.h
--- a/include/xerus_amd.h
+++ b/include/xerus_amd.h
@@ -46,6 +46,19 @@
 int xrs_gemm_batched(xrs_handle_t handle, size_t count, double* const* C, size_t M, size_t N, double alpha,
                      const double* const* A, size_t lda, int transA, size_t K,
                      const double* const* B, size_t ldb, int transB);
+
+typedef struct xrs_gemm_job {
+    double* C;
+    const double* A;
+    const double* B;
+    size_t M, N, K, lda, ldb;
+    int transA, transB, sym;
+    double alpha;
+} xrs_gemm_job;
+int xrs_gemm_grouped(xrs_handle_t handle, size_t count, const xrs_gemm_job* jobs);
+
+int xrs_chol_batched(xrs_handle_t handle, size_t count, const double* const* A, const int* n, double* const* L,
+                     double* const* Z, const double* shift, int* status);
 
 int xrs_gemm_sym(xrs_handle_t handle, double* C, size_t N, double alpha,
                  const double* A, size_t lda, int transA, size_t K,
diff --git a/xerus_amd/capi.py b/xerus_amd/capi.py
--- a/xerus_amd/capi.py
+++ b/xerus_amd/capi.py
@@ -38,6 +38,9 @@
     "xrs_gemm_sym": (C.c_int,[_DP, _DP, _SZ, C.c_double, _DP, _SZ, C.c_int, _SZ, _DP, _SZ, C.c_int]),
     "xrs_gemm_batched": (C.c_int, [_DP, _SZ, C.POINTER(_DP), _SZ, _SZ, C.c_double, C.POINTER(_DP), _SZ, C.c_int, _SZ,
                                    C.POINTER(_DP), _SZ, C.c_int]),
+    "xrs_gemm_grouped": (C.c_int, [_DP, _SZ, _DP]),
+    "xrs_chol_batched": (C.c_int, [_DP, _SZ, C.POINTER(_DP), C.POINTER(C.c_int), C.POINTER(_DP), C.POINTER(_DP),
+                                   C.POINTER(C.c_double), C.POINTER(C.c_int)]),
     "xrs_permute": (C.c_int, [_DP, _DP, _DP, _SZ, C.POINTER(_SZ), C.POINTER(_SZ)]),
     "xrs_qc": (C.c_int, [_DP, _DP, _DP, C.POINTER(_SZ), _DP, _SZ, _SZ]),
     "xrs_cq": (C.c_int, [_DP, _DP, _DP, C.POINTER(_SZ), _DP, _SZ, _SZ]),
@@ -113,6 +116,11 @@
 _lib = None
 
 
+class GemmJobStruct(C.Structure):
+    _fields_ = [("C", _DP), ("A", _DP), ("B", _DP), ("M", _SZ), ("N", _SZ), ("K", _SZ), ("lda", _SZ), ("ldb", _SZ),
+                ("transA", C.c_int), ("transB", C.c_int), ("sym", C.c_int), ("alpha", C.c_double)]
+
+
 class XrsError(RuntimeError):
 
     def __init__(self, fn: str, code: int, msg: str):
@@ -216,6 +224,30 @@
         tab = lambda xs: (_DP * max(1, cnt))(*[_DP(x.ptr) for x in xs])
         _check("xrs_gemm_batched", self.lib.xrs_gemm_batched(self.h, cnt, tab(Cs), M, N, alpha, tab(As), lda, int(transA),
                                                             K, tab(Bs), ldb, int(transB)))
+
+    def gemm_grouped(self, jobs):
+        tab = (GemmJobStruct * max(1, len(jobs)))()
+        for t, j in zip(tab, jobs):
+            ta, tb = bool(j.get("transA", False)), bool(j.get("transB", False))
+            t.C, t.A, t.B = j["C"].ptr, j["A"].ptr, j["B"].ptr
+            t.M, t.N, t.K = j["M"], j["N"], j["K"]
+            t.lda = j.get("lda", j["M"] if ta else j["K"])
+            t.ldb = j.get("ldb", j["K"] if tb else j["N"])
+            t.transA, t.transB, t.sym = int(ta), int(tb), int(bool(j.get("sym", False)))
+            t.alpha = float(j.get("alpha", 1.0))
+        _check("xrs_gemm_grouped", self.lib.xrs_gemm_grouped(self.h, len(jobs), C.cast(tab, _DP)))
+
+    def chol_batched(self, mats, shift=0.0, inverse=True, factor=True):
+        cnt = len(mats)
+        ns = [int(a.shape[0]) for a in mats]
+        Ls = [self.empty((n, n)) for n in ns] if factor else None
+        Zs = [self.empty((n, n)) for n in ns] if factor and inverse else None
+        tab = lambda xs: (_DP * max(1, cnt))(*[_DP(x.ptr) for x in xs]) if xs is not None else None
+        status = (C.c_int * max(1, cnt))()
+        shifts = (C.c_double * max(1, cnt))(*([float(shift)] * cnt))
+        _check("xrs_chol_batched", self.lib.xrs_chol_batched(self.h, cnt, tab(mats), (C.c_int * max(1, cnt))(*ns), tab(Ls),
+                                                            tab(Zs), shifts, status))
+        return Ls, Zs, np.array(status[:cnt], dtype=np.int32)
 
     def tangent_to_tt(self, n, r, Us, Vs, add_base: bool):
         d = len(n)
diff --git a/xerus_amd/csrc/chol_batch.hip b/xerus_amd/csrc/chol_batch.hip
--- a/xerus_amd/csrc/chol_batch.hip
+++ b/xerus_amd/csrc/chol_batch.hip
@@ -275,3 +275,53 @@
 }
 
 }
+
+extern "C" int xrs_chol_batched(xrs_handle_t h, size_t count, const double* const* A, const int* n, double* const* L,
+                                double* const* Z, const double* shift, int* status) {
+    using namespace xrs;
+    return guarded([&] {
+        XRS_REQUIRE(h, "null handle");
+        XRS_REQUIRE(count == 0 || (A && n && status), "null argument");
+        XRS_REQUIRE(count < (1u << 16), "too many jobs");
+        std::vector<CholJob> jobs;
+        for (size_t i = 0; i < count; ++i) {
+            XRS_REQUIRE(A[i] && n[i] >= 1, "empty job");
+            double* Li = L ? L[i] : nullptr;
+            double* Zi = Z ? Z[i] : nullptr;
+            XRS_REQUIRE(Li || !Zi, "an inverse needs its factor");
+            XRS_REQUIRE(Li != A[i], "L must not alias A");
+            jobs.push_back({A[i], n[i], Li, Zi, shift ? shift[i] : 0.0});
+        }
+        if (count == 0) return;
+        fence_readers(h);
+        const int words = chol_status_count(jobs);
+        DevBuf st(h, size_t(words) * 4 + 64);
+        std::vector<DevBuf> keep;
+        chol_enqueue(h, jobs, st.as<int>(), keep);
+        std::vector<int> host(size_t(words), 0);
+        read_status(h, st.as<int>(), words, host.data());
+        int small = 0, big = 0;
+        for (const CholJob& j : jobs) {
+            small += j.n <= 256;
+            big += j.n > 256 && j.n <= 512;
+        }
+        int s_idx = 0, b_idx = 0, h_slot = small + 2 * big;
+        for (size_t i = 0; i < count; ++i) {
+            const int ni = jobs[i].n;
+            status[i] = 0;
+            if (ni <= 256) {
+                status[i] = host[size_t(s_idx++)];
+            } else if (ni <= 512) {
+                const int part0 = b_idx / kBigMax * kBigMax, in_part = std::min(kBigMax, big - part0), j = b_idx - part0;
+                const int w0 = host[size_t(small + 2 * part0 + j)], w1 = host[size_t(small + 2 * part0 + in_part + j)];
+                status[i] = w0 ? w0 : w1;
+                ++b_idx;
+            } else {
+                const int w = chol_full_blocks(size_t(ni));
+                for (int q = 0; q < w; ++q)
+                    if (status[i] == 0) status[i] = host[size_t(h_slot + q)];
+                h_slot += w;
+            }
+        }
+    });
+}
diff --git a/xerus_amd/csrc/elementwise.hpp b/xerus_amd/csrc/elementwise.hpp
--- a/xerus_amd/csrc/elementwise.hpp
+++ b/xerus_amd/csrc/elementwise.hpp
@@ -31,6 +31,14 @@
 void gemm_batched(xrs_handle_t h, int count, double* const* C, size_t M, size_t N, double alpha, const double* const* A,
                   size_t lda, bool ta, size_t K, const double* const* B, size_t ldb, bool tb, bool sym = false,
                   int tri = 0);
+struct GemmRaggedJob {
+    const double* A;
+    const double* B;
+    double* C;
+    size_t M, N, K, lda, ldb;
+};
+void gemm_ragged(xrs_handle_t h, int count, const GemmRaggedJob* jobs, double alpha, bool ta, bool tb, bool sym);
+bool gemm_small_tile(size_t M, size_t N, size_t K, const double* A, size_t lda, const double* B, size_t ldb, bool sym);
 void gemm_sym(xrs_handle_t h, double* C, size_t N, double alpha, const double* A, size_t lda, bool ta, size_t K,
               const double* B, size_t ldb, bool tb);
 
diff --git a/xerus_amd/csrc/gemm.hip b/xerus_amd/csrc/gemm.hip
--- a/xerus_amd/csrc/gemm.hip
+++ b/xerus_amd/csrc/gemm.hip
@@ -14,6 +14,7 @@
 typedef double d4 __attribute__((ext_vector_type(4)));
 
 struct GemmOne {
+    static constexpr bool ragged = false;
     const double* A;
     const double* B;
     double* C;
@@ -22,9 +23,25 @@
     __device__ double* c(int) const { return C; }
 };
 struct GemmMany {
+    static constexpr bool ragged = false;
     const double* A[kGemmBatchMax];
     const double* B[kGemmBatchMax];
     double* C[kGemmBatchMax];
+    __host__ __device__ const double* a(int i) const { return A[i]; }
+    __host__ __device__ const double* b(int i) const { return B[i]; }
+    __device__ double* c(int i) const { return C[i]; }
+};
+struct GemmRagged {
+    static constexpr bool ragged = true;
+    const double* A[kGemmBatchMax];
+    const double* B[kGemmBatchMax];
+    double* C[kGemmBatchMax];
+    size_t lda[kGemmBatchMax], ldb[kGemmBatchMax];
+    size_t slab0[kGemmBatchMax];
+    int M[kGemmBatchMax], N[kGemmBatchMax], K[kGemmBatchMax];
+    int kps[kGemmBatchMax];
+    int tile0[kGemmBatchMax + 1];
+    int count;
     __host__ __device__ const double* a(int i) const { return A[i]; }
     __host__ __device__ const double* b(int i) const { return B[i]; }
     __device__ double* c(int i) const { return C[i]; }
@@ -79,11 +96,9 @@
 template <int TM, int TN, int WGM, int WGN, int WGK, int NACC, class PTR>
 __device__ __forceinline__ void gemm_finish(d4 (&acc2)[NACC][TM][TN], double* lds, const PTR& ptrs, int M, int N,
                                             double alpha, double* __restrict__ slab, int* __restrict__ tickets,
-                                            int sym, int m0, int n0, int wm, int wn, int kg, int pos, int xb, int yb, int zb) {
-    const int bz = yb;
-    double* __restrict__ C = ptrs.c(bz);
-    const int zslice = bz * int(gridDim.z) + zb;
-    const int tslot = bz * int(gridDim.x) + xb;
+                                            int sym, int m0, int n0, int wm, int wn, int kg, int pos, int tslot, int yb,
+                                            int zb, int nsplit) {
+    double* __restrict__ C = ptrs.c(yb);
     const int tid = threadIdx.x;
     const int lane = tid & 63;
     const bool mirror = sym != 0;
@@ -121,7 +136,7 @@
     }
     const bool to_slab = slab != nullptr;
     const size_t MN = size_t(M) * size_t(N);
-    double* out = to_slab ? slab + size_t(zslice) * MN : C;
+    double* out = to_slab ? slab + size_t(zb) * MN : C;
     const double scale = to_slab ? 1.0 : alpha;
     const int lc = lane & 15, lg = lane >> 4;
     if (kg == 0) {
@@ -153,7 +168,7 @@
     double* flag = lds;
     if (tid == 0) {
         const int t = __hip_atomic_fetch_add(&tickets[tslot], 1, __ATOMIC_RELAXED, __HIP_MEMORY_SCOPE_AGENT);
-        const bool last = (t == int(gridDim.z) - 1);
+        const bool last = (t == nsplit - 1);
         if (last) __hip_atomic_store(&tickets[tslot], 0, __ATOMIC_RELAXED, __HIP_MEMORY_SCOPE_AGENT);
         flag[0] = last ? 1.0 : 0.0;
     }
@@ -170,10 +185,9 @@
                 if (row < M && col < N && (!mirror || row >= col)) {
                     const size_t o = size_t(row) * N + col;
                     double sum = 0.0;
-                    for (int z = 0; z < int(gridDim.z); ++z)
+                    for (int z = 0; z < nsplit; ++z)
                         sum += (z == zb) ? acc[i][j][r]
-                                                      : __hip_atomic_load(&slab[(size_t(bz) * gridDim.z + z) * MN + o], __ATOMIC_RELAXED,
-                                                                          __HIP_MEMORY_SCOPE_AGENT);
+                                         : __hip_atomic_load(&slab[size_t(z) * MN + o], __ATOMIC_RELAXED, __HIP_MEMORY_SCOPE_AGENT);
                     C[o] = alpha * sum;
                     if (mirror) C[size_t(col) * N + row] = alpha * sum;
                 }
@@ -186,7 +200,24 @@
 __device__ __forceinline__ void gemm_body(const PTR& ptrs, size_t lda, size_t ldb, int M, int N, int K, int kps,
                                           double alpha, double* __restrict__ slab, int tiles_m, int xcd_group,
                                           int* __restrict__ tickets, int sym) {
-    const int bz = blockIdx.y;
+    int bz = blockIdx.y;
+    int xb = blockIdx.x;
+    int nsplit = gridDim.z;
+    if constexpr (PTR::ragged) {
+        int e = 0;
+        while (e + 1 < ptrs.count && xb >= ptrs.tile0[e + 1]) ++e;
+        bz = e;
+        xb -= ptrs.tile0[e];
+        M = ptrs.M[e], N = ptrs.N[e], K = ptrs.K[e], kps = ptrs.kps[e];
+        lda = ptrs.lda[e], ldb = ptrs.ldb[e];
+        nsplit = (K + kps - 1) / kps;
+        if (int(blockIdx.z) >= nsplit) return;
+        slab = nsplit > 1 ? slab + ptrs.slab0[e] : nullptr;
+        tickets = nsplit > 1 ? tickets : nullptr;
+        tiles_m = (M + BM - 1) / BM;
+    } else if (slab != nullptr) {
+        slab += size_t(bz) * gridDim.z * (size_t(M) * size_t(N));
+    }
     const double* __restrict__ A = ptrs.a(bz);
     const double* __restrict__ B = ptrs.b(bz);
     constexpr int NT = WGM * WGN * WGK * 64;
@@ -215,7 +246,17 @@
     static_assert(WGK == 1 || (WGK - 1) * BM * BN <= 2 * GBK * (SA + SB), "LDS reduction buffer too small");
 
     int tm, tn;
-    {
+    if constexpr (PTR::ragged) {
+        if (sym) {
+            tm = int((__builtin_sqrtf(8.0f * float(xb) + 1.0f) - 1.0f) * 0.5f);
+            while ((tm + 1) * (tm + 2) / 2 <= xb) ++tm;
+            while (tm * (tm + 1) / 2 > xb) --tm;
+            tn = xb - tm * (tm + 1) / 2;
+        } else {
+            tm = xb % tiles_m;
+            tn = xb / tiles_m;
+        }
+    } else {
         const int b = blockIdx.x, tiles_n = gridDim.x / tiles_m;
         if (xcd_group == 1) {
             const int xcd = b & 7, slot = b >> 3;
@@ -347,8 +388,9 @@
         }
     }
 
+    const int tslot = PTR::ragged ? int(blockIdx.x) : bz * int(gridDim.x) + xb;
     gemm_finish<TM, TN, WGM, WGN, WGK, NACC>(acc2, &As[0][0], ptrs, M, N, alpha, slab, tickets, sym, m0, n0, wm, wn, kg, pos,
-                                             int(blockIdx.x), int(blockIdx.y), int(blockIdx.z));
+                                             tslot, bz, int(blockIdx.z), nsplit);
 }
 
 constexpr int kGldsBK = 32;
@@ -552,7 +594,9 @@
         }
     }
     __syncthreads();
-    gemm_finish<TM, TN, WGM, WGN, WGK, NACC>(acc2, lds, ptrs, M, N, alpha, slab, tickets, sym, m0, n0, wm, wn, kg, pos, xb, bz, zb);
+    double* slab_e = slab != nullptr ? slab + size_t(bz) * gridDim.z * (size_t(M) * size_t(N)) : nullptr;
+    gemm_finish<TM, TN, WGM, WGN, WGK, NACC>(acc2, lds, ptrs, M, N, alpha, slab_e, tickets, sym, m0, n0, wm, wn, kg, pos,
+                                             bz * int(gridDim.x) + xb, bz, zb, int(gridDim.z));
 }
 
 template <int BM, int BN, int WGM, int WGN, int WGK, bool TA, bool TB, class PTR, int BK = kGldsBK, int ST = 0>
@@ -705,25 +749,26 @@
     check_launch("k_gemm_glds");
 }
 
-template <class PTR>
-static bool gemm_glds(xrs_handle_t h, const PTR& P, int count, int M, int N, int K, double alpha, size_t lda, bool ta,
-                      size_t ldb, bool tb, bool sym, int tri) {
+static const std::pair<int, int>& glds_env() {
     static const std::pair<int, int> g_env = [] {
         int v = -1, t = 256;
         if (const char* e = std::getenv("XRS_GEMM_GLDS")) std::sscanf(e, "%d,%d", &v, &t);
         return std::make_pair(v, t);
     }();
-    const int g_var = g_env.first, g_target = g_env.second;
-    static const int g_st2 = [] {
-        const char* e = std::getenv("XRS_GLDS_ST2");
-        return e ? std::atoi(e) : 7;
-    }();
-    if (g_var == 0) return false;
-    if (K % kGldsBK != 0 || (lda & 1) || (ldb & 1)) return false;
+    return g_env;
+}
+constexpr int kGldsBm[12] = {0, 64, 80, 64, 64, 32, 64, 80, 64, 80, 64, 64},
+              kGldsBn[12] = {0, 80, 64, 64, 64, 32, 80, 64, 80, 64, 64, 64};
+
+template <class PTR>
+static int glds_variant(const PTR& P, int count, int M, int N, int K, size_t lda, size_t ldb, bool sym) {
+    const int g_var = glds_env().first;
+    if (g_var == 0) return 0;
+    if (K % kGldsBK != 0 || (lda & 1) || (ldb & 1)) return 0;
     for (int i = 0; i < count; ++i)
-        if ((reinterpret_cast<uintptr_t>(P.a(i)) & 15) || (reinterpret_cast<uintptr_t>(P.b(i)) & 15)) return false;
-    const int bms[12] = {0, 64, 80, 64, 64, 32, 64, 80, 64, 80, 64, 64},
-              bns[12] = {0, 80, 64, 64, 64, 32, 80, 64, 80, 64, 64, 64};
+        if ((reinterpret_cast<uintptr_t>(P.a(i)) & 15) || (reinterpret_cast<uintptr_t>(P.b(i)) & 15)) return 0;
+    const int* bms = kGldsBm;
+    const int* bns = kGldsBn;
     auto fits = [&](int v) { return M % bms[v] == 0 && N % bns[v] == 0 && (!sym || bms[v] == bns[v]); };
     auto ntiles = [&](int v) {
         const long tm = M / bms[v], tn = N / bns[v];
@@ -739,9 +784,28 @@
         else if (fits(7) && ntiles(7) >= 192) var = 7;
         else if (fits(4)) var = 4;
         else if (fits(5)) var = 5;
-        if (var == 0) return false;
-    }
-    if (var < 1 || var > 11 || !fits(var)) return false;
+        if (var == 0) return 0;
+    }
+    if (var < 1 || var > 11 || !fits(var)) return 0;
+    return var;
+}
+
+template <class PTR>
+static bool gemm_glds(xrs_handle_t h, const PTR& P, int count, int M, int N, int K, double alpha, size_t lda, bool ta,
+                      size_t ldb, bool tb, bool sym, int tri) {
+    const int g_target = glds_env().second;
+    static const int g_st2 = [] {
+        const char* e = std::getenv("XRS_GLDS_ST2");
+        return e ? std::atoi(e) : 7;
+    }();
+    const int var = glds_variant(P, count, M, N, K, lda, ldb, sym);
+    if (var == 0) return false;
+    const int* bms = kGldsBm;
+    const int* bns = kGldsBn;
+    auto ntiles = [&](int v) {
+        const long tm = M / bms[v], tn = N / bns[v];
+        return sym ? long(count) * tm * (tm + 1) / 2 : long(count) * tm * tn;
+    };
     const int bk = kGldsBK;
     const long tiles = ntiles(var);
     const int ksteps = K / bk;
@@ -786,21 +850,24 @@
     return true;
 }
 
-template <class PTR>
-static void gemm_impl(xrs_handle_t h, const PTR& P, int count, size_t Ms, size_t Ns, double alpha, size_t lda, bool ta,
-                      size_t Ks, size_t ldb, bool tb, bool sym = false, int tri = 0) {
-    const int M = int(Ms), N = int(Ns), K = int(Ks);
-    if (gemm_glds(h, P, count, M, N, K, alpha, lda, ta, ldb, tb, sym, tri)) return;
-    struct Cfg { int var = 0, kmin = 256, target = 512; };
-    static const Cfg g_cfg = [] {
-        Cfg c;
+struct GemmCfg { int var = 0, kmin = 256, target = 512; };
+static const GemmCfg& gemm_cfg() {
+    static const GemmCfg g_cfg = [] {
+        GemmCfg c;
         if (const char* e = std::getenv("XRS_GEMM_CFG")) std::sscanf(e, "%d,%d,%d", &c.var, &c.kmin, &c.target);
         return c;
     }();
+    return g_cfg;
+}
+constexpr int kGenBm[16] = {0, 128, 64, 64, 32, 64, 64, 64, 64, 32, 32, 32, 32, 64, 64, 80},
+              kGenBn[16] = {0, 128, 64, 32, 32, 32, 64, 64, 32, 32, 32, 32, 32, 32, 80, 64};
+
+static int general_variant(int count, int M, int N, int K, bool sym, long& target_eff) {
+    const GemmCfg& g_cfg = gemm_cfg();
     const int cfg_var = g_cfg.var, cfg_kmin = g_cfg.kmin, cfg_target = g_cfg.target;
     auto ntiles = [&](int bm, int bn) { return long(count) * ((M + bm - 1) / bm) * ((N + bn - 1) / bn); };
-    const int bms[16] = {0, 128, 64, 64, 32, 64, 64, 64, 64, 32, 32, 32, 32, 64, 64, 80},
-              bns[16] = {0, 128, 64, 32, 32, 32, 64, 64, 32, 32, 32, 32, 32, 32, 80, 64};
+    const int* bms = kGenBm;
+    const int* bns = kGenBn;
     int var = cfg_var;
     long cfg_target_eff = cfg_target;
     if (sym) cfg_target_eff = 160;
@@ -831,6 +898,21 @@
             }
         }
     }
+    target_eff = cfg_target_eff;
+    return var;
+}
+
+template <class PTR>
+static void gemm_impl(xrs_handle_t h, const PTR& P, int count, size_t Ms, size_t Ns, double alpha, size_t lda, bool ta,
+                      size_t Ks, size_t ldb, bool tb, bool sym = false, int tri = 0) {
+    const int M = int(Ms), N = int(Ns), K = int(Ks);
+    if (gemm_glds(h, P, count, M, N, K, alpha, lda, ta, ldb, tb, sym, tri)) return;
+    const int cfg_kmin = gemm_cfg().kmin;
+    long cfg_target_eff = 0;
+    int var = general_variant(count, M, N, K, sym, cfg_target_eff);
+    const int* bms = kGenBm;
+    const int* bns = kGenBn;
+    auto ntiles = [&](int bm, int bn) { return long(count) * ((M + bm - 1) / bm) * ((N + bn - 1) / bn); };
     const long tiles = sym ? long(count) * ((M + bms[var] - 1) / bms[var]) * ((M + bms[var] - 1) / bms[var] + 1) / 2
                            : ntiles(bms[var], bns[var]);
     int splits = 1;
@@ -914,6 +996,75 @@
     }
 }
 
+bool gemm_small_tile(size_t Ms, size_t Ns, size_t Ks, const double* A, size_t lda, const double* B, size_t ldb, bool sym) {
+    if (Ms == 0 || Ns == 0 || Ks == 0 || Ms >= (1u << 30) || Ns >= (1u << 30) || Ks >= (1u << 30)) return false;
+    const int M = int(Ms), N = int(Ns), K = int(Ks);
+    if (glds_variant(GemmOne{A, B, nullptr}, 1, M, N, K, lda, ldb, sym) != 0) return false;
+    long target = 0;
+    return general_variant(1, M, N, K, sym, target) == 4;
+}
+
+static void launch_ragged(xrs_handle_t h, const GemmRaggedJob* jobs, int count, double alpha, bool ta, bool tb, bool sym) {
+    constexpr int BT = 32, BK = 16;
+    constexpr int kCUs = 256, kSliceMin = 128, kSliceMax = 8;
+    GemmRagged P{};
+    long total = 0;
+    for (int e = 0; e < count; ++e) {
+        const GemmRaggedJob& g = jobs[e];
+        const long tm = long(g.M + BT - 1) / BT, tn = long(g.N + BT - 1) / BT;
+        P.A[e] = g.A, P.B[e] = g.B, P.C[e] = g.C;
+        P.M[e] = int(g.M), P.N[e] = int(g.N), P.K[e] = int(g.K);
+        P.lda[e] = g.lda, P.ldb[e] = g.ldb;
+        P.tile0[e] = int(total);
+        total += sym ? tm * (tm + 1) / 2 : tm * tn;
+        XRS_REQUIRE(total < (1l << 30), "ragged GEMM group too large");
+    }
+    P.tile0[count] = int(total);
+    P.count = count;
+    const bool split = total < kCUs && total <= xrs_handle_s::kTicketCap;
+    int zmax = 1;
+    size_t slab_elems = 0;
+    double flops = 0.0, bytes = 0.0;
+    for (int e = 0; e < count; ++e) {
+        const int K = P.K[e];
+        int s = split ? std::max(1, std::min(kSliceMax, K / kSliceMin)) : 1;
+        int kps = ((K + s - 1) / s + BK - 1) / BK * BK;
+        s = (K + kps - 1) / kps;
+        P.kps[e] = kps;
+        P.slab0[e] = slab_elems;
+        if (s > 1) slab_elems += size_t(s) * P.M[e] * P.N[e];
+        zmax = std::max(zmax, s);
+        const double m = P.M[e], n = P.N[e], k = K;
+        flops += 2.0 * m * n * k;
+        bytes += 8.0 * (m * k + k * n + m * n * s);
+    }
+    DevBuf slab;
+    if (slab_elems) slab = DevBuf(h, slab_elems * sizeof(double));
+    KernelTimer timer(h, XRS_KFAM_GEMM, flops, bytes, true);
+    const dim3 grid(unsigned(total), 1, unsigned(zmax));
+#define XRS_RAGGED_LAUNCH(TA_, TB_)                                                                                 \
+    hipExtLaunchKernelGGL((k_gemm_f64<32, 32, 16, 2, 2, 2, 2, TA_, TB_, GemmRagged>), grid, dim3(512), 0, h->stream, \
+                          timer.start(), timer.stop(), 0, P, size_t(0), size_t(0), 0, 0, 0, 0, alpha, slab.d(), 1, 0, \
+                          h->tickets, sym ? 1 : 0)
+    if (!ta && !tb) XRS_RAGGED_LAUNCH(false, false);
+    else if (!ta && tb) XRS_RAGGED_LAUNCH(false, true);
+    else if (ta && !tb) XRS_RAGGED_LAUNCH(true, false);
+    else XRS_RAGGED_LAUNCH(true, true);
+#undef XRS_RAGGED_LAUNCH
+    check_launch("k_gemm_f64 (ragged)");
+}
+
+void gemm_ragged(xrs_handle_t h, int count, const GemmRaggedJob* jobs, double alpha, bool ta, bool tb, bool sym) {
+    for (int e = 0; e < count; ++e) {
+        const GemmRaggedJob& g = jobs[e];
+        XRS_REQUIRE(g.M >= 1 && g.N >= 1 && g.K >= 1, "ragged GEMM entries must be non-empty");
+        XRS_REQUIRE(g.M < (1u << 30) && g.N < (1u << 30) && g.K < (1u << 30), "GEMM dimension too large");
+        XRS_REQUIRE(!sym || g.M == g.N, "symmetric entry needs a square result");
+    }
+    for (int b0 = 0; b0 < count; b0 += kGemmBatchMax)
+        launch_ragged(h, jobs + b0, std::min(kGemmBatchMax, count - b0), alpha, ta, tb, sym);
+}
+
 }
 
 #ifdef XRS_GEMM_TRACE
diff --git a/xerus_amd/csrc/scratch_map.hpp b/xerus_amd/csrc/scratch_map.hpp
--- a/xerus_amd/csrc/scratch_map.hpp
+++ b/xerus_amd/csrc/scratch_map.hpp
@@ -28,7 +28,7 @@
 constexpr Region kHostDotOnes{32768, 16, "dot_two_ended: the unit boundary environments (upload source)"};
 constexpr Region kHostRangeAmax{32784, 8, "range_controlled: max |A|, read behind the factorisation's own wait"};
 constexpr Region kHostShardLayout{32800, 16320, "shard_layout: world x d mode-size table (<= 2040 doubles)"};
-constexpr Region kHostChainStatus{49152, 3072, "chain_pass: factorisation statuses (<= 64 edges x 3 jobs x 4 words)"};
+constexpr Region kHostChainStatus{49152, 3072, "free (the chain pass's statuses travel with its deviations: kHostChainBack); first part of kHostGeneralStatus"};
 constexpr Region kHostTruncStatus{53248, 4096, "round_truncate: the 1024 status words of a sweep"};
 constexpr Region kHostRangeProbe{57600, 7680, "probe_core_ranges: one norm per core (<= 960)"};
 constexpr Region kHostMap[] = {kHostLocal,       kHostTruncDev,    kHostDotOnes,     kHostRangeAmax,
@@ -43,9 +43,9 @@
 constexpr Region kHostAmax{384, 8, "range_exponent: max |A|"};
 constexpr Region kHostLocalSlots[] = {kHostResult, kHostOrthEmax, kHostIdentityDev, kHostAmax};
 static_assert(disjoint_within(kHostLocalSlots, kHostLocal.off, kHostLocal.off + kHostLocal.len));
-constexpr Region kHostChainDev{512, 8192, "chain_check: (d - 1) x 16 orthonormality deviations"};
+constexpr Region kHostChainBack{512, 11264, "chain_check: (d - 1) x 16 orthonormality deviations, then the pass's factorisation statuses"};
 constexpr Region kHostSvdCheck{640, 40, "svd_bidiag: residuals (4 doubles) and the multisection status"};
-static_assert(kHostChainDev.off + kHostChainDev.len <= kHostLocal.len && kHostSvdCheck.off + kHostSvdCheck.len <= kHostLocal.len);
+static_assert(kHostChainBack.off + kHostChainBack.len <= kHostLocal.len && kHostSvdCheck.off + kHostSvdCheck.len <= kHostLocal.len);
 
 constexpr Region kDevResult{0, 8, "reduce_to_host: the reduced scalar"};
 constexpr Region kDevIdentityDev{256, 8, "max_abs_dev_identity"};
diff --git a/xerus_amd/csrc/tt.hip b/xerus_amd/csrc/tt.hip
--- a/xerus_amd/csrc/tt.hip
+++ b/xerus_amd/csrc/tt.hip
@@ -285,33 +285,67 @@
 
 
 void gemm_grouped(xrs_handle_t h, const std::vector<GemmJob>& jobs) {
-    std::vector<bool> done(jobs.size(), false);
-    for (size_t i = 0; i < jobs.size(); ++i) {
-        if (done[i]) continue;
+    static const bool ragged = [] {
+        const char* e = std::getenv("XRS_GEMM_RAGGED");
+        return !(e && e[0] == '0');
+    }();
+    const size_t nj = jobs.size();
+    std::vector<size_t> leader(nj), members(nj, 0);
+    for (size_t j = 0; j < nj; ++j) {
+        const GemmJob& o = jobs[j];
+        size_t i = 0;
+        for (; i < j; ++i) {
+            const GemmJob& g = jobs[i];
+            if (leader[i] == i && o.M == g.M && o.N == g.N && o.K == g.K && o.lda == g.lda && o.ldb == g.ldb && o.ta == g.ta &&
+                o.tb == g.tb && o.sym == g.sym && o.alpha == g.alpha && o.tri == g.tri)
+                break;
+        }
+        leader[j] = i;
+        ++members[i];
+    }
+    auto odd_small = [&](size_t j) {
+        const GemmJob& o = jobs[j];
+        return ragged && leader[j] == j && members[j] == 1 && (!o.sym || o.M == o.N) &&
+               gemm_small_tile(o.M, o.N, o.K, o.A, o.lda, o.B, o.ldb, o.sym);
+    };
+    std::vector<bool> done(nj, false);
+    for (size_t i = 0; i < nj; ++i) {
+        if (done[i] || leader[i] != i) continue;
         const GemmJob& g = jobs[i];
-        std::vector<const double*> A, B;
-        std::vector<double*> C;
-        for (size_t j = i; j < jobs.size(); ++j) {
-            const GemmJob& o = jobs[j];
-            if (done[j] || o.M != g.M || o.N != g.N || o.K != g.K || o.lda != g.lda || o.ldb != g.ldb || o.ta != g.ta ||
-                o.tb != g.tb || o.sym != g.sym || o.alpha != g.alpha || o.tri != g.tri)
-                continue;
-            done[j] = true;
-            A.push_back(o.A);
-            B.push_back(o.B);
-            C.push_back(o.C);
-        }
-        if (C.size() == 1 && g.sym) gemm_sym(h, C[0], g.N, g.alpha, A[0], g.lda, g.ta, g.K, B[0], g.ldb, g.tb);
-        else if (C.size() == 1) gemm(h, C[0], g.M, g.N, g.alpha, A[0], g.lda, g.ta, g.K, B[0], g.ldb, g.tb, g.tri);
-        else gemm_batched(h, int(C.size()), C.data(), g.M, g.N, g.alpha, A.data(), g.lda, g.ta, g.K, B.data(), g.ldb,
-                          g.tb, g.sym, g.tri);
-    }
-}
-
+        if (members[i] > 1) {
+            std::vector<const double*> A, B;
+            std::vector<double*> C;
+            for (size_t j = i; j < nj; ++j)
+                if (leader[j] == i) {
+                    A.push_back(jobs[j].A);
+                    B.push_back(jobs[j].B);
+                    C.push_back(jobs[j].C);
+                }
+            gemm_batched(h, int(C.size()), C.data(), g.M, g.N, g.alpha, A.data(), g.lda, g.ta, g.K, B.data(), g.ldb, g.tb,
+                         g.sym, g.tri);
+            continue;
+        }
+        std::vector<GemmRaggedJob> rag;
+        if (odd_small(i))
+            for (size_t j = i; j < nj; ++j) {
+                const GemmJob& o = jobs[j];
+                if (done[j] || o.ta != g.ta || o.tb != g.tb || o.sym != g.sym || o.alpha != g.alpha || !odd_small(j)) continue;
+                rag.push_back({o.A, o.B, o.C, o.M, o.N, o.K, o.lda, o.ldb});
+                if (rag.size() > 1) done[j] = true;
+            }
+        if (rag.size() > 1) gemm_ragged(h, int(rag.size()), rag.data(), g.alpha, g.ta, g.tb, g.sym);
+        else if (g.sym) gemm_sym(h, g.C, g.N, g.alpha, g.A, g.lda, g.ta, g.K, g.B, g.ldb, g.tb);
+        else gemm(h, g.C, g.M, g.N, g.alpha, g.A, g.lda, g.ta, g.K, g.B, g.ldb, g.tb, g.tri);
+    }
+}
+
+constexpr int kChainSlices = 16;
 struct ChainPass {
     std::vector<double*> C;
+    DevBuf back;
     int* status = nullptr;
     int count = 0;
+    size_t dev_words(size_t d) const { return (d - 1) * kChainSlices; }
 };
 
 void chain_pass(TT& t, bool certify, ChainPass& out) {
@@ -336,12 +370,12 @@
         }
     }
     const int cnt = chol_status_count(jobs);
-    int* host_status = scratch::host<int>(h, scratch::kHostChainStatus, size_t(cnt));
-    DevBuf st(h, size_t(cnt) * 4 + 64);
-    chol_enqueue(h, jobs, st.as<int>(), Cs);
-    XRS_HIP(hipMemcpyAsync(host_status, st.d(), size_t(cnt) * 4, hipMemcpyDeviceToHost, h->stream));
+    const size_t back_bytes = out.dev_words(d) * 8 + size_t(cnt) * 4;
+    out.back = DevBuf(h, back_bytes + 64);
+    char* host_back = scratch::host<char>(h, scratch::kHostChainBack, back_bytes);
+    chol_enqueue(h, jobs, reinterpret_cast<int*>(out.back.d() + out.dev_words(d)), Cs);
     XRS_MARK("potrf");
-    out.status = host_status;
+    out.status = reinterpret_cast<int*>(host_back + out.dev_words(d) * 8);
     out.count = cnt;
     out.C.assign(d, nullptr);
     std::vector<DevBuf> W(d);
@@ -375,13 +409,13 @@
     return true;
 }
 
-double chain_check(TT& t, const std::vector<double*>& C) {
+double chain_check(TT& t, const ChainPass& p) {
+    const std::vector<double*>& C = p.C;
     const size_t d = t.d;
     xrs_handle_t h = t.h;
     XRS_MARK("check");
     std::vector<double*> Gr(d, nullptr);
     DevIdArgs da{};
-    DevBuf dev(h, d * 16 * 8 + 64);
     int nchk = 0;
     size_t gtot = 0;
     for (size_t k = 1; k < d; ++k) gtot += t.r[k] * t.r[k];
@@ -399,12 +433,13 @@
         da.n[nchk] = int(t.r[k]);
         ++nchk;
     }
-    da.out = dev.d();
-    constexpr int kSlices = 16;
+    da.out = p.back.d();
+    constexpr int kSlices = kChainSlices;
     hipLaunchKernelGGL(k_dev_identity_many, dim3(nchk, kSlices), dim3(256), 0, h->stream, da);
     check_launch("k_dev_identity_many");
-    double* hd = scratch::host<double>(h, scratch::kHostChainDev, size_t(nchk) * kSlices);
-    XRS_HIP(hipMemcpyAsync(hd, dev.d(), size_t(nchk) * kSlices * 8, hipMemcpyDeviceToHost, h->stream));
+    const size_t back_bytes = p.dev_words(d) * 8 + size_t(p.count) * 4;
+    double* hd = reinterpret_cast<double*>(scratch::host<char>(h, scratch::kHostChainBack, back_bytes));
+    XRS_HIP(hipMemcpyAsync(hd, p.back.d(), back_bytes, hipMemcpyDeviceToHost, h->stream));
     XRS_MARK("enq");
     host_wait(h);
     XRS_MARK("sync");
@@ -425,7 +460,7 @@
     g_marks = marks.on ? &marks : nullptr;
     ChainPass p1;
     chain_pass(t, true, p1);
-    double dev = chain_check(t, p1.C);
+    double dev = chain_check(t, p1);
     if (!chain_status_ok(p1)) {
         for (size_t k = 0; k < d; ++k) t.release(p1.C[k]);
         { g_marks = nullptr; return false; }
@@ -437,7 +472,7 @@
         t2.core = C.data();
         ChainPass p2;
         chain_pass(t2, false, p2);
-        const double dev2 = chain_check(t2, p2.C);
+        const double dev2 = chain_check(t2, p2);
         const bool ok2 = chain_status_ok(p2);
         if (dbg) std::fprintf(stderr, "round_chain: pass 2 orthogonality %.3e (factors %s)\n", dev2, ok2 ? "ok" : "failed");
         if (ok2 && dev2 <= kOrthTol) {
@@ -462,7 +497,7 @@
 bool reorthonormalize(TT& t) {
     ChainPass p;
     chain_pass(t, false, p);
-    const double dev = chain_check(t, p.C);
+    const double dev = chain_check(t, p);
     const bool ok = chain_status_ok(p) && dev <= kOrthTol;
     for (size_t k = 0; k < t.d; ++k) {
         if (ok) t.replace(k, p.C[k]);
@@ -903,6 +938,29 @@
 
 extern "C" {
 
+int xrs_gemm_grouped(xrs_handle_t h, size_t count, const xrs_gemm_job* jobs) {
+    return guarded([&] {
+        XRS_REQUIRE(h, "null handle");
+        XRS_REQUIRE(count == 0 || jobs, "null job table");
+        XRS_REQUIRE(count < (1u << 20), "too many jobs");
+        std::vector<GemmJob> list;
+        for (size_t i = 0; i < count; ++i) {
+            const xrs_gemm_job& j = jobs[i];
+            XRS_REQUIRE(!j.sym || j.M == j.N, "symmetric job needs a square result");
+            XRS_REQUIRE(j.M == 0 || j.N == 0 || j.C, "null C");
+            XRS_REQUIRE(j.K == 0 || j.M == 0 || j.N == 0 || (j.A && j.B), "null A/B");
+            XRS_REQUIRE(j.transA ? j.lda >= j.M || j.K == 0 : j.lda >= j.K || j.M == 0, "lda too small");
+            XRS_REQUIRE(j.transB ? j.ldb >= j.K || j.N == 0 : j.ldb >= j.N || j.K == 0, "ldb too small");
+            XRS_REQUIRE(j.C != j.A && j.C != j.B, "C must not alias A or B");
+            GemmJob g{j.M, j.N, j.K, j.lda, j.ldb, j.transA != 0, j.transB != 0, j.A, j.B, j.C, j.sym != 0};
+            g.alpha = j.alpha;
+            list.push_back(g);
+        }
+        fence_readers(h);
+        gemm_grouped(h, list);
+    });
+}
+
 int xrs_tt_move_core(xrs_handle_t h, size_t d, const size_t* n, size_t* r, double** cores, int canonicalized,
                      size_t core_position, size_t position, int keep_rank) {
     return guarded([&] {
```

Measured after the change: 36770 GFLOP/s (median of 6 runs). +1.7%, better.
